# Lynne-Zheng-Linfang/HS-Pose

Hardware: AMD Instinct MI355X
Metric: point-clouds/sec (N=1028) HS-layer fwd+bwd (higher is better)
Workload: dtype f32; 1 GPU; HS stack (FaceRecon backbone -> feat) fwd+bwd, B=16/GPU N=1028 fp32, train-mode BN, random-init weights (BASELINE configs[1] shape); global_batch=16, points=1028, parallelism=dp1, hipgraph=True, split_graph=False, grad_exchange=none

## Files before the change

hs_pose_amd/_lib.py:

```python
import ctypes
import os

_HERE = os.path.dirname(os.path.abspath(__file__))
LIB_PATH = os.environ.get("HSP_LIB") or os.path.join(_HERE, "libhsp.so")
_lib = None

_vp, _i, _sz = ctypes.c_void_p, ctypes.c_int, ctypes.c_size_t

SIGNATURES = {
    "hsp_version": (_i, []),
    "hsp_error_string": (ctypes.c_char_p, [_i]),
    "hsp_last_hip_error": (ctypes.c_char_p, []),
    "hsp_knn_workspace_bytes": (_sz, [_i, _i, _i, _i]),
    "hsp_knn_f32": (_i, [_vp, _i, _i, _i, _i, _i, _vp, _vp, _sz, _vp]),
    "hsp_nn1_f32": (_i, [_vp, _i, _vp, _i, _i, _vp, _vp]),
    "hsp_rf_surface_fwd": (_i, [_vp, _vp, _vp, _i, _i, _i, _i, _i, _vp, _vp, _vp]),
    "hsp_rf_bwd_workspace_bytes": (_sz, [_i]),
    "hsp_rf_surface_bwd": (_i, [_vp, _vp, _vp, _vp, _i, _i, _i, _i, _vp, _vp, _sz, _vp]),
    "hsp_rf_conv_wants_fwin": (_i, [_i, _i, _i]),
    "hsp_rf_conv_fwd": (_i, [_vp, _vp, _vp, _vp, _i, _i, _i, _i, _i, _vp, _vp, _vp, _vp]),
    "hsp_rf_conv_bwd": (_i, [_vp, _vp, _vp, _vp, _vp, _vp, _vp, _i, _i, _i, _i, _i, _vp, _vp, _vp, _sz, _vp]),
    "hsp_rf_bwd_scatter_workspace_bytes": (_sz, [_i, _i]),
    "hsp_rf_conv_bwd_scatter": (_i, [_vp, _vp, _vp, _vp, _vp, _vp, _i, _i, _i, _i, _vp, _vp, _vp, _sz, _vp]),
    "hsp_rev_build": (_i, [_vp, _i, _i, _i, _i, _i, _vp, _vp, _vp]),
    "hsp_gather_max_bwd_csr": (_i, [_vp, _i, _vp, _vp, _vp, _i, _i, _i, _i, _i, _vp, _vp]),
    "hsp_gather_max_fwd": (_i, [_vp, _vp, _vp, _i, _i, _i, _i, _i, _i, _i, _vp, _vp, _vp]),
    "hsp_pool_fwd": (_i, [_vp, _vp, _vp, _vp, _i, _i, _i, _i, _i, _i, _vp, _vp, _vp, _vp]),
    "hsp_gather_max_bwd": (_i, [_vp, _i, _vp, _vp, _vp, _i, _i, _i, _i, _i, _i, _vp, _i, _vp, _vp]),
    "hsp_points_max_fwd": (_i, [_vp, _i, _i, _i, _vp, _vp, _vp]),
    "hsp_points_max_bwd": (_i, [_vp, _vp, _i, _i, _i, _vp, _vp]),
    "hsp_orl_workspace_bytes": (_sz, [_i, _i, _i]),
    "hsp_knn_exact_workspace_bytes": (_sz, [_i, _i, _i, _i, _i]),
    "hsp_knn_exact_f32": (_i, [_vp, _i, _i, _i, _i, _i, _i, _vp, _vp, _sz, _vp, _vp]),
    "hsp_knn_xyz_workspace_bytes": (_sz, [_i, _i]),
    "hsp_knn_xyz_f32": (_i, [_vp, _i, _i, _i, _i, _i, _vp, _vp, _vp, _sz, _vp, _vp]),
    "hsp_geometry_levels_f32": (_i, [_vp, _i, _i, _vp, _i, _vp, _i, _i, _i, _i, _i, _vp, _vp, _vp, _vp, _vp, _vp, _vp, _vp]),
    "hsp_geometry_all_workspace_bytes": (_sz, [_i, _i]),
    "hsp_geometry_all_f32": (_i, [_vp, _i, _i, _i, _i, _vp, _i, _vp, _i, _i, _i, _i, _i, _vp, _vp, _vp, _vp, _vp, _vp, _vp, _vp, _vp, _vp, _sz,
                                  _vp]),
    "hsp_knn_quadmode_f32": (_i, [_vp, _i, _i, _i, _i, _i, _vp, _vp, _sz, _i, _vp]),
    "hsp_quad_outer_f32": (_i, [_vp, _i, _i, _i, _vp, _vp]),
    "hsp_center_cloud_f32": (_i, [_vp, _i, _i, _vp, _vp, _vp]),
    "hsp_orl_exact_workspace_bytes": (_sz, [_i, _i, _i]),
    "hsp_orl_global_exact_f32": (_i, [_vp, _vp, _i, _i, _i, _i, _i, _vp, _vp, _vp, _sz, _vp]),
    "hsp_bn_eval_f32": (_i, [_vp, ctypes.c_longlong, _i, _vp, _vp, _vp, _vp, _vp, ctypes.c_float, _i, _vp, _vp]),
    "hsp_layer_out_exact_f32": (_i, [_vp, _i, _vp, _i, _vp, _i, _vp, _i, _vp, _i, _vp, _i, _vp, _vp, _i, _i, _i, _i, _vp, _i, _vp]),
    "hsp_orl_global_fwd": (_i, [_vp, _vp, _i, _i, _i, _i, _i, _vp, _vp, _vp, _sz, _vp]),
    "hsp_colsum_rows": (_i, [_vp, _i, _i, _i, _vp, _vp, _sz, _vp]),
    "hsp_add_relu_bwd": (_i, [_vp, _i, _vp, _i, _vp, _i, _i, _vp, _vp]),
    "hsp_residual_bias": (_i, [_vp, _vp, _vp, _i, _i, _i, _vp]),
    "hsp_concat_rows": (_i, [_i, _vp, _vp, _vp, _vp, _vp, _i, _i, _vp, _vp]),
    "hsp_gather_rows_fwd": (_i, [_vp, _vp, _i, _i, _i, _i, _i, _vp, _i, _vp]),
    "hsp_gather_rows_bwd": (_i, [_vp, _i, _vp, _i, _i, _i, _i, _i, _vp, _vp]),
    "hsp_gather_rows_bwd_csr": (_i, [_vp, _i, _vp, _vp, _i, _i, _i, _i, _vp, _vp]),
    "hsp_gemm_rows_workspace_bytes": (_sz, [_i, _i, _i, _i, _i]),
    "hsp_gemm_rows_f32": (_i, [_vp, _i, _vp, _i, _i, _i, _vp, _i, _vp, _i, _i, _i, _i, _i, _vp, _vp, _i, _vp, _i, ctypes.c_float, _vp, _vp, _vp, _i, _vp, _sz, _vp]),
    "hsp_gemm_rows_bf16": (_i, [_vp, _i, _vp, _i, _i, _vp, _i, _vp, _i, _i, _i, _i, _vp, _vp, _i, _vp, _i, ctypes.c_float, _vp, _vp, _vp, _i, _i, _vp, _sz, _vp]),
    "hsp_gemm_wave_supported": (_i, [_i, _i, _i, _i, _i]),
    "hsp_gemm_wave_plan_info": (_i, [_i, _i, _i, _i, _i, _vp]),
    "hsp_gemm_wave_f32": (_i, [_vp, _i, _vp, _i, _i, _i, _vp, _i, _vp, _i, _i, _i, _i, _i, _vp, _vp, _i, _vp, _i, ctypes.c_float, _vp, _vp, _vp, _i, _i, _vp]),
    "hsp_split_params_x3": (_i, [_vp, _i, _i, _vp]),
    "hsp_gemm_x3_supported": (_i, [_i, _i, _i, _i]),
    "hsp_gemm_x3_workspace_bytes": (_sz, [_i, _i, _i, _i]),
    "hsp_gemm_x3_f32": (_i, [_vp, _i, _vp, _i, ctypes.c_longlong, _i, _vp, _i, _vp, _i, ctypes.c_longlong, _i, _i, _i, _vp, _vp, _i, _vp, _i,
                             ctypes.c_float, _vp, _i, _vp, _sz, _vp]),
    "hsp_small_rows_f32": (_i, [_vp, _i, _vp, _i, _i, _i, _i, _i, ctypes.c_float, _vp, _i, _vp]),
    "hsp_small_outer_f32": (_i, [_vp, _i, _vp, _i, _i, _i, _i, _vp, _i, _vp, _i, _i, _vp, _vp]),
    "hsp_colsum_rows_xyz": (_i, [_vp, _vp, _i, _i, _i, _vp, _vp, _sz, _vp]),
    "hsp_colsum_rows_xyz_bf16": (_i, [_vp, _vp, _i, _i, _i, _vp, _vp, _sz, _vp]),
    "hsp_colsum_cloud_ok": (_i, [_i, _i, _i, _i]),
    "hsp_colsum_cloud_f32": (_i, [_vp, _vp, _i, _i, _i, _vp, _vp]),
    "hsp_small_pair_f32": (_i, [_vp, _i, _i, _i, _vp, _i, _i, ctypes.c_float, _vp, _i, _vp, _i, _i, _vp, _i, _vp, _i, _i, _vp, _vp]),
    "hsp_bn_relu_fwd_mixed": (_i, [_vp, _i, _i, _vp, _vp, ctypes.c_float, ctypes.c_float, _i, _vp, _vp, _vp, _vp, _vp, _vp, _vp, _sz, _vp]),
    "hsp_bn_relu_apply_mixed": (_i, [_vp, _i, _i, _vp, _vp, _vp, _vp, _i, _vp, _vp]),
    "hsp_bn_relu_bwd_mixed": (_i, [_vp, _vp, _i, _i, _vp, _vp, _vp, _vp, _i, _vp, _vp, _vp, _vp, _sz, _vp]),
    "hsp_cast_params_bf16": (_i, [_vp, _i, _i, _vp]),
    "hsp_cast_params_pitched_bf16": (_i, [_vp, _i, _i, _vp]),
    "hsp_wgrad_ragged_bf16": (_i, [_vp, _i, _vp, _i, _i, _i, _i, _vp, _i, _vp, _vp, _sz, _vp]),
    "hsp_wgrad_ragged_partial_bf16": (_i, [_vp, _i, _vp, _i, _i, _i, _i, _vp, _i, _vp, _vp, _sz, _vp, _vp]),
    "hsp_gemm_rows_acc_bf16": (_i, [_vp, _i, _vp, _i, _i, _vp, _i, _vp, _i, _i, _i, _i, _vp, _i, _vp, _i, _i, _vp, _sz, _vp]),
    "hsp_points_max_fwd_bf16": (_i, [_vp, _i, _i, _i, _vp, _vp, _vp]),
    "hsp_gemm_rows_bn_tiles_bf16": (_i, [_i, _i, _i]),
    "hsp_gemm_rows_bn_bf16": (_i, [_vp, _i, _vp, _i, _i, _i, _i, _vp, _vp, _i, _vp, _vp, _vp, _i, _vp, _vp, _vp]),
    "hsp_bn_relu_fwd_partials_mixed": (_i, [_vp, _i, _i, _vp, _vp, ctypes.c_float, ctypes.c_float, _i, _vp, _vp, _vp, _vp, _vp, _vp,
                                            _vp, _i, _vp, _vp]),
    "hsp_points_max_bwd_bf16": (_i, [_vp, _vp, _i, _i, _i, _vp, _vp]),
    "hsp_knn_bf16": (_i, [_vp, _i, _i, _i, _i, _i, _vp, _vp, _sz, _vp]),
    "hsp_rf_surface_fwd_bf16": (_i, [_vp, _vp, _vp, _i, _i, _i, _i, _i, _vp, _vp, _vp]),
    "hsp_rf_surface_bwd_bf16": (_i, [_vp, _vp, _vp, _vp, _i, _i, _i, _i, _vp, _vp, _sz, _vp]),
    "hsp_rf_conv_wants_fwin_bf16": (_i, [_i, _i, _i]),
    "hsp_rf_conv_fwd_bf16": (_i, [_vp, _vp, _vp, _vp, _i, _i, _i, _i, _i, _vp, _vp, _vp, _vp]),
    "hsp_rf_conv_bwd_scatter_bf16": (_i, [_vp, _vp, _vp, _vp, _vp, _vp, _i, _i, _i, _i, _vp, _vp, _vp, _sz, _vp]),
    "hsp_gather_max_fwd_bf16": (_i, [_vp, _vp, _vp, _i, _i, _i, _i, _i, _i, _i, _vp, _vp, _vp]),
    "hsp_gather_max_bwd_bf16": (_i, [_vp, _i, _vp, _vp, _vp, _i, _i, _i, _i, _i, _i, _vp, _i, _vp, _vp]),
    "hsp_orl_global_fwd_bf16": (_i, [_vp, _vp, _i, _i, _i, _i, _i, _vp, _vp, _vp, _sz, _vp]),
    "hsp_colsum_rows_bf16": (_i, [_vp, _i, _i, _i, _vp, _vp, _sz, _vp]),
    "hsp_concat_rows_pitched": (_i, [_i, _vp, _vp, _vp, _vp, _vp, _i, _i, _vp, _i, _vp]),
    "hsp_concat_rows_bf16": (_i, [_i, _vp, _vp, _vp, _vp, _vp, _i, _i, _vp, _i, _vp]),
    "hsp_gather_rows_bwd_csr_bf16": (_i, [_vp, _i, _vp, _vp, _i, _i, _i, _i, _vp, _vp]),
    "hsp_wgrad_bf16": (_i, [_vp, _i, _vp, _i, _i, _i, _i, _vp, _i, _vp, _vp, _sz, _vp]),
    "hsp_bn_relu_fwd_bf16": (_i, [_vp, _i, _i, _vp, _vp, ctypes.c_float, ctypes.c_float, _i, _vp, _vp, _vp, _vp, _vp, _vp, _vp, _sz, _vp]),
    "hsp_bn_relu_apply_bf16": (_i, [_vp, _i, _i, _vp, _vp, _vp, _vp, _i, _vp, _vp]),
    "hsp_bn_relu_bwd_bf16": (_i, [_vp, _vp, _i, _i, _vp, _vp, _vp, _vp, _i, _vp, _vp, _vp, _vp, _sz, _vp]),
    "hsp_wgrad_workspace_bytes": (_sz, [_i, _i, _i]),
    "hsp_wgrad_f32": (_i, [_vp, _i, _vp, _i, _i, _i, _i, _vp, _i, _vp, _vp, _sz, _vp]),
    "hsp_bn_workspace_bytes": (_sz, [_i, _i]),
    "hsp_bn_relu_fwd": (_i, [_vp, _i, _i, _vp, _vp, ctypes.c_float, ctypes.c_float, _i, _vp, _vp, _vp, _vp, _vp, _vp, _vp, _sz, _vp]),
    "hsp_bn_relu_apply": (_i, [_vp, _i, _i, _vp, _vp, _vp, _vp, _i, _vp, _vp]),
    "hsp_bn_relu_bwd": (_i, [_vp, _vp, _i, _i, _vp, _vp, _vp, _vp, _i, _vp, _vp, _vp, _vp, _sz, _vp]),
    "hsp_gemm_x3_bn_f32": (_i, [_vp, _i, _vp, _i, ctypes.c_longlong, _i, _vp, _i, _vp, _i, ctypes.c_longlong, _i, _i, _i, _vp, _i, _vp, _i,
                                _vp, _i, _vp, _vp, _vp]),
    "hsp_gemm_x3_bn_tiles": (_i, [_i, _i]),
    "hsp_gemm_x3_bias_bn_f32": (_i, [_vp, _i, _vp, _i, ctypes.c_longlong, _i, _i, _i, _vp, _vp, _i, _vp, _vp, _vp]),
    "hsp_bn_relu_fwd_partials": (_i, [_vp, _i, _i, _vp, _vp, ctypes.c_float, ctypes.c_float, _i, _vp, _vp, _vp, _vp, _vp, _vp, _vp, _i,
                                      _vp, _vp]),
    "hsp_bn_relu_bwd2": (_i, [_vp, _vp, _i, _vp, _i, _i, _i, _vp, _vp, _vp, _vp, _i, _vp, _vp, _vp, _vp, _sz, _vp]),
    "hsp_pc_compact_workspace_bytes": (_sz, [_i, _i]),
    "hsp_pc_compact": (_i, [_vp, _vp, _i, _i, _vp, _vp, _vp, _sz, _vp]),
    "hsp_pc_gather": (_i, [_vp, _vp, _vp, _vp, _vp, _i, _i, _i, _vp, _vp]),
    "hsp_depth_to_pcl": (_i, [_vp, _vp, _vp, _vp, _vp, _i, _i, _i, _vp, _vp]),
    "hsp_generate_rt": (_i, [_vp, _vp, _vp, _vp, _vp, _vp, _i, _i, _vp, _vp]),
    "hsp_sumsq_workspace_bytes": (_sz, [ctypes.c_longlong]),
    "hsp_sumsq_f32": (_i, [_vp, ctypes.c_longlong, _vp, _vp, _sz, _vp]),
    "hsp_ranger_step": (_i, [_vp, _vp, _vp, _vp, _vp, _vp, _i, ctypes.c_float, ctypes.c_float, ctypes.c_float,
                             ctypes.c_float, ctypes.c_float, _i, _i, ctypes.c_float, _i, _vp, ctypes.c_float, _vp]),
    "hsp_chamfer_fwd": (_i, [_vp, _vp, _i, _i, _i, _vp, _vp, _vp, _vp, _vp]),
    "hsp_chamfer_bwd": (_i, [_vp, _vp, _vp, _vp, _vp, _vp, _i, _i, _i, _vp, _vp, _vp]),
    "hsp_fps_workspace_bytes": (_sz, [_i, _i]),
    "hsp_fps_f32": (_i, [_vp, _i, _i, _i, _vp, _vp, _sz, _vp]),
    "hsp_fps_f64": (_i, [_vp, _i, _i, _i, _vp, _vp, _sz, _vp]),
    "hsp_axis_conf_fwd": (_i, [_vp, _i, _vp, _vp, _vp]),
    "hsp_axis_conf_bwd": (_i, [_vp, _vp, _vp, _i, _vp, _vp]),
    "hsp_face_split_fwd": (_i, [_vp, ctypes.c_longlong, _vp, _vp, _vp, _vp]),
    "hsp_face_split_bwd": (_i, [_vp, _vp, _vp, _vp, ctypes.c_longlong, _vp, _vp]),
    "hsp_pose_losses_workspace_bytes": (_sz, [_i]),
    "hsp_pose_losses_fwd": (_i, [_vp] * 17 + [_i, _i, _vp, _vp, _vp, _sz, _vp]),
    "hsp_pose_losses_bwd": (_i, [_vp] * 17 + [_i, _i, _vp, _vp, _vp, _sz] + [_vp] * 11 + [_vp]),
    "hsp_wgrad_partial_f32": (_i, [_vp, _i, _vp, _i, _i, _i, _i, _vp, _i, _vp, _vp, _sz, _vp, _vp]),
    "hsp_wgrad_partial_bf16": (_i, [_vp, _i, _vp, _i, _i, _i, _i, _vp, _i, _vp, _vp, _sz, _vp, _vp]),
    "hsp_wgrad_fold": (_i, [_vp, _i, _vp]),
    "hsp_step_fold": (_i, [_vp, _i, _vp, _i, _vp]),
    "hsp_rf_surface_bwd_partial": (_i, [_vp, _vp, _vp, _vp, _i, _i, _i, _i, _vp, _vp, _sz, _vp, _vp]),
    "hsp_rf_conv_bwd_scatter_partial": (_i, [_vp, _vp, _vp, _vp, _vp, _vp, _i, _i, _i, _i, _vp, _vp, _vp, _sz, _vp, _vp]),
    "hsp_rf_surface_bwd_partial_bf16": (_i, [_vp, _vp, _vp, _vp, _i, _i, _i, _i, _vp, _vp, _sz, _vp, _vp]),
    "hsp_rf_conv_bwd_scatter_partial_bf16": (_i, [_vp, _vp, _vp, _vp, _vp, _vp, _i, _i, _i, _i, _vp, _vp, _vp, _sz, _vp, _vp]),
    "hsp_wgrad_partial_pair_f32": (_i, [_vp, _i, _vp, _i, _i, _i, _i, _vp, _i, _vp, _sz] * 2 + [_vp, _vp]),
    "hsp_pose_augment": (_i, [_vp] * 14 + [_i, _i, _i] + [ctypes.c_float] * 4 + [_vp] * 5),
}


class HspLossCfg(ctypes.Structure):
    _fields_ = [(n, ctypes.c_float) for n in (
        "rot_1_w", "rot_2_w", "rot_regular", "tran_w", "size_w", "r_con_w", "recon_n_w", "recon_d_w", "recon_f_w",
        "recon_v_w", "recon_bb_r_w", "recon_bb_t_w", "recon_bb_s_w", "recon_bb_self_w", "geo_p_w", "prop_pm_w",
        "prop_sym_w")] + [("smooth_l1", ctypes.c_int)]


class HspSplitDesc(ctypes.Structure):
    _fields_ = [("src", ctypes.c_void_p), ("dst", ctypes.c_void_p), ("rows", ctypes.c_int), ("cols", ctypes.c_int),
                ("ld", ctypes.c_int), ("transpose", ctypes.c_int), ("kp", ctypes.c_int), ("tile0", ctypes.c_int),
                ("ps", ctypes.c_longlong)]


class HspError(RuntimeError):
    pass


def lib():
    global _lib
    if _lib is None:
        if not os.path.exists(LIB_PATH):
            raise HspError(
                f"{LIB_PATH} not found: the HIP extension is not built. Run "
                "`python -c 'import __graft_entry__ as g; g.build()'` (or `make -C hs_pose_amd/csrc`). "
                "hs_pose_amd has no CPU / eager fallback.")
        import torch
        L = ctypes.CDLL(LIB_PATH)
        for name, (res, args) in SIGNATURES.items():
            fn = getattr(L, name)
            fn.restype = res
            fn.argtypes = args
        _lib = L
    return _lib


def check(rc, what):
    if rc != 0:
        L = lib()
        msg = L.hsp_error_string(rc).decode()
        hip = L.hsp_last_hip_error().decode()
        raise HspError(f"{what} failed: {msg} (code {rc})" + (f" [hip: {hip}]" if hip and rc == -4 else ""))


class HspWgradPending(ctypes.Structure):
    _fields_ = [("part", ctypes.c_void_p), ("cs_part", ctypes.c_void_p), ("C", ctypes.c_void_p), ("colsum", ctypes.c_void_p),
                ("nparts", ctypes.c_int), ("M", ctypes.c_int), ("N", ctypes.c_int), ("ldc", ctypes.c_int)]


class HspDirsPending(ctypes.Structure):
# ... 3 lines not shown
```

hs_pose_amd/csrc/common.h:

```cpp
#pragma once
#include <hip/hip_runtime.h>
#include <stdint.h>
#include <limits.h>
#include <math.h>

#include "hsp.h"

#define HSP_WAVE 64
#define HSP_NUM_XCD 8
#define HSP_NUM_CU 256

namespace hsp {

void set_last_hip_error(hipError_t e);

inline int check_launch() {
    hipError_t e = hipGetLastError();
    if (e != hipSuccess) {
        set_last_hip_error(e);
        return HSP_ERR_LAUNCH;
    }
    return HSP_OK;
}

inline hipStream_t as_stream(hspStream_t s) { return reinterpret_cast<hipStream_t>(s); }

int knn_feat_select_flags(const float* x, int B, int N, int C, int k, int drop, int quad_mode, int32_t* idx, void* ws, size_t ws_bytes,
                          uint8_t* tie, float* dmat, hspStream_t stream);
int knn3_select_flags(const float* x, int B, int N, int k, int drop, int k2, int32_t* idx, int32_t* idx2, uint8_t* tie,
                      hipStream_t st, bool* needs_tie_pass);

inline int persistent_blocks(long long work_items, int blocks_per_cu) {
    long long g = (long long)HSP_NUM_CU * blocks_per_cu;
    if (work_items < g) g = ((work_items + HSP_NUM_XCD - 1) / HSP_NUM_XCD) * HSP_NUM_XCD;
    if (g < HSP_NUM_XCD) g = HSP_NUM_XCD;
    return (int)g;
}

__device__ __forceinline__ float mul_rn(float a, float b) { return __fmul_rn(a, b); }
__device__ __forceinline__ float add_rn(float a, float b) { return __fadd_rn(a, b); }
__device__ __forceinline__ float sub_rn(float a, float b) { return __fsub_rn(a, b); }

__device__ __forceinline__ float quad3(float x, float y, float z) {
    return add_rn(add_rn(mul_rn(x, x), mul_rn(y, y)), mul_rn(z, z));
}

__device__ __forceinline__ float dot3_chain(float ax, float ay, float az, float bx, float by, float bz) {
    return __fmaf_rn(az, bz, __fmaf_rn(ay, by, mul_rn(ax, bx)));
}

__device__ __forceinline__ float norm2_chain(float x, float y, float z) { return __fmaf_rn(z, z, __fmaf_rn(y, y, mul_rn(x, x))); }

__device__ __forceinline__ float3 unit_dir(float px, float py, float pz, float qx, float qy, float qz) {
    float dx = sub_rn(qx, px), dy = sub_rn(qy, py), dz = sub_rn(qz, pz);
    float n2 = norm2_chain(dx, dy, dz);
    float nrm = fmaxf(sqrtf(n2), 1e-12f);
    return make_float3(__fdiv_rn(dx, nrm), __fdiv_rn(dy, nrm), __fdiv_rn(dz, nrm));
}

__device__ __forceinline__ float3 unit_dir_fast(float px, float py, float pz, float qx, float qy, float qz) {
    const float dx = qx - px, dy = qy - py, dz = qz - pz;
    const float inv = fminf(__builtin_amdgcn_rsqf(dx * dx + dy * dy + dz * dz), 1e12f);
    return make_float3(dx * inv, dy * inv, dz * inv);
}

typedef unsigned short bf16_t;

__device__ __forceinline__ float bf16_bits_to_f32(unsigned v) { return __uint_as_float(v << 16); }
__device__ __forceinline__ unsigned f32_to_bf16_bits(float f) {
    unsigned u = __float_as_uint(f);
    if ((u & 0x7fffffffu) > 0x7f800000u) return (u >> 16) | 0x40u;
    u += 0x7fffu + ((u >> 16) & 1u);
    return u >> 16;
}

template <typename FT> struct Feat;
template <> struct Feat<float> {
    static __device__ __forceinline__ float ld(const float* p) { return *p; }
    static __device__ __forceinline__ void st(float* p, float v) { *p = v; }
    static __device__ __forceinline__ void st_nt(float* p, float v) { __builtin_nontemporal_store(v, p); }
    static __device__ __forceinline__ float4 ld4(const float* p) { return *reinterpret_cast<const float4*>(p); }
    static __device__ __forceinline__ void st4(float* p, float4 v) { *reinterpret_cast<float4*>(p) = v; }
    static __device__ __forceinline__ void st4_nt(float* p, float4 v) {
// ... 28 lines not shown
```

hs_pose_amd/csrc/csr.hip:

```cpp
#include "common.h"

namespace hsp {

#define REV_THREADS 1024

template <bool EDGES_IN_LDS>
__global__ __launch_bounds__(REV_THREADS) void rev_build_kernel(const int32_t* __restrict__ idx, int Nq, int Nsrc,
                                                                int k, int kstride, int32_t* __restrict__ rev_off,
                                                                int32_t* __restrict__ rev_edge) {
    extern __shared__ __attribute__((aligned(16))) char smem[];
    int* cnt = reinterpret_cast<int*>(smem);
    int* led = cnt + Nsrc + 1;
    __shared__ int wsum[REV_THREADS / 64];
    const int b = blockIdx.x, tid = threadIdx.x, lane = tid & 63, wv = tid >> 6;
    const int32_t* ib = idx + (size_t)b * Nq * kstride;
    int32_t* off = rev_off + (size_t)b * (Nsrc + 1);
    int32_t* edge = rev_edge + (size_t)b * Nq * k;
    int* ed = EDGES_IN_LDS ? led : edge;
    const int E = Nq * k;

    for (int m = tid; m <= Nsrc; m += REV_THREADS) cnt[m] = 0;
    __syncthreads();
    for (int e = tid; e < E; e += REV_THREADS) {
        const int i = e / k, n = e - i * k;
        atomicAdd(&cnt[ib[(size_t)i * kstride + n]], 1);
    }
    __syncthreads();
    const int per = (Nsrc + REV_THREADS - 1) / REV_THREADS;
    const int lo = min(tid * per, Nsrc), hi = min(lo + per, Nsrc);
    int s = 0;
    for (int m = lo; m < hi; ++m) s += cnt[m];
    int inc = s;
#pragma unroll
    for (int d = 1; d < 64; d <<= 1) {
        const int v = __shfl_up(inc, d);
        if (lane >= d) inc += v;
    }
    if (lane == 63) wsum[wv] = inc;
    __syncthreads();
    if (wv == 0) {
        int t = lane < REV_THREADS / 64 ? wsum[lane] : 0;
#pragma unroll
        for (int d = 1; d < REV_THREADS / 64; d <<= 1) {
            const int v = __shfl_up(t, d);
            if (lane >= d) t += v;
        }
        if (lane < REV_THREADS / 64) wsum[lane] = t;
    }
    __syncthreads();
    int run = inc - s + (wv ? wsum[wv - 1] : 0);
    for (int m = lo; m < hi; ++m) {
        const int c = cnt[m];
        cnt[m] = run;
        off[m] = run;
        run += c;
    }
    if (tid == 0) off[Nsrc] = E;
    __syncthreads();
    for (int e0 = 0; e0 < E; e0 += REV_THREADS) {
        const int e = e0 + tid;
        if (e < E) {
            const int i = e / k, n = e - i * k;
            const int pos = atomicAdd(&cnt[ib[(size_t)i * kstride + n]], 1);
            ed[pos] = e;
        }
        __syncthreads();
    }
    if (!EDGES_IN_LDS) __threadfence_block();
    __syncthreads();
    if (EDGES_IN_LDS && k == 1) {
        for (int p = tid; p < E; p += REV_THREADS) {
            const int e = led[p];
            const int i = e / k, n = e - i * k;
            const int m = ib[(size_t)i * kstride + n];
            const int a = m ? cnt[m - 1] : 0, z = cnt[m];
            int c = 0;
            for (int q = a; q < z; ++q) c += led[q] < e ? 1 : 0;
            edge[a + c] = e;
        }
    } else {
        for (int m = tid; m < Nsrc; m += REV_THREADS) {
            const int a = m ? cnt[m - 1] : 0, z = cnt[m];
            for (int p = a + 1; p < z; ++p) {
                const int v = ed[p];
                int q = p - 1;
                while (q >= a && ed[q] > v) { ed[q + 1] = ed[q]; --q; }
                ed[q + 1] = v;
            }
        }
        if (EDGES_IN_LDS) {
            __syncthreads();
            for (int e = tid; e < E; e += REV_THREADS) edge[e] = led[e];
        }
    }
}

}

using namespace hsp;

extern "C" int hsp_rev_build(const int32_t* idx, int B, int Nq, int Nsrc, int k, int kstride, int32_t* rev_off,
                             int32_t* rev_edge, hspStream_t stream) {
    if (!idx || !rev_off || !rev_edge || B <= 0 || Nq <= 0 || Nsrc <= 0 || k <= 0 || kstride < k) return HSP_ERR_BAD_ARG;
    const size_t lds0 = (size_t)(Nsrc + 1) * sizeof(int);
    if (lds0 > 140 * 1024) return HSP_ERR_UNSUPPORTED;
    const size_t lds1 = lds0 + (size_t)Nq * k * sizeof(int);
    const bool in_lds = lds1 <= 140 * 1024;
    const size_t lds = in_lds ? lds1 : lds0;
    auto kern = in_lds ? rev_build_kernel<true> : rev_build_kernel<false>;
    if (lds > 60 * 1024) {
        hipError_t e = hipFuncSetAttribute(reinterpret_cast<const void*>(kern), hipFuncAttributeMaxDynamicSharedMemorySize, (int)lds);
        if (e != hipSuccess) { set_last_hip_error(e); return HSP_ERR_LAUNCH; }
    }
    hipLaunchKernelGGL(kern, dim3(B), dim3(REV_THREADS), lds, as_stream(stream), idx, Nq, Nsrc, k, kstride, rev_off,
                       rev_edge);
    return check_launch();
}
```

hs_pose_amd/csrc/gather.hip:

```cpp
#include "common.h"
#include <type_traits>

namespace hsp {

template <typename FT>
__device__ __forceinline__ void gather_max_rows(const FT* __restrict__ fb, const int32_t* __restrict__ nb, int k,
                                                int C, float4& best, int& a0, int& a1, int& a2, int& a3) {
    constexpr int NB = 8;
    int cur[NB], nxt[NB];
#pragma unroll
    for (int u = 0; u < NB; ++u) cur[u] = nb[min(u, k - 1)];
    for (int n0 = 0; n0 < k; n0 += NB) {
#pragma unroll
        for (int u = 0; u < NB; ++u) nxt[u] = nb[min(n0 + NB + u, k - 1)];
        float4 f[NB];
#pragma unroll
        for (int u = 0; u < NB; ++u) f[u] = Feat<FT>::ld4(fb + (size_t)cur[u] * C);
#pragma unroll
        for (int u = 0; u < NB; ++u) {
            const int n = n0 + u;
            if (n < k) {
                if (f[u].x > best.x) { best.x = f[u].x; a0 = n; }
                if (f[u].y > best.y) { best.y = f[u].y; a1 = n; }
                if (f[u].z > best.z) { best.z = f[u].z; a2 = n; }
                if (f[u].w > best.w) { best.w = f[u].w; a3 = n; }
            }
        }
#pragma unroll
        for (int u = 0; u < NB; ++u) cur[u] = nxt[u];
    }
}


template <typename FT>
__global__ __launch_bounds__(256) void gather_max_fwd_kernel(const FT* __restrict__ feat,
                                                             const int32_t* __restrict__ idx,
                                                             const int32_t* __restrict__ qsel, int B, int Nsrc,
                                                             int Nidx, int Nq, int k, int kstride, int C,
                                                             FT* __restrict__ out,
                                                             uint8_t* __restrict__ argmax,
                                                             const float* __restrict__ xyz = nullptr,
                                                             float* __restrict__ xyz_sel = nullptr) {
    const int cq = C >> 2;
    const long long total = (long long)B * Nq * cq;
    for (long long e = (long long)blockIdx.x * 256 + threadIdx.x; e < total; e += (long long)gridDim.x * 256) {
        const int g = (int)(e % cq);
        const long long row = e / cq;
        const int q = (int)(row % Nq);
        const int b = (int)(row / Nq);
        const int qi = qsel ? qsel[q] : q;
        if (xyz_sel && g < 3)
            xyz_sel[row * 3 + g] = xyz[((size_t)b * Nidx + qi) * 3 + g];
        const int32_t* nb = idx + ((size_t)b * Nidx + qi) * kstride;
// ... 107 lines not shown
        if (i < N) {
            const unsigned short* my = strip + pw * k;
            float4 f[K];
#pragma unroll
            for (int n = 0; n < K; ++n) {
                const char* rp = slab + ((unsigned)my[n] << SH);
                if constexpr (sizeof(FT) == 4) f[n] = *reinterpret_cast<const float4*>(rp);
                else {
                    const uint2 u2 = *reinterpret_cast<const uint2*>(rp);
                    f[n] = make_float4(__uint_as_float(u2.x << 16), __uint_as_float(u2.x & 0xffff0000u), __uint_as_float(u2.y << 16),
                                       __uint_as_float(u2.y & 0xffff0000u));
                }
            }
            ORL_STAMP(3 + 3 * (i0 / PASS));
            float4 best = f[0];
#pragma unroll
            for (int n = 1; n + 1 < K; n += 2) {
                best.x = max3_raw(best.x, f[n].x, f[n + 1].x); best.y = max3_raw(best.y, f[n].y, f[n + 1].y);
                best.z = max3_raw(best.z, f[n].z, f[n + 1].z); best.w = max3_raw(best.w, f[n].w, f[n + 1].w);
            }
            if ((K & 1) == 0) {
                best.x = max3_raw(best.x, f[K - 1].x, f[K - 1].x); best.y = max3_raw(best.y, f[K - 1].y, f[K - 1].y);
                best.z = max3_raw(best.z, f[K - 1].z, f[K - 1].z); best.w = max3_raw(best.w, f[K - 1].w, f[K - 1].w);
            }
            int a0 = 0, a1 = 0, a2 = 0, a3 = 0;
#pragma unroll
            for (int n = K - 1; n >= 1; --n) {
                a0 = f[n].x == best.x ? n : a0; a1 = f[n].y == best.y ? n : a1;
                a2 = f[n].z == best.z ? n : a2; a3 = f[n].w == best.w ? n : a3;
            }
            a0 = f[0].x == best.x ? 0 : a0; a1 = f[0].y == best.y ? 0 : a1; a2 = f[0].z == best.z ? 0 : a2; a3 = f[0].w == best.w ? 0 : a3;
            *reinterpret_cast<uchar4*>(argmax + ((size_t)b * N + i) * C + c0 + (q << 2)) =
                make_uchar4((unsigned char)a0, (unsigned char)a1, (unsigned char)a2, (unsigned char)a3);
            s.x += best.x; s.y += best.y; s.z += best.z; s.w += best.w;
        }
        __builtin_amdgcn_fence(__ATOMIC_ACQUIRE, "wavefront");
        ORL_STAMP(4 + 3 * (i0 / PASS));
    }
    ORL_STAMP(30);
#pragma unroll
    for (int d = 2; d < 64; d <<= 1) {
        s.x += __shfl_xor(s.x, d); s.y += __shfl_xor(s.y, d); s.z += __shfl_xor(s.z, d); s.w += __shfl_xor(s.w, d);
    }
    if (lane < 2) red[wave * 2 + q] = s;
    __syncthreads();
    if (tid < 2) {
        float4 t = red[q];
        for (int w = 1; w < ORLT_WG / 64; ++w) { const float4 v = red[w * 2 + q]; t.x += v.x; t.y += v.y; t.z += v.z; t.w += v.w; }
        *reinterpret_cast<float4*>(fg + (size_t)b * C + c0 + (q << 2)) = make_float4(t.x * inv_n, t.y * inv_n, t.z * inv_n, t.w * inv_n);
    }
    ORL_STAMP(31);
}

__device__ __forceinline__ float chunk_fold8(const float* __restrict__ p, int nchunk, int stride) {
    float s[8] = {0.f, 0.f, 0.f, 0.f, 0.f, 0.f, 0.f, 0.f};
    int ch = 0;
    for (; ch + 7 < nchunk; ch += 8) {
#pragma unroll
        for (int u = 0; u < 8; ++u) s[u] += p[(size_t)(ch + u) * stride];
    }
    for (; ch < nchunk; ++ch) s[ch & 7] += p[(size_t)ch * stride];
    return ((s[0] + s[1]) + (s[2] + s[3])) + ((s[4] + s[5]) + (s[6] + s[7]));
}

__global__ __launch_bounds__(256) void chunk_fold_kernel(const float* __restrict__ part, int B, int nchunk, int C,
                                                         float scale, float* __restrict__ out) {
    const int e = blockIdx.x * 256 + threadIdx.x;
    if (e >= B * C) return;
    const int b = e / C, c = e - b * C;
    out[e] = chunk_fold8(part + (size_t)b * nchunk * C + c, nchunk, C) * scale;
}

template <typename FT>
__global__ __launch_bounds__(256) void colsum_partial_kernel(const FT* __restrict__ x, int N, int C,
                                                             float* __restrict__ part, int nchunk, int rows) {
    __shared__ float4 red[256];
    const int cq = C >> 2;
    const int tid = threadIdx.x;
    const int g = tid % cq, rl = tid / cq, RL = 256 / cq;
    const int b = blockIdx.y, chunk = blockIdx.x;
    const int r0 = chunk * rows, r1 = min(N, r0 + rows);
    float4 s = make_float4(0.f, 0.f, 0.f, 0.f);
    for (int i = r0 + rl; i < r1; i += RL) {
        const float4 v = Feat<FT>::ld4(x + ((size_t)b * N + i) * C + (g << 2));
        s.x += v.x; s.y += v.y; s.z += v.z; s.w += v.w;
    }
    red[tid] = s;
    __syncthreads();
    if (rl == 0) {
        for (int l = 1; l < RL; ++l) { const float4 v = red[l * cq + g]; s.x += v.x; s.y += v.y; s.z += v.z; s.w += v.w; }
        *reinterpret_cast<float4*>(part + ((size_t)b * nchunk + chunk) * C + (g << 2)) = s;
    }
}

__device__ __forceinline__ float fma_plain(float a, float b, float c) {
    float r;
    asm volatile("v_fma_f32 %0, %1, %2, %3" : "=v"(r) : "v"(a), "v"(b), "v"(c));
    return r;
}

template <typename FT>
__global__ __launch_bounds__(256) void colsum_xyz_partial_kernel(const FT* __restrict__ x, const float* __restrict__ xyz, int N, int C,
                                                                 float* __restrict__ part, int nchunk, int rows) {
    __shared__ float4 red[4][256];
    const int cq = C >> 2;
    const int tid = threadIdx.x;
    const int g = tid % cq, rl = tid / cq, RL = 256 / cq;
    const int b = blockIdx.y, chunk = blockIdx.x;
    const int r0 = chunk * rows, r1 = min(N, r0 + rows);
    float4 s[4];
#pragma unroll
    for (int q = 0; q < 4; ++q) s[q] = make_float4(0.f, 0.f, 0.f, 0.f);
    for (int i = r0 + rl; i < r1; i += RL) {
        const float4 v = Feat<FT>::ld4(x + ((size_t)b * N + i) * C + (g << 2));
        const float* p3 = xyz + ((size_t)b * N + i) * 3;
        const float w[3] = {p3[0], p3[1], p3[2]};
        s[0].x += v.x; s[0].y += v.y; s[0].z += v.z; s[0].w += v.w;
#pragma unroll
        for (int q = 0; q < 3; ++q) {
            s[q + 1].x = fma_plain(v.x, w[q], s[q + 1].x); s[q + 1].y = fma_plain(v.y, w[q], s[q + 1].y);
            s[q + 1].z = fma_plain(v.z, w[q], s[q + 1].z); s[q + 1].w = fma_plain(v.w, w[q], s[q + 1].w);
        }
    }
#pragma unroll
    for (int q = 0; q < 4; ++q) red[q][tid] = s[q];
    __syncthreads();
    if (rl == 0) {
#pragma unroll
        for (int q = 0; q < 4; ++q) {
            float4 a = s[q];
            for (int l = 1; l < RL; ++l) { const float4 v = red[q][l * cq + g]; a.x += v.x; a.y += v.y; a.z += v.z; a.w += v.w; }
            *reinterpret_cast<float4*>(part + (((size_t)b * nchunk + chunk) * 4 + q) * C + (g << 2)) = a;
        }
    }
}

template <bool XYZ>
__global__ __launch_bounds__(1024) void colsum_cloud_kernel(const float* __restrict__ x, const float* __restrict__ xyz, int N, int C,
                                                            int nchunk, int rows, float* __restrict__ out) {
    extern __shared__ float4 cc_smem[];
    constexpr int NS = XYZ ? 4 : 1;
    const int cq = C >> 2, RL = 256 / cq, G = cq >> 3;
    const int tid = threadIdx.x;
    const int gl = tid % G, rl = (tid / G) % RL, cs = tid / (G * RL);
    const int g = blockIdx.x * G + gl, b = blockIdx.y;
    float4* red = cc_smem;
    float4* cp = cc_smem + 1024;
    for (int c0 = 0; c0 < nchunk; c0 += 32) {
        const int chunk = c0 + cs;
        const int r0 = chunk * rows, r1 = chunk < nchunk ? min(N, r0 + rows) : 0;
        float4 s[NS];
#pragma unroll
        for (int q = 0; q < NS; ++q) s[q] = make_float4(0.f, 0.f, 0.f, 0.f);
        for (int i = r0 + rl; i < r1; i += RL) {
            const float4 v = *reinterpret_cast<const float4*>(x + ((size_t)b * N + i) * C + (g << 2));
            s[0].x += v.x; s[0].y += v.y; s[0].z += v.z; s[0].w += v.w;
            if constexpr (XYZ) {
                const float* p3 = xyz + ((size_t)b * N + i) * 3;
                const float w[3] = {p3[0], p3[1], p3[2]};
#pragma unroll
                for (int q = 0; q < 3; ++q) {
                    s[q + 1].x = fma_plain(v.x, w[q], s[q + 1].x); s[q + 1].y = fma_plain(v.y, w[q], s[q + 1].y);
                    s[q + 1].z = fma_plain(v.z, w[q], s[q + 1].z); s[q + 1].w = fma_plain(v.w, w[q], s[q + 1].w);
                }
            }
        }
#pragma unroll
        for (int q = 0; q < NS; ++q) {
            red[tid] = s[q];
            __syncthreads();
            if (rl == 0 && chunk < nchunk) {
                float4 a = s[q];
                for (int l = 1; l < RL; ++l) { const float4 v = red[(cs * RL + l) * G + gl]; a.x += v.x; a.y += v.y; a.z += v.z; a.w += v.w; }
                cp[((size_t)q * nchunk + chunk) * G + gl] = a;
            }
            __syncthreads();
        }
    }
    const int TC = G << 2;
    if (tid < NS * TC) {
        const int q = tid / TC, c = tid - q * TC;
        out[(size_t)b * NS * C + (size_t)q * C + blockIdx.x * TC + c] =
            chunk_fold8(reinterpret_cast<const float*>(cp) + (size_t)q * nchunk * TC + c, nchunk, TC);
    }
}

__global__ __launch_bounds__(256) void colsum_partial_scalar_kernel(const float* __restrict__ x, int N, int C,
                                                                    float* __restrict__ part, int nchunk, int rows) {
    __shared__ float red[256];
    const int tid = threadIdx.x;
    const int RL = 256 / C;
    const int col = tid % C, rl = tid / C;
    const int b = blockIdx.y, chunk = blockIdx.x;
    const int r0 = chunk * rows, r1 = min(N, r0 + rows);
    float s = 0.f;
    if (rl < RL)
        for (int i = r0 + rl; i < r1; i += RL) s += x[((size_t)b * N + i) * C + col];
    red[tid] = s;
    __syncthreads();
    if (rl == 0) {
        for (int l = 1; l < RL; ++l) s += red[l * C + col];
        part[((size_t)b * nchunk + chunk) * C + col] = s;
    }
}

struct ConcatSeg { const void* src; const int32_t* idx; int width; int kind; int nsrc; int col0; };
struct ConcatDesc { ConcatSeg seg[8]; int nseg; int even; int q0[9]; };

template <typename FT>
__global__ __launch_bounds__(256) void concat_rows_kernel(ConcatDesc d, int B, int N, int W, FT* __restrict__ out) {
    using Pair = typename std::conditional<sizeof(FT) == 4, float2, unsigned>::type;
    const long long rows = (long long)B * N;
    if (d.even == 2) {
        const int lane = threadIdx.x & 63;
        const int total = d.q0[d.nseg];
        for (long long row = (long long)blockIdx.x * 4 + (threadIdx.x >> 6); row < rows; row += (long long)gridDim.x * 4) {
            const int b = (int)(row / N);
            FT* o = out + (size_t)row * W;
            for (int q = lane; q < total; q += 64) {
                int sgi = 0;
                while (q >= d.q0[sgi + 1]) ++sgi;
                const ConcatSeg sg = d.seg[sgi];
                const int c = q - d.q0[sgi];
                if (sg.kind >= 2) {
                    const float* ps = reinterpret_cast<const float*>(sg.src);
                    Feat<FT>::st(o + sg.col0 + c, sg.kind == 2 ? ps[(size_t)b * sg.width + c] : ((long long)ps[b] == c ? 1.f : 0.f));
                    continue;
                }
                const FT* src = reinterpret_cast<const FT*>(sg.src);
                src += sg.kind == 0 ? (size_t)row * sg.width : ((size_t)b * sg.nsrc + sg.idx[row]) * sg.width;
                reinterpret_cast<uint4*>(o + sg.col0)[c] = reinterpret_cast<const uint4*>(src)[c];
            }
            const int used = d.seg[d.nseg - 1].col0 + d.seg[d.nseg - 1].width;
            if (lane < W - used) Feat<FT>::st(o + used + lane, 0.f);
        }
        return;
    }
// ... 467 lines not shown
        hipLaunchKernelGGL(gather_max_bwd_kernel, dim3(stream_grid(total)), dim3(256), 0, st,
                           reinterpret_cast<const float*>(grad_out), grad_bcast, idx, qsel, argmax, B, Nsrc, Nidx, Nq, kstride, C,
                           grad_feat);
        return check_launch();
    }
    return HSP_ERR_UNSUPPORTED;
}
extern "C" int hsp_gather_max_bwd(const float* grad_out, int grad_bcast, const int32_t* idx, const int32_t* qsel,
                                  const uint8_t* argmax, int B, int Nsrc, int Nidx, int Nq, int kstride, int C,
                                  float* grad_feat, int accumulate, const float* extra, hspStream_t stream) {
    return gather_max_bwd_impl<float>(grad_out, grad_bcast, idx, qsel, argmax, B, Nsrc, Nidx, Nq, kstride, C, grad_feat,
                                      accumulate, extra, stream);
}
extern "C" int hsp_gather_max_bwd_bf16(const void* grad_out, int grad_bcast, const int32_t* idx, const int32_t* qsel,
                                       const uint8_t* argmax, int B, int Nsrc, int Nidx, int Nq, int kstride, int C,
                                       hsp_bf16_t* grad_feat, int accumulate, const hsp_bf16_t* extra, hspStream_t stream) {
    return gather_max_bwd_impl<bf16_t>(grad_out, grad_bcast, idx, qsel, argmax, B, Nsrc, Nidx, Nq, kstride, C, grad_feat,
                                       accumulate, extra, stream);
}

extern "C" int hsp_gather_rows_fwd(const float* feat, const int32_t* idx, int idx_shared, int B, int Nsrc, int Nq,
                                   int C, float* out, int out_stride, hspStream_t stream) {
    if (!feat || !idx || !out || B <= 0 || Nsrc <= 0 || Nq <= 0 || C <= 0 || out_stride < C) return HSP_ERR_BAD_ARG;
    hipStream_t st = as_stream(stream);
    if ((C & 3) == 0) {
        const long long total = (long long)B * Nq * (C >> 2);
        hipLaunchKernelGGL(gather_rows_fwd_kernel, dim3(stream_grid(total)), dim3(256), 0, st, feat, idx, idx_shared, B,
                           Nsrc, Nq, C, out, out_stride);
    } else {
        const long long total = (long long)B * Nq * C;
        hipLaunchKernelGGL(gather_rows_fwd_scalar_kernel, dim3(stream_grid(total)), dim3(256), 0, st, feat, idx,
                           idx_shared, B, Nsrc, Nq, C, out, out_stride);
    }
    return check_launch();
}

extern "C" int hsp_gather_rows_bwd(const float* grad_out, int grad_stride, const int32_t* idx, int idx_shared, int B,
                                   int Nsrc, int Nq, int C, float* grad_feat, hspStream_t stream) {
    if (!grad_out || !idx || !grad_feat || B <= 0 || Nsrc <= 0 || Nq <= 0 || C <= 0 || grad_stride < C)
        return HSP_ERR_BAD_ARG;
    hipStream_t st = as_stream(stream);
    if ((C & 3) == 0 && (grad_stride & 1) == 0 && (reinterpret_cast<uintptr_t>(grad_out) & 7) == 0)
        if (const int tc = pick_scatter_cols(Nsrc, C))
            return launch_scatter_tile<1, float>(tc, grad_out, nullptr, grad_stride, 0, idx, idx_shared, nullptr, nullptr, B,
                                                 Nsrc, Nq, Nq, 1, C, grad_feat, 0, nullptr, st);
    hipError_t e = hipMemsetAsync(grad_feat, 0, (size_t)B * Nsrc * C * sizeof(float), st);
    if (e != hipSuccess) { set_last_hip_error(e); return HSP_ERR_LAUNCH; }
    const long long total = (long long)B * Nq * C;
    hipLaunchKernelGGL(gather_rows_bwd_kernel, dim3(stream_grid(total)), dim3(256), 0, st, grad_out, grad_stride, idx,
                       idx_shared, B, Nsrc, Nq, C, grad_feat);
    return check_launch();
}

template <typename FT>
__global__ __launch_bounds__(256) void gather_rows_bwd_csr_kernel(const FT* __restrict__ gout, int gstride,
                                                                  const int32_t* __restrict__ rev_off,
                                                                  const int32_t* __restrict__ rev_edge, int B,
                                                                  int Nsrc, int Nq, int C,
                                                                  FT* __restrict__ gfeat) {
    const int pairs = C >> 1;
    const int tpr = pairs < 256 ? pairs : 256;
    const int RB = 256 / tpr;
    const int rl = threadIdx.x / tpr, t = threadIdx.x - rl * tpr;
    const long long row = (long long)blockIdx.x * RB + rl;
    if (rl >= RB || row >= (long long)B * Nsrc) return;
    const int m = (int)(row % Nsrc), b = (int)(row / Nsrc);
    const int32_t* off = rev_off + (size_t)b * (Nsrc + 1);
    const int32_t* edge = rev_edge + (size_t)b * Nq;
    const int o0 = off[m], o1 = off[m + 1];
    const FT* gb = gout + (size_t)b * Nq * gstride;
    for (int p = t; p < pairs; p += tpr) {
        float2 acc = make_float2(0.f, 0.f);
        for (int e = o0; e < o1; e += 4) {
            float2 v[4];
#pragma unroll
            for (int u = 0; u < 4; ++u) {
                const int q = edge[min(e + u, o1 - 1)];
                if constexpr (sizeof(FT) == 4) {
                    v[u] = *reinterpret_cast<const float2*>(gb + (size_t)q * gstride + 2 * p);
                } else {
                    const unsigned w = *reinterpret_cast<const unsigned*>(gb + (size_t)q * gstride + 2 * p);
                    v[u] = make_float2(__uint_as_float(w << 16), __uint_as_float(w & 0xffff0000u));
                }
            }
#pragma unroll
            for (int u = 0; u < 4; ++u)
                if (e + u < o1) { acc.x += v[u].x; acc.y += v[u].y; }
        }
        if constexpr (sizeof(FT) == 4) *reinterpret_cast<float2*>(gfeat + (size_t)row * C + 2 * p) = acc;
        else *reinterpret_cast<unsigned*>(gfeat + (size_t)row * C + 2 * p) = f32_to_bf16_bits(acc.x) | (f32_to_bf16_bits(acc.y) << 16);
    }
}

template <typename FT>
static int gather_rows_bwd_csr_impl(const FT* grad_out, int grad_stride, const int32_t* rev_off,
                                    const int32_t* rev_edge, int B, int Nsrc, int Nq, int C, FT* grad_feat,
                                    hspStream_t stream) {
    if (!grad_out || !rev_off || !rev_edge || !grad_feat || B <= 0 || Nsrc <= 0 || Nq <= 0 || C <= 0 || grad_stride < C)
        return HSP_ERR_BAD_ARG;
    if ((C & 1) || (grad_stride & 1) || (reinterpret_cast<uintptr_t>(grad_out) & (2 * sizeof(FT) - 1)) ||
        (256 % ((C >> 1) < 256 ? (C >> 1) : 256)))
        return HSP_ERR_UNSUPPORTED;
    const int tpr = (C >> 1) < 256 ? (C >> 1) : 256;
    const int RB = 256 / tpr;
    const long long rows = (long long)B * Nsrc;
    hipLaunchKernelGGL(gather_rows_bwd_csr_kernel<FT>, dim3((unsigned)((rows + RB - 1) / RB)), dim3(256), 0, as_stream(stream),
                       grad_out, grad_stride, rev_off, rev_edge, B, Nsrc, Nq, C, grad_feat);
    return check_launch();
}
extern "C" int hsp_gather_rows_bwd_csr(const float* grad_out, int grad_stride, const int32_t* rev_off,
                                       const int32_t* rev_edge, int B, int Nsrc, int Nq, int C, float* grad_feat,
                                       hspStream_t stream) {
    return gather_rows_bwd_csr_impl<float>(grad_out, grad_stride, rev_off, rev_edge, B, Nsrc, Nq, C, grad_feat, stream);
}
extern "C" int hsp_gather_rows_bwd_csr_bf16(const hsp_bf16_t* grad_out, int grad_stride, const int32_t* rev_off,
                                            const int32_t* rev_edge, int B, int Nsrc, int Nq, int C, hsp_bf16_t* grad_feat,
                                            hspStream_t stream) {
    return gather_rows_bwd_csr_impl<bf16_t>(grad_out, grad_stride, rev_off, rev_edge, B, Nsrc, Nq, C, grad_feat, stream);
}

extern "C" int hsp_gather_max_bwd_csr(const float* grad_out, int grad_bcast, const uint8_t* argmax,
                                      const int32_t* rev_off, const int32_t* rev_edge, int B, int Nsrc, int Nq, int k,
                                      int C, float* grad_feat, hspStream_t stream) {
    if (!grad_out || !argmax || !rev_off || !rev_edge || !grad_feat || B <= 0 || Nsrc <= 0 || Nq <= 0 || k <= 0 || C <= 0)
        return HSP_ERR_BAD_ARG;
    if (C & 3) return HSP_ERR_UNSUPPORTED;
    const long long total = (long long)B * Nsrc * (C >> 2);
    hipLaunchKernelGGL(gather_max_bwd_csr_kernel, dim3(stream_grid(total)), dim3(256), 0, as_stream(stream), grad_out,
                       grad_bcast, argmax, rev_off, rev_edge, B, Nsrc, Nq, k, C, grad_feat);
    return check_launch();
}

extern "C" int hsp_points_max_fwd(const float* x, int B, int N, int C, float* out, int32_t* argrow, hspStream_t stream) {
    if (!x || !out || !argrow || B <= 0 || N <= 0 || C <= 0) return HSP_ERR_BAD_ARG;
    hipLaunchKernelGGL(points_max_fwd_kernel<float>, dim3((C + 63) / 64, B), dim3(1024), 0, as_stream(stream), x, N, C, out,
                       argrow);
    return check_launch();
}

extern "C" int hsp_points_max_fwd_bf16(const hsp_bf16_t* x, int B, int N, int C, float* out, int32_t* argrow,
                                       hspStream_t stream) {
    if (!x || !out || !argrow || B <= 0 || N <= 0 || C <= 0) return HSP_ERR_BAD_ARG;
    hipLaunchKernelGGL(points_max_fwd_kernel<bf16_t>, dim3((C + 63) / 64, B), dim3(1024), 0, as_stream(stream),
                       reinterpret_cast<const bf16_t*>(x), N, C, out, argrow);
    return check_launch();
}

extern "C" int hsp_points_max_bwd(const float* grad_out, const int32_t* argrow, int B, int N, int C, float* grad_x,
                                  hspStream_t stream) {
    if (!grad_out || !argrow || !grad_x || B <= 0 || N <= 0 || C <= 0) return HSP_ERR_BAD_ARG;
    if (C & 3) return HSP_ERR_UNSUPPORTED;
    const long long total = (long long)B * N * (C >> 2);
    hipLaunchKernelGGL(points_max_bwd_kernel<float>, dim3(stream_grid(total)), dim3(256), 0, as_stream(stream), grad_out,
                       argrow, N, C >> 2, total, grad_x);
    return check_launch();
}

extern "C" int hsp_points_max_bwd_bf16(const float* grad_out, const int32_t* argrow, int B, int N, int C, hsp_bf16_t* grad_x,
                                       hspStream_t stream) {
    if (!grad_out || !argrow || !grad_x || B <= 0 || N <= 0 || C <= 0) return HSP_ERR_BAD_ARG;
    if (C & 3) return HSP_ERR_UNSUPPORTED;
// ... 41 lines not shown
}
extern "C" int hsp_orl_global_fwd(const float* feat, const int32_t* idx, int B, int N, int k, int kstride, int C,
                                  float* fg, uint8_t* argmax, void* ws, size_t ws_bytes, hspStream_t stream) {
    return orl_global_fwd_impl<float>(feat, idx, B, N, k, kstride, C, fg, argmax, ws, ws_bytes, stream);
}
extern "C" int hsp_orl_global_fwd_bf16(const hsp_bf16_t* feat, const int32_t* idx, int B, int N, int k, int kstride, int C,
                                       float* fg, uint8_t* argmax, void* ws, size_t ws_bytes, hspStream_t stream) {
    return orl_global_fwd_impl<bf16_t>(feat, idx, B, N, k, kstride, C, fg, argmax, ws, ws_bytes, stream);
}

extern "C" int hsp_colsum_rows(const float* x, int B, int N, int C, float* out, void* ws, size_t ws_bytes,
                               hspStream_t stream) {
    if (!x || !out || B <= 0 || N <= 0 || C <= 0) return HSP_ERR_BAD_ARG;
    if (!colsum_vec4(C) && C > 256) return HSP_ERR_UNSUPPORTED;
    if (!ws || ws_bytes < hsp_orl_workspace_bytes(B, N, C)) return HSP_ERR_WORKSPACE;
    hipStream_t st = as_stream(stream);
    const int rows = chunk_rows(B, N, C);
    const int nchunk = (N + rows - 1) / rows;
    float* part = reinterpret_cast<float*>(ws);
    if (colsum_vec4(C))
        hipLaunchKernelGGL(colsum_partial_kernel<float>, dim3(nchunk, B), dim3(256), 0, st, x, N, C, part, nchunk, rows);
    else
        hipLaunchKernelGGL(colsum_partial_scalar_kernel, dim3(nchunk, B), dim3(256), 0, st, x, N, C, part, nchunk, rows);
    hipLaunchKernelGGL(chunk_fold_kernel, dim3((B * C + 255) / 256), dim3(256), 0, st, part, B, nchunk, C, 1.0f, out);
    return check_launch();
}

template <typename FT>
static int colsum_rows_xyz_impl(const FT* x, const float* xyz, int B, int N, int C, float* out4, void* ws, size_t ws_bytes,
                                hspStream_t stream) {
    if (!x || !xyz || !out4 || B <= 0 || N <= 0 || C <= 0) return HSP_ERR_BAD_ARG;
    if (!colsum_vec4(C)) return HSP_ERR_UNSUPPORTED;
    if (!ws || ws_bytes < 4 * hsp_orl_workspace_bytes(B, N, C)) return HSP_ERR_WORKSPACE;
    hipStream_t st = as_stream(stream);
    const int rows = chunk_rows(B, N, C);
    const int nchunk = (N + rows - 1) / rows;
    float* part = reinterpret_cast<float*>(ws);
    hipLaunchKernelGGL(colsum_xyz_partial_kernel<FT>, dim3(nchunk, B), dim3(256), 0, st, x, xyz, N, C, part, nchunk, rows);
    hipLaunchKernelGGL(chunk_fold_kernel, dim3((B * 4 * C + 255) / 256), dim3(256), 0, st, part, B, nchunk, 4 * C, 1.0f, out4);
    return check_launch();
}
extern "C" int hsp_colsum_rows_xyz(const float* x, const float* xyz, int B, int N, int C, float* out4, void* ws, size_t ws_bytes,
                                   hspStream_t stream) {
    return colsum_rows_xyz_impl<float>(x, xyz, B, N, C, out4, ws, ws_bytes, stream);
}
extern "C" int hsp_colsum_rows_xyz_bf16(const hsp_bf16_t* x, const float* xyz, int B, int N, int C, float* out4, void* ws,
                                        size_t ws_bytes, hspStream_t stream) {
    return colsum_rows_xyz_impl<bf16_t>(x, xyz, B, N, C, out4, ws, ws_bytes, stream);
}

static size_t colsum_cloud_lds(int B, int N, int C, int with_xyz) {
    const int rows = chunk_rows(B, N, C);
    return (1024 + (size_t)(with_xyz ? 4 : 1) * ((N + rows - 1) / rows) * (C >> 5)) * sizeof(float4);
}
extern "C" int hsp_colsum_cloud_ok(int B, int N, int C, int with_xyz) {
    if (B <= 0 || B > 65535 || N <= 0 || C <= 0 || (C & 31) || !colsum_vec4(C)) return 0;
    return colsum_cloud_lds(B, N, C, with_xyz) <= 64 * 1024 ? 1 : 0;
}
extern "C" int hsp_colsum_cloud_f32(const float* x, const float* xyz, int B, int N, int C, float* out, hspStream_t stream) {
    if (!x || !out || B <= 0 || N <= 0 || C <= 0) return HSP_ERR_BAD_ARG;
    if (!hsp_colsum_cloud_ok(B, N, C, xyz != nullptr)) return HSP_ERR_UNSUPPORTED;
    hipStream_t st = as_stream(stream);
    const int rows = chunk_rows(B, N, C);
    const int nchunk = (N + rows - 1) / rows;
    const size_t lds = colsum_cloud_lds(B, N, C, xyz != nullptr);
    if (xyz)
        hipLaunchKernelGGL(colsum_cloud_kernel<true>, dim3(8, B), dim3(1024), lds, st, x, xyz, N, C, nchunk, rows, out);
    else
        hipLaunchKernelGGL(colsum_cloud_kernel<false>, dim3(8, B), dim3(1024), lds, st, x, xyz, N, C, nchunk, rows, out);
    return check_launch();
}

extern "C" int hsp_colsum_rows_bf16(const hsp_bf16_t* x, int B, int N, int C, float* out, void* ws, size_t ws_bytes,
                                    hspStream_t stream) {
    if (!x || !out || B <= 0 || N <= 0 || C <= 0) return HSP_ERR_BAD_ARG;
    if (!colsum_vec4(C)) return HSP_ERR_UNSUPPORTED;
    if (!ws || ws_bytes < hsp_orl_workspace_bytes(B, N, C)) return HSP_ERR_WORKSPACE;
    hipStream_t st = as_stream(stream);
    const int rows = chunk_rows(B, N, C);
    const int nchunk = (N + rows - 1) / rows;
    float* part = reinterpret_cast<float*>(ws);
    hipLaunchKernelGGL(colsum_partial_kernel<bf16_t>, dim3(nchunk, B), dim3(256), 0, st, x, N, C, part, nchunk, rows);
    hipLaunchKernelGGL(chunk_fold_kernel, dim3((B * C + 255) / 256), dim3(256), 0, st, part, B, nchunk, C, 1.0f, out);
    return check_launch();
}

template <typename FT>
static int concat_rows_impl(int nseg, const void* const* src, const int32_t* const* idx, const int* width,
                            const int* kind, const int* nsrc, int B, int N, FT* out, int out_pitch, hspStream_t stream) {
    if (nseg <= 0 || nseg > 8 || !src || !width || !kind || !out || B <= 0 || N <= 0) return HSP_ERR_BAD_ARG;
    ConcatDesc d;
    d.nseg = nseg;
    int col = 0;
    for (int s = 0; s < nseg; ++s) {
        if (!src[s] || width[s] <= 0 || kind[s] < 0 || kind[s] > 3 || (kind[s] == 1 && (!idx || !idx[s]))) return HSP_ERR_BAD_ARG;
        d.seg[s].src = src[s];
        d.seg[s].idx = idx ? idx[s] : nullptr;
        d.seg[s].width = width[s];
        d.seg[s].kind = kind[s];
        d.seg[s].nsrc = nsrc ? nsrc[s] : 0;
        d.seg[s].col0 = col;
        col += width[s];
    }
    if (out_pitch < col) return HSP_ERR_BAD_ARG;
    d.even = (out_pitch & 1) ? 0 : 1;
    for (int s = 0; s < nseg; ++s)
// ... 58 lines not shown
```

hs_pose_amd/csrc/gemm.hip:

```cpp
#include "common.h"
#include "folds.h"

namespace hsp {

using f32x16 = __attribute__((ext_vector_type(16))) float;

#define WG_UNROLL 4

template <bool COLSUM, int KB, typename FT>
__device__ __forceinline__ void wgrad_body(const int bid, const FT* __restrict__ A, int lda,
                                           const FT* __restrict__ B, int ldb, int M, int N, int K,
                                           int SK, int kslice, float* __restrict__ part,
                                           float* __restrict__ cs_part) {
    extern __shared__ __attribute__((aligned(16))) char smem[];
    const int lane = threadIdx.x & 63;
    const int wv = __builtin_amdgcn_readfirstlane(threadIdx.x >> 6);
    const int tiles = (M >> 6) * (N >> 6);
    int slice, t;
    if (KB == 1) {
        const int w = bid * 4 + wv;
        if (w >= tiles * SK) return;
        slice = w / tiles; t = w - slice * tiles;
    } else {
        const int grp = bid / tiles;
        t = bid - grp * tiles;
        slice = grp * 4 + wv;
    }
    const int tiles_m = M >> 6;
    const int tn = t / tiles_m, tm = t - tn * tiles_m;
    const int m0 = tm << 6, n0 = tn << 6;
    const int k0 = slice * kslice;
    const int k1 = min(K, k0 + kslice);
    const int h = lane >> 5, i = lane & 31;
    constexpr int ES = sizeof(FT);
    const __amdgpu_buffer_rsrc_t ra = __builtin_amdgcn_make_buffer_rsrc(
        const_cast<FT*>(A), 0, (int)((((size_t)K - 1) * lda + M) * ES), 0x00020000);
    const __amdgpu_buffer_rsrc_t rb = __builtin_amdgcn_make_buffer_rsrc(
        const_cast<FT*>(B), 0, (int)((((size_t)K - 1) * ldb + N) * ES), 0x00020000);
    const int va = (h * lda + m0 + 2 * i) * ES, vb = (h * ldb + n0 + 2 * i) * ES;
    f32x16 c00, c01, c10, c11;
#pragma unroll
    for (int r = 0; r < 16; ++r) { c00[r] = 0.f; c01[r] = 0.f; c10[r] = 0.f; c11[r] = 0.f; }
    float2 cs = make_float2(0.f, 0.f);

    float2 a0[WG_UNROLL], b0[WG_UNROLL], a1[WG_UNROLL], b1[WG_UNROLL];
    auto load_group = [&](int kk, float2 (&aa)[WG_UNROLL], float2 (&bb)[WG_UNROLL]) {
#pragma unroll
        for (int u = 0; u < WG_UNROLL; ++u) {
            if constexpr (ES == 4) {
                const auto x = __builtin_amdgcn_raw_buffer_load_b64(ra, va, (kk + 2 * u) * lda * 4, 0);
                const auto y = __builtin_amdgcn_raw_buffer_load_b64(rb, vb, (kk + 2 * u) * ldb * 4, 0);
                aa[u] = make_float2(__int_as_float(x[0]), __int_as_float(x[1]));
                bb[u] = make_float2(__int_as_float(y[0]), __int_as_float(y[1]));
            } else {
// ... 33 lines not shown
            const int row = (r & 3) + 8 * (r >> 2) + 4 * h;
            *reinterpret_cast<float2*>(pc + (size_t)(m0 + 2 * row) * N + n0 + 2 * i) = make_float2(c00[r], c01[r]);
            *reinterpret_cast<float2*>(pc + (size_t)(m0 + 2 * row + 1) * N + n0 + 2 * i) = make_float2(c10[r], c11[r]);
        }
        if (COLSUM && tm == 0) {
            cs.x += __shfl_xor(cs.x, 32);
            cs.y += __shfl_xor(cs.y, 32);
            if (h == 0) *reinterpret_cast<float2*>(cs_part + (size_t)slice * N + n0 + 2 * i) = cs;
        }
        return;
    }
    float* buf = reinterpret_cast<float*>(smem);
    float2* csb = reinterpret_cast<float2*>(buf + 4 * 4 * 16 * 64);
#pragma unroll
    for (int r = 0; r < 16; ++r) {
        buf[((wv * 4 + 0) * 16 + r) * 64 + lane] = c00[r];
        buf[((wv * 4 + 1) * 16 + r) * 64 + lane] = c01[r];
        buf[((wv * 4 + 2) * 16 + r) * 64 + lane] = c10[r];
        buf[((wv * 4 + 3) * 16 + r) * 64 + lane] = c11[r];
    }
    if (COLSUM) csb[wv * 64 + lane] = cs;
    __syncthreads();
    const int grp = bid / tiles;
    float* pc = part + (size_t)grp * M * N;
    const int ta = wv >> 1, tb = wv & 1;
#pragma unroll
    for (int r = 0; r < 16; ++r) {
        float v = buf[((0 * 4 + wv) * 16 + r) * 64 + lane];
        v += buf[((1 * 4 + wv) * 16 + r) * 64 + lane];
        v += buf[((2 * 4 + wv) * 16 + r) * 64 + lane];
        v += buf[((3 * 4 + wv) * 16 + r) * 64 + lane];
        const int row = (r & 3) + 8 * (r >> 2) + 4 * h;
        pc[(size_t)(m0 + 2 * row + ta) * N + n0 + 2 * i + tb] = v;
    }
    if (COLSUM && tm == 0 && wv == 0) {
        float2 c = csb[lane];
#pragma unroll
        for (int w2 = 1; w2 < 4; ++w2) { c.x += csb[w2 * 64 + lane].x; c.y += csb[w2 * 64 + lane].y; }
        c.x += __shfl_xor(c.x, 32);
        c.y += __shfl_xor(c.y, 32);
        if (h == 0) *reinterpret_cast<float2*>(cs_part + (size_t)grp * N + n0 + 2 * i) = c;
    }
}

template <bool COLSUM, int KB, typename FT>
__global__ __launch_bounds__(256) void wgrad_kernel(const FT* __restrict__ A, int lda,
                                                    const FT* __restrict__ B, int ldb, int M, int N, int K,
                                                    int SK, int kslice, float* __restrict__ part,
                                                    float* __restrict__ cs_part) {
    wgrad_body<COLSUM, KB, FT>((int)blockIdx.x, A, lda, B, ldb, M, N, K, SK, kslice, part, cs_part);
}

struct WgradProb { const float* A; const float* B; float* part; int lda, ldb, M, N, K, SK, kslice; };
__global__ __launch_bounds__(256) void wgrad_pair_kernel(const WgradProb p0, const WgradProb p1, int blocks0) {
    const bool second = (int)blockIdx.x >= blocks0;
    const WgradProb& p = second ? p1 : p0;
    wgrad_body<false, 4, float>((int)blockIdx.x - (second ? blocks0 : 0), p.A, p.lda, p.B, p.ldb, p.M, p.N, p.K, p.SK, p.kslice,
                                p.part, nullptr);
}

__global__ __launch_bounds__(256) void wgrad_reduce_kernel(const float* __restrict__ part, int SK, int M, int N,
                                                           float* __restrict__ C, int ldc,
                                                           const float* __restrict__ cs_part,
                                                           float* __restrict__ colsum) {
    __shared__ float4 red[4][64];
    const int le = threadIdx.x & 63, sg = threadIdx.x >> 6;
    const int nq = N >> 2;
    const long long total = (long long)M * nq;
    const long long ncs = colsum ? (N >> 2) : 0;
    const long long e = (long long)blockIdx.x * 64 + le;
    float4 s = make_float4(0.f, 0.f, 0.f, 0.f);
    const float* src = nullptr;
    size_t stride = 0;
    if (e < total) { src = part + (size_t)e * 4; stride = (size_t)M * N; }
    else if (e < total + ncs) { src = cs_part + (size_t)(e - total) * 4; stride = (size_t)N; }
    if (src) {
        float4 s2 = make_float4(0.f, 0.f, 0.f, 0.f);
        int sl = sg;
        for (; sl + 4 < SK; sl += 8) {
            const float4 v = *reinterpret_cast<const float4*>(src + (size_t)sl * stride);
            const float4 u = *reinterpret_cast<const float4*>(src + (size_t)(sl + 4) * stride);
            s.x += v.x; s.y += v.y; s.z += v.z; s.w += v.w;
            s2.x += u.x; s2.y += u.y; s2.z += u.z; s2.w += u.w;
        }
        if (sl < SK) {
            const float4 v = *reinterpret_cast<const float4*>(src + (size_t)sl * stride);
            s.x += v.x; s.y += v.y; s.z += v.z; s.w += v.w;
        }
        s.x += s2.x; s.y += s2.y; s.z += s2.z; s.w += s2.w;
    }
    red[sg][le] = s;
    __syncthreads();
    if (sg == 0 && src) {
        float4 r = red[0][le];
#pragma unroll
        for (int g = 1; g < 4; ++g) { const float4 v = red[g][le]; r.x += v.x; r.y += v.y; r.z += v.z; r.w += v.w; }
        if (e < total) {
            const int m = (int)(e / nq), q = (int)(e - (long long)m * nq);
            float* c = C + (size_t)m * ldc + (q << 2);
            c[0] = r.x; c[1] = r.y; c[2] = r.z; c[3] = r.w;
        } else {
            *reinterpret_cast<float4*>(colsum + (size_t)(e - total) * 4) = r;
        }
    }
}

struct WgradFoldTab {
// ... 469 lines not shown
            if (rc) return rc;
            if (pending) { *pending = HspWgradPending{part, cs_part, C, colsum_B, sk2, M, N, ldc}; return HSP_OK; }
            const long long total = (long long)M * (N >> 2) + (colsum_B ? (N >> 2) : 0);
            hipLaunchKernelGGL(wgrad_reduce_kernel, dim3((unsigned)((total + 63) / 64)), dim3(256), 0, st, part, sk2, M, N, C, ldc,
                               cs_part, colsum_B);
            return check_launch();
        }
    }
    const int sk = wgrad_pick_sk(M, N, K, &ks, &kb);
    const int nparts = sk / kb;
    float* part = reinterpret_cast<float*>(ws);
    float* cs_part = part + (size_t)nparts * M * N;
    int rc = colsum_B ? wgrad_launch<true, FT>(A, lda, B, ldb, M, N, K, sk, ks, kb, part, cs_part, st)
                      : wgrad_launch<false, FT>(A, lda, B, ldb, M, N, K, sk, ks, kb, part, cs_part, st);
    if (rc) return rc;
    if (pending) { *pending = HspWgradPending{part, cs_part, C, colsum_B, nparts, M, N, ldc}; return HSP_OK; }
    const long long total = (long long)M * (N >> 2) + (colsum_B ? (N >> 2) : 0);
    hipLaunchKernelGGL(wgrad_reduce_kernel, dim3((unsigned)((total + 63) / 64)), dim3(256), 0, st, part, nparts, M, N, C,
                       ldc, cs_part, colsum_B);
    return check_launch();
}

extern "C" int hsp_wgrad_f32(const float* A, int lda, const float* B, int ldb, int M, int N, int K, float* C, int ldc,
                             float* colsum_B, void* ws, size_t ws_bytes, hspStream_t stream) {
    return wgrad_impl<float>(A, lda, B, ldb, M, N, K, C, ldc, colsum_B, ws, ws_bytes, stream);
}
extern "C" int hsp_wgrad_bf16(const hsp_bf16_t* A, int lda, const hsp_bf16_t* B, int ldb, int M, int N, int K, float* C,
                              int ldc, float* colsum_B, void* ws, size_t ws_bytes, hspStream_t stream) {
    return wgrad_impl<bf16_t>(A, lda, B, ldb, M, N, K, C, ldc, colsum_B, ws, ws_bytes, stream);
}

extern "C" int hsp_wgrad_ragged_bf16(const hsp_bf16_t* A, int lda, const hsp_bf16_t* B, int ldb, int M, int N, int K, float* C,
                                     int ldc, float* colsum_B, void* ws, size_t ws_bytes, hspStream_t stream) {
    return wgrad_impl<bf16_t>(A, lda, B, ldb, M, N, K, C, ldc, colsum_B, ws, ws_bytes, stream, nullptr, true);
}
extern "C" int hsp_wgrad_ragged_partial_bf16(const hsp_bf16_t* A, int lda, const hsp_bf16_t* B, int ldb, int M, int N, int K,
                                             float* C, int ldc, float* colsum_B, void* ws, size_t ws_bytes,
                                             HspWgradPending* pending, hspStream_t stream) {
    if (!pending) return HSP_ERR_BAD_ARG;
    return wgrad_impl<bf16_t>(A, lda, B, ldb, M, N, K, C, ldc, colsum_B, ws, ws_bytes, stream, pending, true);
}

extern "C" int hsp_wgrad_partial_f32(const float* A, int lda, const float* B, int ldb, int M, int N, int K, float* C, int ldc,
                                     float* colsum_B, void* ws, size_t ws_bytes, HspWgradPending* pending, hspStream_t stream) {
    if (!pending) return HSP_ERR_BAD_ARG;
    return wgrad_impl<float>(A, lda, B, ldb, M, N, K, C, ldc, colsum_B, ws, ws_bytes, stream, pending);
}
extern "C" int hsp_wgrad_partial_bf16(const hsp_bf16_t* A, int lda, const hsp_bf16_t* B, int ldb, int M, int N, int K, float* C,
                                      int ldc, float* colsum_B, void* ws, size_t ws_bytes, HspWgradPending* pending,
                                      hspStream_t stream) {
    if (!pending) return HSP_ERR_BAD_ARG;
    return wgrad_impl<bf16_t>(A, lda, B, ldb, M, N, K, C, ldc, colsum_B, ws, ws_bytes, stream, pending);
}
extern "C" int hsp_wgrad_partial_pair_f32(const float* A0, int lda0, const float* B0, int ldb0, int M0, int N0, int K0, float* C0,
                                          int ldc0, void* ws0, size_t ws_bytes0, const float* A1, int lda1, const float* B1,
                                          int ldb1, int M1, int N1, int K1, float* C1, int ldc1, void* ws1, size_t ws_bytes1,
                                          HspWgradPending* pending, hspStream_t stream) {
    if (!pending) return HSP_ERR_BAD_ARG;
    int ks0, kb0, ks1, kb1;
    const bool shapes_ok = A0 && B0 && C0 && A1 && B1 && C1 && M0 > 0 && N0 > 0 && K0 > 0 && M1 > 0 && N1 > 0 && K1 > 0 &&
                           !((M0 | N0 | M1 | N1) & 63) && !((lda0 | ldb0 | lda1 | ldb1) & 1) && lda0 >= M0 && ldb0 >= N0 &&
                           lda1 >= M1 && ldb1 >= N1 && ldc0 >= N0 && ldc1 >= N1;
    if (shapes_ok) {
        int sk0 = wgrad_pick_sk(M0, N0, K0, &ks0, &kb0), sk1 = wgrad_pick_sk(M1, N1, K1, &ks1, &kb1);
        if (kb0 == 4 && kb1 == 4) {
            constexpr int G = 4 * WG_UNROLL;
            const int t0 = (M0 >> 6) * (N0 >> 6), t1 = (M1 >> 6) * (N1 >> 6);
            int total = t0 * (sk0 / 4) + t1 * (sk1 / 4);
            for (int it = 0; it < 8 && total > 2 * HSP_NUM_CU && sk0 > 8 && sk1 > 8; ++it) {
                const double f = (double)(2 * HSP_NUM_CU) / total;
                auto shrink = [&](int K, int& sk, int& ks) {
                    int want = (int)(sk * f) & ~3;
                    if (want >= sk) want = sk - 4;
                    if (want < 8) want = 8;
                    ks = ((K + want - 1) / want + G - 1) / G * G;
                    sk = (((K + ks - 1) / ks) + 3) & ~3;
                };
                shrink(K0, sk0, ks0);
                shrink(K1, sk1, ks1);
                total = t0 * (sk0 / 4) + t1 * (sk1 / 4);
            }
        }
        if (kb0 == 4 && kb1 == 4 && ws0 && ws1 && ws_bytes0 >= hsp_wgrad_workspace_bytes(M0, N0, K0) &&
            ws_bytes1 >= hsp_wgrad_workspace_bytes(M1, N1, K1)) {
            const WgradProb p0{A0, B0, reinterpret_cast<float*>(ws0), lda0, ldb0, M0, N0, K0, sk0, ks0};
            const WgradProb p1{A1, B1, reinterpret_cast<float*>(ws1), lda1, ldb1, M1, N1, K1, sk1, ks1};
            const int blocks0 = (M0 >> 6) * (N0 >> 6) * (sk0 / 4), blocks1 = (M1 >> 6) * (N1 >> 6) * (sk1 / 4);
            const size_t lds = (size_t)4 * 4 * 16 * 64 * sizeof(float) + (size_t)4 * 64 * sizeof(float2);
            static bool attr_set = false;
            if (!attr_set) {
                hipError_t e = hipFuncSetAttribute(reinterpret_cast<const void*>(wgrad_pair_kernel),
                                                   hipFuncAttributeMaxDynamicSharedMemorySize, (int)lds);
                if (e != hipSuccess) { set_last_hip_error(e); return HSP_ERR_LAUNCH; }
                attr_set = true;
            }
            hipLaunchKernelGGL(wgrad_pair_kernel, dim3(blocks0 + blocks1), dim3(256), lds, as_stream(stream), p0, p1, blocks0);
            int rc = check_launch();
            if (rc) return rc;
            pending[0] = HspWgradPending{p0.part, nullptr, C0, nullptr, sk0 / 4, M0, N0, ldc0};
            pending[1] = HspWgradPending{p1.part, nullptr, C1, nullptr, sk1 / 4, M1, N1, ldc1};
            return HSP_OK;
        }
    }
    int rc = wgrad_impl<float>(A0, lda0, B0, ldb0, M0, N0, K0, C0, ldc0, nullptr, ws0, ws_bytes0, stream, pending);
    if (rc) return rc;
    return wgrad_impl<float>(A1, lda1, B1, ldb1, M1, N1, K1, C1, ldc1, nullptr, ws1, ws_bytes1, stream, pending + 1);
}

extern "C" int hsp_wgrad_fold(const HspWgradPending* pending, int n, hspStream_t stream) {
    if (!pending || n <= 0 || n > HSP_FOLD_MAX_WGRAD) return HSP_ERR_BAD_ARG;
    WgradFoldTab tab;
    tab.n = n;
    int blocks = 0;
    for (int i = 0; i < n; ++i) {
        const HspWgradPending& p = pending[i];
        if (!p.part || !p.C || p.nparts <= 0 || p.M <= 0 || p.N <= 0 || (p.N & 3) || p.ldc < p.N || (p.colsum && !p.cs_part))
            return HSP_ERR_BAD_ARG;
        tab.first[i] = blocks;
        const long long total = (long long)p.M * (p.N >> 2) + (p.colsum ? (p.N >> 2) : 0);
        blocks += (int)((total + 63) / 64);
        tab.p[i] = p;
    }
    tab.first[n] = blocks;
    hipLaunchKernelGGL(wgrad_reduce_multi_kernel, dim3((unsigned)blocks), dim3(256), 0, as_stream(stream), tab);
    return check_launch();
}

static bool wgrad_pending_ok(const HspWgradPending& p) {
    return p.part && p.C && p.nparts > 0 && p.M > 0 && p.N > 0 && !(p.N & 3) && p.ldc >= p.N && !(p.colsum && !p.cs_part);
}

extern "C" int hsp_step_fold(const HspWgradPending* wgrads, int nw, const HspDirsPending* dirs, int nd, hspStream_t stream) {
    if (nw < 0 || nd < 0 || nw > HSP_FOLD_MAX_WGRAD || nd > HSP_FOLD_MAX_DIRS || (nw && !wgrads) || (nd && !dirs)) return HSP_ERR_BAD_ARG;
    if (nw + nd == 0) return HSP_OK;
    StepFoldTab tab;
    tab.nw = nw; tab.nd = nd;
    int blocks = 0;
    for (int i = 0; i < nw; ++i) {
        const HspWgradPending& p = wgrads[i];
        if (!wgrad_pending_ok(p)) return HSP_ERR_BAD_ARG;
        tab.wfirst[i] = blocks;
        const long long total = (long long)p.M * (p.N >> 2) + (p.colsum ? (p.N >> 2) : 0);
        blocks += (int)((total + 63) / 64);
        tab.w[i] = p;
    }
    tab.wfirst[nw] = blocks;
    int dblocks = 0;
    for (int i = 0; i < nd; ++i) {
        const HspDirsPending& p = dirs[i];
        if (!p.part || !p.dirs || !p.grad_dirs || p.nparts <= 0 || p.SC <= 0) return HSP_ERR_BAD_ARG;
        tab.dfirst[i] = dblocks;
        dblocks += (p.SC + 63) / 64;
        tab.d[i] = p;
    }
    tab.dfirst[nd] = dblocks;
    hipLaunchKernelGGL(step_fold_kernel, dim3((unsigned)(blocks + dblocks)), dim3(256), 0, as_stream(stream), tab);
    return check_launch();
}
```

hs_pose_amd/ops.py:

```python
import ctypes
import os

import torch

from ._lib import HspError, check, lib

_vp = ctypes.c_void_p

DETERMINISTIC = os.environ.get("HSP_DETERMINISTIC", "0") == "1"


def _p(t):
    return _vp(t.data_ptr()) if t is not None else _vp(0)


def _stream():
    return _vp(torch.cuda.current_stream().cuda_stream)


def _req(t, dtype, name):
    if not isinstance(t, torch.Tensor) or not t.is_cuda:
        raise HspError(f"{name}: expected a GPU tensor (hs_pose_amd has no CPU path), got "
                       f"{getattr(t, 'device', type(t))}")
    if t.dtype != dtype:
# ... 2 lines not shown


_FEAT_DTYPES = (torch.float32, torch.bfloat16)


def _reqf(t, name, like=None):
    if not isinstance(t, torch.Tensor) or not t.is_cuda:
        raise HspError(f"{name}: expected a GPU tensor (hs_pose_amd has no CPU path), got "
                       f"{getattr(t, 'device', type(t))}")
    if t.dtype not in _FEAT_DTYPES or (like is not None and t.dtype != like.dtype):
        raise HspError(f"{name}: expected dtype {like.dtype if like is not None else 'float32 or bfloat16'}, got {t.dtype}")
    return t if t.is_contiguous() else t.contiguous()


def _sfx(t):
    return "_bf16" if t.dtype == torch.bfloat16 else ""


def _es(t):
    return 2 if t.dtype == torch.bfloat16 else 4


def _ws(nbytes, device):
    return torch.empty(max(int(nbytes), 16), dtype=torch.uint8, device=device)


class KernelTimer:

    def __init__(self, only=None):
        self.only = set(only) if only else None
        self.records = []

    def summary(self):
        out = {}
        for name, key, ab, fl, e0, e1 in self.records:
            d = out.setdefault((name, key), dict(calls=0, total_ms=0.0, abytes=ab, aflops=fl))
            d["calls"] += 1
            d["total_ms"] += e0.elapsed_time(e1)
        for d in out.values():
            d["avg_us"] = 1e3 * d["total_ms"] / d["calls"]
        return out


_timer = None
design_stream_bytes = {}


def set_timer(t):
    global _timer
    prev, _timer = _timer, t
    return prev


def _run(name, args, key="", abytes=0, aflops=0):
    fn = getattr(lib(), name)
    t = _timer
    if t is not None and (t.only is None or name in t.only):
        e0 = torch.cuda.Event(enable_timing=True)
        e1 = torch.cuda.Event(enable_timing=True)
        e0.record()
        rc = fn(*args)
        e1.record()
        t.records.append((name, key, abytes, aflops, e0, e1))
    else:
        rc = fn(*args)
    check(rc, name)



def knn_xyz(xyz, k, k2=0, drop_first=True):
    x = _req(xyz.detach(), torch.float32, "knn_xyz.xyz")
    B, N, C = x.shape
    if C != 3:
        raise HspError("knn_xyz: expects (B,N,3) coordinates")
    k2 = int(k2) if k2 and k2 < k else 0
    m = k + (1 if drop_first else 0)
    if m + 1 > 33 or N < 2 or N * 16 > 160 * 1024:
        idx = knn(x, k, drop_first, _plain_xyz=True)
        return idx, (idx[:, :, :k2].contiguous() if k2 else None)
    idx = torch.empty(B, N, k, dtype=torch.int32, device=x.device)
    idx2 = torch.empty(B, N, k2, dtype=torch.int32, device=x.device) if k2 else None
    wsb = lib().hsp_knn_xyz_workspace_bytes(B, N)
    ws = _ws(wsb, x.device)
    _run("hsp_knn_xyz_f32", (_p(x), B, N, k, k2, 1 if drop_first else 0, _p(idx), _p(idx2), _p(ws), wsb, None, _stream()),
         key=f"B{B}N{N}k{k}", abytes=B * N * (12 + 4 * (k + k2)))
    return idx, idx2


def geometry_all(xyz, k0, kpool0, sel1, sel2, k1, kpool, k2):
    x = _req(xyz.detach(), torch.float32, "geometry_all.xyz")
    s1, s2 = _req(sel1, torch.int32, "geometry_all.sel1"), _req(sel2, torch.int32, "geometry_all.sel2")
    B, N0, C = x.shape
    N1, N2 = s1.numel(), s2.numel()
    if (C != 3 or not (64 <= N2 <= N1 <= 576) or not (576 < N0 <= 1088) or B * N0 >= 131072 or k1 + 2 > 33 or k2 + 2 > 33 or k0 + 2 > 33
            or k1 + 1 > N1 or k2 + 1 > N2 or not 0 < kpool <= k1 or not 0 < kpool0 < k0):
        return None
    dev = x.device
    i32 = dict(dtype=torch.int32, device=dev)
    out = dict(v1=torch.empty(B, N1, 3, dtype=torch.float32, device=dev), v2=torch.empty(B, N2, 3, dtype=torch.float32, device=dev),
               idx0=torch.empty(B, N0, k0, **i32), idx0_pool=torch.empty(B, N0, kpool0, **i32),
               idx1=torch.empty(B, N1, k1, **i32), idx1_pool=torch.empty(B, N1, kpool, **i32), idx2=torch.empty(B, N2, k2, **i32),
               up1=torch.empty(B, N0, **i32), up2=torch.empty(B, N0, **i32))
    wsb = lib().hsp_geometry_all_workspace_bytes(B, N0)
    ws = _ws(wsb, dev)
    _run("hsp_geometry_all_f32", (_p(x), B, N0, k0, kpool0, _p(s1), N1, _p(s2), N2, k1, kpool, k2, 1, _p(out["idx0"]), _p(out["idx0_pool"]),
                                  _p(out["v1"]), _p(out["v2"]), _p(out["idx1"]), _p(out["idx1_pool"]), _p(out["idx2"]), _p(out["up1"]),
                                  _p(out["up2"]), _p(ws), wsb, _stream()),
         key=f"B{B}N{N0}/{N1}/{N2}k{k0}", abytes=B * (12 * N0 + 4 * (N0 * (k0 + kpool0) + N1 * (k1 + kpool + 3) + N2 * (k2 + 3)) + 8 * N0))
    return out


def geometry_levels(xyz, sel1, sel2, k1, kpool, k2):
    x = _req(xyz.detach(), torch.float32, "geometry_levels.xyz")
    s1, s2 = _req(sel1, torch.int32, "geometry_levels.sel1"), _req(sel2, torch.int32, "geometry_levels.sel2")
    B, N0, C = x.shape
    N1, N2 = s1.numel(), s2.numel()
    if C != 3 or not (64 <= N2 <= N1 <= 576) or N1 > N0 or k1 + 2 > 33 or k2 + 2 > 33 or k1 + 1 > N1 or k2 + 1 > N2 or not 0 < kpool <= k1:
        return None
    dev = x.device
# ... 46 lines not shown
    if _ext_state is None:
        from . import _ext
        try:
            _ext_state = bool(_ext.available()) and _ext.ext() is not None
        except _ext.HspExtError:
            _ext_state = False
    return _ext_state


def center_cloud(points):
    pts = _req(points.detach(), torch.float32, "center_cloud.points")
    if _timer is None and _ext_ok():
        from ._ext import ext
        return ext().center_cloud(pts)
    B, N, _ = pts.shape
    out = torch.empty_like(pts)
    mean = torch.empty(B, 1, 3, dtype=torch.float32, device=pts.device)
    _run("hsp_center_cloud_f32", (_p(pts), B, N, _p(out), _p(mean), _stream()), key=f"B{B}N{N}", abytes=24 * B * N)
    return out, mean


def nn1(target, source):
    t = _req(target.detach(), torch.float32, "nn1.target")
    s = _req(source.detach(), torch.float32, "nn1.source")
    B, Nt, C = t.shape
    if C != 3 or s.shape[2] != 3 or s.shape[0] != B:
        raise HspError("nn1: expects (B,Nt,3) and (B,Ns,3)")
    idx = torch.empty(B, Nt, dtype=torch.int32, device=t.device)
    _run("hsp_nn1_f32", (_p(t), Nt, _p(s), s.shape[1], B, _p(idx), _stream()),
         key=f"B{B}Nt{Nt}Ns{s.shape[1]}", abytes=B * (16 * Nt + 12 * s.shape[1]))
    return idx


def rev_index(idx, k, n_src):
    cache = getattr(idx, "_hsp_rev", None)
    if cache is None:
        cache = {}
        idx._hsp_rev = cache
    hit = cache.get((k, n_src))
    if hit is not None:
        return hit
    if idx.dim() == 2:
        (B, Nq), kstride = idx.shape, 1
    else:
        B, Nq, kstride = idx.shape
    off = torch.empty(B, n_src + 1, dtype=torch.int32, device=idx.device)
    edge = torch.empty(B, Nq * k, dtype=torch.int32, device=idx.device)
    _run("hsp_rev_build", (_p(idx), B, Nq, n_src, k, kstride, _p(off), _p(edge), _stream()),
         key=f"B{B}Nq{Nq}k{k}", abytes=B * (8 * Nq * k + 4 * n_src))
    cache[(k, n_src)] = (off, edge)
    return off, edge



class _RFSurface(torch.autograd.Function):
    @staticmethod
    def forward(ctx, xyz, idx, dirs_n, S):
        xyz = _req(xyz, torch.float32, "rf_surface.xyz")
        idx = _req(idx, torch.int32, "rf_surface.idx")
        dirs_n = _req(dirs_n, torch.float32, "rf_surface.dirs")
        B, N, k = idx.shape
        SC = dirs_n.shape[1]
        K = SC // S
        out = torch.empty(B, N, K, dtype=torch.float32, device=xyz.device)
        arg = torch.empty(B, N, SC, dtype=torch.uint16, device=xyz.device)
        _run("hsp_rf_surface_fwd", (_p(xyz), _p(idx), _p(dirs_n), B, N, k, S, K, _p(out), _p(arg), _stream()),
             key=f"B{B}N{N}k{k}S{S}C{K}", abytes=B * N * (12 + 4 * k + 4 * K + SC) + 12 * SC)
        ctx.save_for_backward(xyz, idx, dirs_n, arg)
        ctx.S = S
        return out

    @staticmethod
    def backward(ctx, g):
        xyz, idx, dirs_n, arg = ctx.saved_tensors
        g = _req(g, torch.float32, "rf_surface.grad")
        B, N, k = idx.shape
        SC = dirs_n.shape[1]
        gd = torch.empty_like(dirs_n)
        L = lib()
        wsb = L.hsp_rf_bwd_scatter_workspace_bytes(B, SC)
        ws = _ws(wsb, g.device)
        _rf_bwd_dirs_call("hsp_rf_surface_bwd", "", (_p(xyz), _p(dirs_n), _p(arg), _p(g), B, N, ctx.S, SC // ctx.S, _p(gd)), ws, wsb,
                          (dirs_n, gd), key=f"B{B}N{N}S{ctx.S}C{SC // ctx.S}", abytes=B * N * (12 + 4 * (SC // ctx.S) + SC) + 24 * SC)
        return None, None, gd, None


class _RFConv(torch.autograd.Function):
    @staticmethod
    def forward(ctx, xyz, idx, dirs_n, fm, S):
        xyz = _req(xyz, torch.float32, "rf_conv.xyz")
        idx = _req(idx, torch.int32, "rf_conv.idx")
        dirs_n = _req(dirs_n, torch.float32, "rf_conv.dirs")
        fm = _req(fm, torch.float32, "rf_conv.fm")
        B, N, k = idx.shape
        SC = dirs_n.shape[1]
        C = SC // S
        if fm.shape[-1] != (S + 1) * C:
            raise HspError("rf_conv: fm must have (S+1)*C columns")
        out = torch.empty(B, N, C, dtype=torch.float32, device=xyz.device)
        out, arg, fwin = _rf_conv_fwd_raw(xyz, idx, dirs_n, fm, S, any(ctx.needs_input_grad))
        ctx.save_for_backward(xyz, idx, dirs_n, fwin if fwin is not None else fm, arg)
        ctx.S = S
        return out

    @staticmethod
    def backward(ctx, g):
# ... 257 lines not shown
    sfx = "bf16" if A2.dtype == torch.bfloat16 else "f32"
    es = 2 if A2.dtype == torch.bfloat16 else 4
    batch = WgradBatch.current
    sf = StepFolds.current
    sink = batch.items if batch is not None else sf.wgrads if sf is not None and sf.bare_wgrad else None
    if sink is not None:
        from ._lib import HspWgradPending
        pend = HspWgradPending()
        _run(f"{entry}_partial_{sfx}", (_p(A2), A2.stride(0), _p(B2), B2.stride(0), M, N, K, _p(out), out.stride(0), _p(cs),
                                        _p(ws), wsb, ctypes.byref(pend), _stream()),
             key=f"M{M}N{N}K{K}", abytes=es * K * (M + N) + 4 * M * N, aflops=2 * M * N * K)
        sink.append((pend, ws, _hold(out), _hold(cs)))
    else:
        _run(f"{entry}_{sfx}", (_p(A2), A2.stride(0), _p(B2), B2.stride(0), M, N, K, _p(out), out.stride(0), _p(cs),
                                _p(ws), wsb, _stream()),
             key=f"M{M}N{N}K{K}", abytes=es * K * (M + N) + 4 * M * N, aflops=2 * M * N * K)
    return (out, cs) if colsum else out


def wgrad(A2, B2, out=None, colsum=False):
    K, M = A2.shape
    N = B2.shape[1]
    if out is None:
        out = torch.empty(M, N, dtype=torch.float32, device=A2.device)
    bf16 = A2.dtype == torch.bfloat16
    if _wgrad_ragged_ok(A2, B2, out):
        return _wgrad_custom(A2, B2, out, colsum, entry="hsp_wgrad_ragged" if bf16 else "hsp_wgrad")
    if _wgrad_ok(A2, B2, out):
        return _wgrad_custom(A2, B2, out, colsum)
    if bf16:
        raise HspError("bf16 weight gradient: channel counts must be multiples of 64")
    return _wgrad_fallback(A2, B2, out, colsum)


def _wgrad_ragged_ok(A2, B2, out):
    K, M = A2.shape
    N = B2.shape[1]
    if A2.dtype == torch.bfloat16:
        return (M % 64 != 0 and N % 128 == 0 and A2.stride(1) == 1 and B2.stride(1) == 1 and A2.stride(0) % 8 == 0
                and B2.stride(0) % 8 == 0)
    return (M % 64 != 0 and M >= 128 and N % 128 == 0
            and -(-M // 128) * (N // 128) >= 4 and A2.dtype == torch.float32 and B2.dtype == torch.float32 and A2.is_cuda
            and A2.stride(1) == 1 and B2.stride(1) == 1 and out.stride(1) == 1 and A2.stride(0) % 4 == 0 and B2.stride(0) % 4 == 0
            and A2.stride(0) >= (M + 3) // 4 * 4 and A2.data_ptr() % 16 == 0 and B2.data_ptr() % 16 == 0)


def _wgrad_ok(A2, B2, out):
    K, M = A2.shape
    N = B2.shape[1]
    return (M % 64 == 0 and N % 64 == 0 and A2.stride(1) == 1 and B2.stride(1) == 1 and out.stride(1) == 1
            and A2.stride(0) % 2 == 0 and B2.stride(0) % 2 == 0 and A2.dtype in _FEAT_DTYPES and A2.is_cuda)


def wgrad_pair(A0, B0, out0, A1, B1, out1):
    batch = WgradBatch.current
    if batch is None or A0.dtype != torch.float32 or not _wgrad_ok(A0, B0, out0) or not _wgrad_ok(A1, B1, out1):
        wgrad(A0, B0, out=out0)
        wgrad(A1, B1, out=out1)
        return
    from ._lib import HspWgradPending
    L = lib()
    (K0, M0), N0 = A0.shape, B0.shape[1]
    (K1, M1), N1 = A1.shape, B1.shape[1]
    wsb0, wsb1 = L.hsp_wgrad_workspace_bytes(M0, N0, K0), L.hsp_wgrad_workspace_bytes(M1, N1, K1)
    ws0, ws1 = _ws(wsb0, A0.device), _ws(wsb1, A0.device)
    pend = (HspWgradPending * 2)()
    _run("hsp_wgrad_partial_pair_f32", (_p(A0), A0.stride(0), _p(B0), B0.stride(0), M0, N0, K0, _p(out0), out0.stride(0), _p(ws0), wsb0,
                                        _p(A1), A1.stride(0), _p(B1), B1.stride(0), M1, N1, K1, _p(out1), out1.stride(0), _p(ws1), wsb1,
                                        pend, _stream()),
         key=f"M{M0}N{N0}K{K0}+M{M1}N{N1}K{K1}", abytes=4 * (K0 * (M0 + N0) + M0 * N0 + K1 * (M1 + N1) + M1 * N1),
         aflops=2 * (M0 * N0 * K0 + M1 * N1 * K1))
    batch.items.append((HspWgradPending.from_buffer_copy(pend[0]), ws0, _hold(out0)))
    batch.items.append((HspWgradPending.from_buffer_copy(pend[1]), ws1, _hold(out1)))


def _ld(t):
    if t.dim() != 2 or t.stride(1) != 1:
        raise HspError("gemm_rows: operands must be 2-D with contiguous rows (stride(1) == 1)")
    return t.stride(0) if t.shape[0] > 1 else max(t.stride(0), t.shape[1])


def gemm_rows(A1, B1, nn1=False, A2=None, B2=None, nn2=False, bias=None, resid=None, cloud_bias=None, rows_per_cloud=0,
              out=None, alpha=1.0, xyz3=None, w3=None):
    dt = A1.dtype
    if dt not in (torch.float32, torch.bfloat16):
        raise HspError(f"gemm_rows: fp32 or bf16 operands, got {dt}")
    for t_, nm in ((A1, "A1"), (B1, "B1"), (A2, "A2"), (B2, "B2"), (resid, "resid")):
        if t_ is not None and (not t_.is_cuda or t_.dtype != dt):
            raise HspError(f"gemm_rows.{nm}: expected a {dt} GPU tensor")
    if out is not None and (not out.is_cuda or out.dtype not in (dt, torch.float32)):
        raise HspError(f"gemm_rows.out: expected a {dt} (or, for bf16 operands, fp32) GPU tensor")
    M, K1 = A1.shape
    N = B1.shape[1] if nn1 else B1.shape[0]
    if (B1.shape[0] if nn1 else B1.shape[1]) != K1:
        raise HspError("gemm_rows: A1 / B1 inner dimensions differ")
    K2 = 0
    if A2 is not None:
        K2 = A2.shape[1]
        if A2.shape[0] != M or (B2.shape[1] if nn2 else B2.shape[0]) != N or (B2.shape[0] if nn2 else B2.shape[1]) != K2:
            raise HspError("gemm_rows: second source has the wrong shape")
    if out is None:
        out = torch.empty(M, N, dtype=dt, device=A1.device)
    for t_ in (bias, cloud_bias, xyz3, w3):
        if t_ is not None and (t_.dtype != torch.float32 or not t_.is_cuda or not t_.is_contiguous()):
            raise HspError("gemm_rows: bias / cloud_bias / xyz3 / w3 must be contiguous fp32 GPU tensors")
    if (xyz3 is None) != (w3 is None) or (xyz3 is not None and (xyz3.shape != (M, 3) or w3.shape != (N, 3))):
        raise HspError("gemm_rows: xyz3 (M,3) and w3 (N,3) go together")
    flops = 2 * M * N * (K1 + K2)
    es = 4 if dt == torch.float32 else 2
    ab = es * (M * (K1 + K2) + N * (K1 + K2) + M * N * (2 if resid is not None else 1))
    key = f"M{M}N{N}K{K1}" + (f"+{K2}" if K2 else "")
    wsb = lib().hsp_gemm_rows_workspace_bytes(M, N, K1, K2, es)
    ws = _ws(wsb, A1.device) if wsb else None
    if dt == torch.float32:
        _run("hsp_gemm_rows_f32", (_p(A1), _ld(A1), _p(B1), _ld(B1), 1 if nn1 else 0, K1,
                                   _p(A2), _ld(A2) if A2 is not None else 0, _p(B2), _ld(B2) if B2 is not None else 0,
                                   1 if nn2 else 0, K2, M, N, _p(bias), _p(resid), _ld(resid) if resid is not None else 0,
                                   _p(cloud_bias), int(rows_per_cloud), float(alpha), _p(xyz3), _p(w3), _p(out), _ld(out),
                                   _p(ws), wsb, _stream()),
             key=key, abytes=ab, aflops=flops)
    else:
        if nn1 or nn2:
            raise HspError("gemm_rows: bf16 operands must be (N,K) (pass the transposed copy)")
        _run("hsp_gemm_rows_bf16", (_p(A1), _ld(A1), _p(B1), _ld(B1), K1,
                                    _p(A2), _ld(A2) if A2 is not None else 0, _p(B2), _ld(B2) if B2 is not None else 0, K2,
                                    M, N, _p(bias), _p(resid), _ld(resid) if resid is not None else 0, _p(cloud_bias),
# ... 340 lines not shown
    return out


def _orl_fwd_raw(F3, idx_x, k):
    B, N, C = F3.shape
    fg = torch.empty(B, C, dtype=torch.float32, device=F3.device)
    arg = torch.empty(B, N, C, dtype=torch.uint8, device=F3.device)
    L = lib()
    wsb = L.hsp_orl_workspace_bytes(B, N, C)
    ws = _ws(wsb, F3.device)
    _run("hsp_orl_global_fwd" + _sfx(F3), (_p(F3), _p(idx_x), B, N, k, idx_x.shape[2], C, _p(fg), _p(arg), _p(ws), wsb, _stream()),
         key=f"B{B}N{N}k{k}C{C}", abytes=B * N * (_es(F3) * C + 4 * k + C))
    return fg, arg


def _residual_bias(out3, f3, t2):
    B, N, C = out3.shape
    _run("hsp_residual_bias", (_p(out3), _p(f3), _p(t2.contiguous()), B, N, C, _stream()), key=f"B{B}N{N}C{C}",
         abytes=12 * B * N * C)


def colsum_rows(x3):
    B, N, C = x3.shape
    if x3.dtype == torch.float32 and (((C % 4 or 256 % (C // 4)) and C > 256) or not x3.is_contiguous()):
        return x3.sum(dim=1)
    out = torch.empty(B, C, dtype=torch.float32, device=x3.device)
    L = lib()
    wsb = L.hsp_orl_workspace_bytes(B, N, C)
    ws = _ws(wsb, x3.device)
    _run("hsp_colsum_rows" + _sfx(x3), (_p(x3), B, N, C, _p(out), _p(ws), wsb, _stream()), key=f"B{B}N{N}C{C}",
         abytes=_es(x3) * B * N * C)
    return out


def colsum_rows_xyz(g, xyz):
    B, N, C = g.shape
    mom = torch.empty(B, 4 * C, dtype=torch.float32, device=g.device)
    wsb = 4 * lib().hsp_orl_workspace_bytes(B, N, C)
    ws = _ws(wsb, g.device)
    _run("hsp_colsum_rows_xyz" + _sfx(g), (_p(g), _p(xyz), B, N, C, _p(mom), _p(ws), wsb, _stream()), key=f"B{B}N{N}C{C}",
         abytes=B * N * (_es(g) * C + 12))
    return mom


LAUNCH_DIET = True
_between_launches_hook = None


def _orl_bwd_small_ok(B, N, C, with_xyz):
    return (LAUNCH_DIET and B <= 64 and C % 128 == 0 and C <= 2048
            and lib().hsp_colsum_cloud_ok(B, N, C, 1 if with_xyz else 0) == 1)


def _orl_bwd_small(g, xyz, fg, Wb, gWb, gste=None):
    B, N, C = g.shape
    ns = 4 if xyz is not None else 1
    mom = torch.empty(B, ns * C, dtype=torch.float32, device=g.device)
    _run("hsp_colsum_cloud_f32", (_p(g), _p(xyz), B, N, C, _p(mom), _stream()), key=f"B{B}N{N}C{C}{'x' if xyz is not None else ''}",
         abytes=B * N * (4 * C + (12 if xyz is not None else 0)))
    if _between_launches_hook is not None:
        _between_launches_hook(mom)
    gfg = torch.empty(B, C, dtype=torch.float32, device=g.device)
    _run("hsp_small_pair_f32", (_p(mom), _ld(mom), B, C, _p(Wb), _ld(Wb), Wb.shape[1], 1.0 / N, _p(gfg), _ld(gfg),
                                _p(fg), _ld(fg), fg.shape[1], _p(gWb), _ld(gWb),
                                _p(mom[:, C:]) if xyz is not None else None, _ld(mom) if xyz is not None else 0,
                                C if xyz is not None else 0, _p(gste), _stream()),
         key=f"B{B}C{C}", abytes=4 * (B * 3 * C + 2 * C * C))
    return gfg


def _orl_bwd_accumulate_raw(gfg_over_n, idx_x, arg, k, gF3, extra=None):
    B, N, C = gF3.shape
    if DETERMINISTIC and gF3.dtype == torch.float32:
        tmp = torch.empty_like(gF3)
        off, edge = rev_index(idx_x, k, N)
        _run("hsp_gather_max_bwd_csr", (_p(gfg_over_n), 1, _p(arg), _p(off), _p(edge), B, N, N, k, C, _p(tmp), _stream()),
             key=f"B{B}Ns{N}Nq{N}k{k}C{C}bc", abytes=B * N * (4 * C + 8 * k + C))
        gF3.add_(tmp)
        if extra is not None:
            gF3.add_(extra)
    else:
        _run("hsp_gather_max_bwd" + _sfx(gF3), (_p(gfg_over_n), 1, _p(idx_x), _vp(0), _p(arg), B, N, N, N, idx_x.shape[2], C,
                                                _p(gF3), 1, _p(extra), _stream()),
             key=f"B{B}Ns{N}Nq{N}C{C}bc+", abytes=B * N * (3 * _es(gF3) * C + 4 * idx_x.shape[2] + C))


def _rf_conv_fwd_raw(xyz, idx, directions, fm, S, need_bwd=True):
    B, N, k = idx.shape
    SC = directions.shape[1]
    C = SC // S
    sfx, es = _sfx(fm), _es(fm)
    out = torch.empty(B, N, C, dtype=fm.dtype, device=xyz.device)
    arg = torch.empty(B, N, SC, dtype=torch.uint16, device=xyz.device)
    want = need_bwd and (sfx or not DETERMINISTIC) and getattr(lib(), "hsp_rf_conv_wants_fwin" + sfx)(N, S, C)
    fwin = torch.empty(B, N, SC, dtype=fm.dtype, device=xyz.device) if want else None
    key = f"B{B}N{N}k{k}S{S}C{C}"
    stream = B * N * (12 + 4 * k + es * (S + 1) * C + es * C + 2 * SC + (es * SC if fwin is not None else 0)) + 12 * SC
    if sfx:
        ab = stream
    else:
        design_stream_bytes[("hsp_rf_conv_fwd", key)] = stream
        ab = B * N * (12 + 4 * k + 4 * (S + 1) * C + 4 * C + SC) + 12 * SC
    _run("hsp_rf_conv_fwd" + sfx, (_p(xyz), _p(idx), _p(directions), _p(fm), B, N, k, S, C, _p(out), _p(arg), _p(fwin), _stream()),
         key=key, abytes=ab)
    return out, arg, fwin


def _rf_conv_bwd_raw(xyz, idx, directions, fm, arg, gF3, S):
    B, N, _ = gF3.shape
    SC = directions.shape[1]
    C = SC // S
    sfx, es = _sfx(gF3), _es(gF3)
# ... 93 lines not shown
    def forward(ctx, xyz, X, idx_f, idx_x, k, S, weights, bias, directions, w_ste3, w_conv23, bn_shift=None, out_f32=False):
        w_ste, w_conv2 = w_ste3.squeeze(-1), w_conv23.squeeze(-1)
        xyz = _req(xyz, torch.float32, "hs_layer.xyz")
        X = _reqf(X, "hs_layer.X")
        idx_f = _req(idx_f, torch.int32, "hs_layer.idx_f")
        idx_x = _req(idx_x, torch.int32, "hs_layer.idx_x")
        directions = _req(directions, torch.float32, "hs_layer.directions")
        B, N, Cin = X.shape
        SC = directions.shape[1]
        C = SC // S
        X2 = X.view(B * N, Cin)
        exact = _exact and bn_shift is None and _exact_layer_ok(N, Cin, C, (X2, weights, w_ste, w_conv2))
        fm = gemm_wave(X2, weights, True, bias=bias) if exact else _fm_rows(X2, weights, bias)
        need_bwd = any(ctx.needs_input_grad)
        F3, arg, fwin = _rf_conv_fwd_raw(xyz, idx_f, directions, fm.view(B, N, -1), S, need_bwd)
        if fwin is not None:
            fm = fwin
        fm = fm.view(B, N, -1)
        F2 = F3.view(B * N, C)
        out3 = torch.empty(B, N, C, dtype=torch.float32 if out_f32 else X.dtype, device=X.device)
        if exact:
            fg, arg_o = _orl_fwd_exact(F3, idx_x, k)
            _layer_out_exact(F2, w_conv2, fg, N, out3, ste=gemm_wave(X2, w_ste, False))
            part = None
        else:
            fg, arg_o = _orl_fwd_raw(F3, idx_x, k)
            t2 = _mm_nt(fg, w_conv2[:, C:])
            part = _layer_out_rows(X2, w_ste, F2, w_conv2, t2, out3, bn_shift=bn_shift)
        ctx.save_for_backward(xyz, X, idx_f, idx_x, fm, arg, F3, arg_o, fg, weights, directions, w_ste3, w_conv23)
        ctx.k, ctx.S, ctx.x3 = k, S, x3_planes
        if bn_shift is not None:
            if part is None:
                part = torch.empty(0, dtype=torch.float32, device=out3.device)
            ctx.mark_non_differentiable(part)
            ctx.set_materialize_grads(False)
            return out3, part
        return out3

    @staticmethod
    def backward(ctx, g, _gpart=None):
        xyz, X, idx_f, idx_x, fm, arg, F3, arg_o, fg, weights, directions, w_ste3, w_conv23 = ctx.saved_tensors
        w_ste, w_conv2 = w_ste3.squeeze(-1), w_conv23.squeeze(-1)
        k, S = ctx.k, ctx.S
        f32 = X.dtype == torch.float32
        if not f32 and g.dtype == torch.float32:
            g = g.bfloat16()
        g = _reqf(g, "hs_layer.grad", like=X)
        B, N, Cin = X.shape
        C = F3.shape[2]
        g2, X2, F2 = g.view(B * N, C), X.view(B * N, Cin), F3.view(B * N, C)
        Wb = w_conv2[:, C:]
        small = f32 and _orl_bwd_small_ok(B, N, C, False)
        g_conv2 = torch.empty_like(w_conv2)
        if small:
            gfg_n = _orl_bwd_small(g, None, fg, Wb, g_conv2[:, C:])
        else:
            gt = colsum_rows(g)
        with WgradBatch(), x3_scope(ctx.x3):
            g_ste = torch.empty(C, Cin, dtype=torch.float32, device=g.device)
            wgrad_pair(g2, F2, g_conv2[:, :C], g2, X2, g_ste)
            if not small:
                _tiny_tn(gt, fg, g_conv2[:, C:])
            gF3 = torch.empty(B, N, C, dtype=g.dtype, device=g.device)
            _mm_nn(g2, w_conv2, out=gF3.view(B * N, C), cols=slice(0, C))
            if not small:
                gfg_n = _mm_nn(gt, Wb, alpha=1.0 / N)
            _orl_bwd_accumulate_raw(gfg_n, idx_x, arg_o, k, gF3, extra=g)
            gfm, gD = _rf_conv_bwd_raw(xyz, idx_f, directions, fm.view(B, N, -1), arg, gF3, S)
            gfm2 = gfm.view(B * N, -1)
            gW, gb = wgrad(X2, gfm2, colsum=True)
            gX3 = torch.empty(B, N, Cin, dtype=g.dtype, device=g.device)
            _grad_in_rows(g2, w_ste, gfm2, weights, gX3.view(B * N, Cin))
        return None, gX3, None, None, None, None, gW, gb, gD, g_ste.unsqueeze_(-1), g_conv2.unsqueeze_(-1), None, None


class _SurfaceLayer(torch.autograd.Function):

    @staticmethod
    def forward(ctx, xyz, idx_x, k, S, directions, w_ste3, w_conv23, relu=False, out_dtype=torch.float32):
        w_ste, w_conv2 = w_ste3.squeeze(-1), w_conv23.squeeze(-1)
        xyz = _req(xyz, torch.float32, "surface_layer.xyz")
        idx_x = _req(idx_x, torch.int32, "surface_layer.idx")
        directions = _req(directions, torch.float32, "surface_layer.directions")
        B, N, _ = xyz.shape
        SC = directions.shape[1]
        C = SC // S
        if idx_x.shape[2] != k:
            raise HspError("surface_layer: idx must have exactly k columns")
        F3 = torch.empty(B, N, C, dtype=out_dtype, device=xyz.device)
        arg = torch.empty(B, N, SC, dtype=torch.uint16, device=xyz.device)
        slot = 1 if out_dtype == torch.float32 else 2
        _run("hsp_rf_surface_fwd" + _sfx(F3), (_p(xyz), _p(idx_x), _p(directions), B, N, k, S, C, _p(F3), _p(arg), _stream()),
             key=f"B{B}N{N}k{k}S{S}C{C}", abytes=B * N * (12 + 4 * k + _es(F3) * C + slot * SC) + 12 * SC)
        F2, x2 = F3.view(B * N, C), xyz.view(B * N, 3)
        out3 = torch.empty(B, N, C, dtype=out_dtype, device=xyz.device)
        if _exact and _exact_layer_ok(N, 3, C, (w_conv2, F2)):
            fg, arg_o = _orl_fwd_exact(F3, idx_x, k)
            _layer_out_exact(F2, w_conv2, fg, N, out3, xyz3=x2, w3=w_ste.contiguous(), relu=relu)
        else:
            fg, arg_o = _orl_fwd_raw(F3, idx_x, k)
            t2 = _mm_nt(fg, w_conv2[:, C:])
            _layer_out_rows(x2, w_ste, F2, w_conv2, t2, out3, relu=relu)
        ctx.k, ctx.S, ctx.relu, ctx.x3 = k, S, relu, x3_planes
        if relu:
            ctx.save_for_backward(xyz, idx_x, arg, F3, arg_o, fg, directions, w_conv23, out3)
            ctx.set_materialize_grads(False)
            return out3, out3.view_as(out3)
        ctx.save_for_backward(xyz, idx_x, arg, F3, arg_o, fg, directions, w_conv23)
        return out3

    @staticmethod
    def backward(ctx, *gs):
        if ctx.relu:
# ... 470 lines not shown
            from ._ext import ext
            y = ext().bn_eval(x, bn.running_mean, bn.running_var, _eval_invstd(bn), bn.weight, bn.bias, bn.eps, relu)
            return (y, y.view_as(y)) if fork else y
        y = _BNEval.apply(x, bn.weight, bn.bias, bn.running_mean, bn.running_var, _eval_invstd(bn), bn.eps, relu)
        return (y, y.view_as(y)) if fork else y
    if not fused:
        y = bn(x.reshape(-1, C)).view_as(x)
        y = torch.relu_(y) if relu else y
        return (y, y) if fork else y
    return _BNRelu.apply(x, bn.weight, bn.bias, bn.running_mean, bn.running_var, bn.num_batches_tracked, bn.eps,
                         bn.momentum, relu, out_dtype, fork, partial)



class _GatherRows(torch.autograd.Function):
    @staticmethod
    def forward(ctx, feat, idx):
        feat = _req(feat, torch.float32, "gather_rows.feat")
        idx = _req(idx, torch.int32, "gather_rows.idx")
        B, Nsrc, C = feat.shape
        shared = 1 if idx.dim() == 1 else 0
        Nq = idx.shape[-1]
        out = torch.empty(B, Nq, C, dtype=torch.float32, device=feat.device)
        _run("hsp_gather_rows_fwd", (_p(feat), _p(idx), shared, B, Nsrc, Nq, C, _p(out), C, _stream()),
             key=f"B{B}Ns{Nsrc}Nq{Nq}C{C}", abytes=B * (4 * Nsrc * C + Nq * (4 + 4 * C)))
        ctx.save_for_backward(idx)
        ctx.dims = (B, Nsrc, Nq, C, shared)
        return out

    @staticmethod
    def backward(ctx, g):
        (idx,) = ctx.saved_tensors
        B, Nsrc, Nq, C, shared = ctx.dims
        if not (g.is_cuda and g.dtype == torch.float32):
            raise HspError("gather_rows.grad: expected a float32 GPU tensor")
        if g.stride(2) == 1 and g.stride(0) == Nq * g.stride(1) and g.stride(1) >= C:
            gstride = g.stride(1)
        else:
            g = g.contiguous()
            gstride = C
        gfeat = torch.empty(B, Nsrc, C, dtype=torch.float32, device=g.device)
        _run("hsp_gather_rows_bwd", (_p(g), gstride, _p(idx), shared, B, Nsrc, Nq, C, _p(gfeat), _stream()),
             key=f"B{B}Ns{Nsrc}Nq{Nq}C{C}", abytes=B * (4 * Nsrc * C + Nq * (4 + 4 * C)))
        return gfeat, None


def gather_rows(feat, idx):
    return _GatherRows.apply(feat, idx)



ONE_HOT_WIDTH = 6

FEAT_PITCH_ALIGN = 8


class _AssembleFeat(torch.autograd.Function):

    @staticmethod
    def forward(ctx, kinds, idxs, *tensors):
        B, N, dt = None, None, None
        for t, kd in zip(tensors, kinds):
            if kd == 0:
                B, N, dt = t.shape[0], t.shape[1], t.dtype
        tensors = [(_req(t, torch.float32, "assemble_feat.src") if kd >= 2 or dt == torch.float32 else
                    _req(t, dt, "assemble_feat.src")) for t, kd in zip(tensors, kinds)]
        idxs = [(_req(i, torch.int32, "assemble_feat.idx") if i is not None else None) for i in idxs]
        n = len(tensors)
        widths = [(t.shape[-1] if kd != 3 else ONE_HOT_WIDTH) for t, kd in zip(tensors, kinds)]
        for t, kd in zip(tensors, kinds):
            if kd == 3 and t.numel() != B:
                raise HspError("assemble_feat: a kind-3 segment is one float id per cloud")
        W = sum(widths)
        P = (W + FEAT_PITCH_ALIGN - 1) // FEAT_PITCH_ALIGN * FEAT_PITCH_ALIGN if FEAT_PITCH_ALIGN > 1 else W
        full = torch.empty(B, N, P, dtype=dt, device=tensors[0].device)
        out = full[:, :, :W] if P != W else full
        src = (ctypes.c_void_p * n)(*[t.data_ptr() for t in tensors])
        ix = (ctypes.c_void_p * n)(*[(i.data_ptr() if i is not None else 0) for i in idxs])
        wd = (ctypes.c_int * n)(*widths)
        kd = (ctypes.c_int * n)(*kinds)
        ns = (ctypes.c_int * n)(*[(t.shape[1] if k_ == 1 else 0) for t, k_ in zip(tensors, kinds)])
        es = 2 if dt == torch.bfloat16 else 4
        if dt == torch.bfloat16:
            _run("hsp_concat_rows_bf16", (n, ctypes.cast(src, _vp), ctypes.cast(ix, _vp), ctypes.cast(wd, _vp),
                                          ctypes.cast(kd, _vp), ctypes.cast(ns, _vp), B, N, _p(full), P, _stream()),
                 key=f"B{B}N{N}W{W}", abytes=2 * es * B * N * W)
        else:
            _run("hsp_concat_rows_pitched", (n, ctypes.cast(src, _vp), ctypes.cast(ix, _vp), ctypes.cast(wd, _vp),
                                             ctypes.cast(kd, _vp), ctypes.cast(ns, _vp), B, N, _p(full), P, _stream()),
                 key=f"B{B}N{N}W{W}", abytes=2 * es * B * N * W)
        ctx.kinds, ctx.widths = kinds, widths
        ctx.nsrc = [(t.shape[1] if t.dim() > 1 else 0) for t in tensors]
        ctx.save_for_backward(*[i for i in idxs if i is not None])
        ctx.has_idx = [i is not None for i in idxs]
        return out

    @staticmethod
    def backward(ctx, g):
        if not g.is_contiguous():
            g = g.contiguous()
        B, N, W = g.shape
        saved = list(ctx.saved_tensors)
        grads, col = [], 0
        for s_, (kd, w) in enumerate(zip(ctx.kinds, ctx.widths)):
            gs = g[:, :, col:col + w]
            if not ctx.needs_input_grad[2 + s_]:
                grads.append(None)
                if ctx.has_idx[s_]:
                    saved.pop(0)
            elif kd == 0:
                grads.append(gs)
            elif kd == 1:
                idx = saved.pop(0)
                Ns = ctx.nsrc[s_]
                gfeat = torch.empty(B, Ns, w, dtype=g.dtype, device=g.device)
                es = _es(g)
                if w % 2 == 0 and W % 2 == 0 and (w // 2 >= 256 or 256 % (w // 2) == 0) and gs.data_ptr() % (2 * es) == 0:
                    off, edge = rev_index(idx, 1, Ns)
                    _run("hsp_gather_rows_bwd_csr" + _sfx(g), (_p(gs), W, _p(off), _p(edge), B, Ns, N, w, _p(gfeat), _stream()),
                         key=f"B{B}Ns{Ns}Nq{N}C{w}", abytes=B * (es * Ns * w + N * (4 + es * w)))
                elif g.dtype == torch.bfloat16:
                    raise HspError("assemble_feat backward: bf16 segments must be even-width and 4-byte aligned")
                else:
                    _run("hsp_gather_rows_bwd", (_p(gs), W, _p(idx), 0, B, Ns, N, w, _p(gfeat), _stream()),
                         key=f"B{B}Ns{Ns}Nq{N}C{w}", abytes=B * (4 * Ns * w + N * (4 + 4 * w)))
                grads.append(gfeat)
            elif kd == 3:
                grads.append(None)
            else:
                grads.append(gs.sum(dim=1))
            col += w
        return (None, None, *grads)


def assemble_feat(segments):
    tensors = [s_[0] for s_ in segments]
    idxs = [s_[1] for s_ in segments]
    kinds = [s_[2] for s_ in segments]
    return _AssembleFeat.apply(kinds, idxs, *tensors)



class _Chamfer(torch.autograd.Function):
    @staticmethod
    def forward(ctx, xyz1, xyz2):
        xyz1 = _req(xyz1, torch.float32, "chamfer.xyz1")
        xyz2 = _req(xyz2, torch.float32, "chamfer.xyz2")
        B, n, _ = xyz1.shape
        m = xyz2.shape[1]
        d1 = torch.empty(B, n, dtype=torch.float32, device=xyz1.device)
        d2 = torch.empty(B, m, dtype=torch.float32, device=xyz1.device)
        i1 = torch.empty(B, n, dtype=torch.int32, device=xyz1.device)
        i2 = torch.empty(B, m, dtype=torch.int32, device=xyz1.device)
        _run("hsp_chamfer_fwd", (_p(xyz1), _p(xyz2), B, n, m, _p(d1), _p(d2), _p(i1), _p(i2), _stream()),
             key=f"B{B}n{n}m{m}", abytes=B * (n + m) * 20)
        ctx.save_for_backward(xyz1, xyz2, i1, i2)
        ctx.mark_non_differentiable(i1, i2)
        return d1, d2, i1, i2

    @staticmethod
    def backward(ctx, g1, g2, _gi1, _gi2):
        xyz1, xyz2, i1, i2 = ctx.saved_tensors
        B, n, _ = xyz1.shape
        m = xyz2.shape[1]
        g1 = _req(g1 if g1 is not None else torch.zeros(B, n, device=xyz1.device), torch.float32, "chamfer.g1")
        g2 = _req(g2 if g2 is not None else torch.zeros(B, m, device=xyz1.device), torch.float32, "chamfer.g2")
        gx1 = torch.empty_like(xyz1)
        gx2 = torch.empty_like(xyz2)
        _run("hsp_chamfer_bwd", (_p(xyz1), _p(xyz2), _p(i1), _p(i2), _p(g1), _p(g2), B, n, m, _p(gx1), _p(gx2),
                                 _stream()), key=f"B{B}n{n}m{m}", abytes=B * (n + m) * 32)
# ... 85 lines not shown
```

include/hsp.h:

```cpp
#ifndef HSP_H_
#define HSP_H_

#include <stddef.h>
#include <stdint.h>

#ifdef __cplusplus
extern "C" {
#endif

#define HSP_OK 0
#define HSP_ERR_BAD_ARG (-1)
#define HSP_ERR_UNSUPPORTED (-2)
#define HSP_ERR_WORKSPACE (-3)
#define HSP_ERR_LAUNCH (-4)

#define HSP_MAX_K 32

typedef void *hspStream_t;
typedef uint16_t hsp_bf16_t;

int hsp_version(void);
const char *hsp_error_string(int code);
const char *hsp_last_hip_error(void);

size_t hsp_knn_workspace_bytes(int B, int N, int C, int k);
int hsp_knn_f32(const float *x, int B, int N, int C, int k, int drop_first, int32_t *idx,
                void *ws, size_t ws_bytes, hspStream_t stream);
size_t hsp_knn_exact_workspace_bytes(int B, int N, int C, int k, int drop_first);
int hsp_knn_exact_f32(const float *x, int B, int N, int C, int k, int drop_first, int quad_mode, int32_t *idx, void *ws,
                      size_t ws_bytes, int *tie_rows, hspStream_t stream);
size_t hsp_knn_xyz_workspace_bytes(int B, int N);
int hsp_knn_xyz_f32(const float *xyz, int B, int N, int k, int k2, int drop_first, int32_t *idx, int32_t *idx2, void *ws,
                    size_t ws_bytes, int *tie_rows, hspStream_t stream);
int hsp_geometry_levels_f32(const float *xyz, int B, int N0, const int32_t *sel1, int N1, const int32_t *sel2, int N2, int k1,
                            int kpool, int k2, int drop_first, float *v1, float *v2, int32_t *idx1, int32_t *idx1_pool,
                            int32_t *idx2, int32_t *up1, int32_t *up2, hspStream_t stream);
size_t hsp_geometry_all_workspace_bytes(int B, int N0);
int hsp_geometry_all_f32(const float *xyz, int B, int N0, int k0, int kpool0, const int32_t *sel1, int N1, const int32_t *sel2, int N2,
                         int k1, int kpool, int k2, int drop_first, int32_t *idx0, int32_t *idx0_pool, float *v1, float *v2,
                         int32_t *idx1, int32_t *idx1_pool, int32_t *idx2, int32_t *up1, int32_t *up2, void *ws, size_t ws_bytes,
                         hspStream_t stream);
int hsp_knn_quadmode_f32(const float *x, int B, int N, int C, int k, int drop_first, int32_t *idx, void *ws, size_t ws_bytes,
                         int quad_mode, hspStream_t stream);
int hsp_quad_outer_f32(const float *x, int B, int N, int C, float *quad, hspStream_t stream);
int hsp_center_cloud_f32(const float *pts, int B, int N, float *centred, float *mean, hspStream_t stream);

int hsp_nn1_f32(const float *tgt, int Nt, const float *src, int Ns, int B, int32_t *idx,
                hspStream_t stream);

int hsp_rf_surface_fwd(const float *xyz, const int32_t *idx, const float *dirs, int B, int N, int k,
                       int S, int K, float *out, uint16_t *argrow, hspStream_t stream);
size_t hsp_rf_bwd_scatter_workspace_bytes(int B, int SC);
int hsp_rf_surface_bwd(const float *xyz, const float *dirs, const uint16_t *argrow, const float *grad_out,
                       int B, int N, int S, int K, float *grad_dirs, void *ws, size_t ws_bytes,
                       hspStream_t stream);

int hsp_rf_conv_wants_fwin(int N, int S, int C);
int hsp_rf_conv_fwd(const float *xyz, const int32_t *idx, const float *dirs, const float *fm, int B,
                    int N, int k, int S, int C, float *out, uint16_t *argrow, float *fwin,
                    hspStream_t stream);
int hsp_rf_conv_bwd_scatter(const float *xyz, const float *dirs, const float *fm, const float *fwin,
                            const uint16_t *argrow,
                            const float *grad_out, int B, int N, int S, int C, float *grad_fm,
                            float *grad_dirs, void *ws, size_t ws_bytes, hspStream_t stream);
size_t hsp_rf_bwd_workspace_bytes(int SC);
int hsp_rf_conv_bwd(const float *xyz, const float *dirs, const float *fm, const uint16_t *argrow,
                    const float *grad_out, const int32_t *rev_off, const int32_t *rev_edge, int B, int N,
                    int k, int S, int C, float *grad_fm, float *grad_dirs, void *ws, size_t ws_bytes,
                    hspStream_t stream);

int hsp_rev_build(const int32_t *idx, int B, int Nq, int Nsrc, int k, int kstride, int32_t *rev_off,
                  int32_t *rev_edge, hspStream_t stream);

int hsp_gather_max_fwd(const float *feat, const int32_t *idx, const int32_t *qsel, int B, int Nsrc,
                       int Nidx, int Nq, int k, int kstride, int C, float *out, uint8_t *argmax,
                       hspStream_t stream);
int hsp_pool_fwd(const float *feat, const float *xyz, const int32_t *idx, const int32_t *qsel, int B, int N, int Nq, int k,
                 int kstride, int C, float *out, uint8_t *argmax, float *xyz_sel, hspStream_t stream);
int hsp_gather_max_bwd(const float *grad_out, int grad_bcast, const int32_t *idx, const int32_t *qsel,
                       const uint8_t *argmax, int B, int Nsrc, int Nidx, int Nq, int kstride, int C,
                       float *grad_feat, int accumulate ,
                       const float *extra ,
                       hspStream_t stream);
int hsp_gather_max_bwd_csr(const float *grad_out, int grad_bcast, const uint8_t *argmax, const int32_t *rev_off,
                           const int32_t *rev_edge, int B, int Nsrc, int Nq, int k, int C, float *grad_feat,
                           hspStream_t stream);

int hsp_points_max_fwd(const float *x, int B, int N, int C, float *out, int32_t *argrow, hspStream_t stream);
int hsp_points_max_bwd(const float *grad_out, const int32_t *argrow, int B, int N, int C, float *grad_x,
                       hspStream_t stream);

size_t hsp_orl_workspace_bytes(int B, int N, int C);
int hsp_orl_global_fwd(const float *feat, const int32_t *idx, int B, int N, int k, int kstride, int C,
                       float *fg, uint8_t *argmax, void *ws, size_t ws_bytes, hspStream_t stream);
size_t hsp_orl_exact_workspace_bytes(int B, int N, int C);
int hsp_orl_global_exact_f32(const float *feat, const int32_t *idx, int B, int N, int k, int kstride, int C, float *fg,
                             uint8_t *argmax, void *ws, size_t ws_bytes, hspStream_t stream);
int hsp_bn_eval_f32(const float *x, long long R, int C, const float *running_mean, const float *running_var,
                    const float *invstd, const float *weight, const float *bias, float eps, int relu, float *y,
                    hspStream_t stream);
int hsp_layer_out_exact_f32(const float *F, int ldf, const float *Wa, int ldwa, const float *fg, int ldfg, const float *Wb,
                            int ldwb, const float *cloud_t, int two_chain, const float *ste, int ldste, const float *xyz3,
                            const float *w3, int relu, int M, int C, int rows_per_cloud, float *out, int ldo,
                            hspStream_t stream);
int hsp_colsum_rows(const float *x, int B, int N, int C, float *out, void *ws, size_t ws_bytes,
                    hspStream_t stream);

int hsp_add_relu_bwd(const float *ga, int lda, const float *gb, int ldb, const float *y, int R, int C, float *out,
                     hspStream_t stream);
int hsp_residual_bias(float *out, const float *f, const float *t, int B, int N, int C, hspStream_t stream);

int hsp_concat_rows(int nseg, const float *const *src, const int32_t *const *idx, const int *width,
                    const int *kind, const int *nsrc, int B, int N, float *out, hspStream_t stream);

int hsp_gather_rows_fwd(const float *feat, const int32_t *idx, int idx_shared, int B, int Nsrc, int Nq,
                        int C, float *out, int out_stride, hspStream_t stream);
int hsp_gather_rows_bwd(const float *grad_out, int grad_stride, const int32_t *idx, int idx_shared, int B,
                        int Nsrc, int Nq, int C, float *grad_feat, hspStream_t stream);
int hsp_gather_rows_bwd_csr(const float *grad_out, int grad_stride, const int32_t *rev_off, const int32_t *rev_edge,
                            int B, int Nsrc, int Nq, int C, float *grad_feat, hspStream_t stream);

int hsp_gemm_rows_f32(const float *A1, int lda1, const float *B1, int ldb1, int b1_layout, int K1,
                      const float *A2, int lda2, const float *B2, int ldb2, int b2_layout, int K2, int M, int N,
                      const float *bias, const float *resid, int ldr, const float *cloud_bias, int rows_per_cloud,
                      float alpha, const float *xyz3, const float *w3, float *C, int ldc, void *ws, size_t ws_bytes,
                      hspStream_t stream);
size_t hsp_gemm_rows_workspace_bytes(int M, int N, int K1, int K2, int elem_bytes);
int hsp_gemm_rows_bf16(const hsp_bf16_t *A1, int lda1, const hsp_bf16_t *B1, int ldb1, int K1,
                       const hsp_bf16_t *A2, int lda2, const hsp_bf16_t *B2, int ldb2, int K2, int M, int N,
                       const float *bias, const hsp_bf16_t *resid, int ldr, const float *cloud_bias,
                       int rows_per_cloud, float alpha, const float *xyz3, const float *w3, void *C, int ldc,
                       int c_is_f32 ,
                       void *ws, size_t ws_bytes, hspStream_t stream);

int hsp_gemm_wave_supported(int M, int N, int K1, int K2, int cfg);
int hsp_gemm_wave_plan_info(int M, int N, int K1, int K2, int cfg, int *out);
int hsp_gemm_wave_f32(const float *A1, int lda1, const float *B1, int ldb1, int b1_layout, int K1,
                      const float *A2, int lda2, const float *B2, int ldb2, int b2_layout, int K2, int M, int N,
                      const float *bias, const float *resid, int ldr, const float *cloud_bias, int rows_per_cloud,
                      float alpha, const float *xyz3, const float *w3, float *C, int ldc, int cfg, hspStream_t stream);

typedef struct HspSplitDesc { const float *src; void *dst; int rows, cols, ld, transpose, kp, tile0; long long ps; } HspSplitDesc;
int hsp_split_params_x3(const HspSplitDesc *table_dev, int n, int total_tiles, hspStream_t stream);
int hsp_gemm_x3_supported(int M, int N, int K1, int K2);
size_t hsp_gemm_x3_workspace_bytes(int M, int N, int K1, int K2);
int hsp_gemm_x3_f32(const float *A1, int lda1, const hsp_bf16_t *P1, int ldp1, long long ps1, int K1,
                    const float *A2, int lda2, const hsp_bf16_t *P2, int ldp2, long long ps2, int K2, int M, int N,
                    const float *bias, const float *resid, int ldr, const float *cloud_bias, int rows_per_cloud,
                    float alpha, float *C, int ldc, void *ws, size_t ws_bytes, hspStream_t stream);
int hsp_gemm_x3_bn_f32(const float *A1, int lda1, const hsp_bf16_t *P1, int ldp1, long long ps1, int K1,
                       const float *A2, int lda2, const hsp_bf16_t *P2, int ldp2, long long ps2, int K2, int M, int N,
                       const float *resid, int ldr, const float *cloud_bias, int rows_per_cloud, float *C, int ldc,
                       float *bn_shift, float *bn_part, hspStream_t stream);
int hsp_gemm_x3_bn_tiles(int M, int N);
int hsp_gemm_x3_bias_bn_f32(const float *A1, int lda1, const hsp_bf16_t *P1, int ldp1, long long ps1, int K1, int M, int N,
                            const float *bias, float *C, int ldc, float *bn_shift, float *bn_part, hspStream_t stream);

int hsp_small_rows_f32(const float *A, int lda, const float *W, int ldw, int w_layout, int M, int N, int K, float alpha,
                       float *out, int ldo, hspStream_t stream);
int hsp_small_outer_f32(const float *a, int lda, const float *c, int ldc, int B, int Ma, int Nb, float *out, int ldo,
                        const float *mom, int ldm, int Cm, float *gste, hspStream_t stream);
int hsp_colsum_rows_xyz(const float *x, const float *xyz, int B, int N, int C, float *out4, void *ws, size_t ws_bytes,
                        hspStream_t stream);
int hsp_colsum_rows_xyz_bf16(const hsp_bf16_t *x, const float *xyz, int B, int N, int C, float *out4, void *ws, size_t ws_bytes,
                             hspStream_t stream);

int hsp_colsum_cloud_ok(int B, int N, int C, int with_xyz);
int hsp_colsum_cloud_f32(const float *x, const float *xyz, int B, int N, int C, float *out, hspStream_t stream);
int hsp_small_pair_f32(const float *gt, int ldgt, int B, int Ma, const float *W, int ldw, int Nn, float alpha, float *out_nn,
                       int ldnn, const float *c, int ldc, int Nb, float *out_o, int ldo, const float *mom, int ldm, int Cm,
                       float *gste, hspStream_t stream);

typedef struct HspCastDesc { const float *src; void *dst; void *dstT; int rows, cols, ld, tile0; } HspCastDesc;
int hsp_cast_params_bf16(const HspCastDesc *table_dev, int n, int total_tiles, hspStream_t stream);
typedef struct HspCastPitchedDesc {
    const float *src; void *dst; void *dstT; int rows, cols, ld, tile0, ldd, lddT;
} HspCastPitchedDesc;
int hsp_cast_params_pitched_bf16(const HspCastPitchedDesc *table_dev, int n, int total_tiles, hspStream_t stream);

size_t hsp_wgrad_workspace_bytes(int M, int N, int K);
#define HSP_FOLD_MAX_WGRAD 24
#define HSP_FOLD_MAX_DIRS 8
typedef struct HspWgradPending {
    const void *part, *cs_part;
    void *C, *colsum;
    int nparts, M, N, ldc;
} HspWgradPending;
int hsp_wgrad_fold(const HspWgradPending *pending, int n, hspStream_t stream);
typedef struct HspDirsPending {
    const void *part, *dirs;
    void *grad_dirs;
    int nparts, SC;
} HspDirsPending;
int hsp_step_fold(const HspWgradPending *wgrads, int nw, const HspDirsPending *dirs, int nd, hspStream_t stream);
int hsp_rf_surface_bwd_partial(const float *xyz, const float *dirs, const uint16_t *argrow, const float *grad_out, int B, int N,
                               int S, int K, float *grad_dirs, void *ws, size_t ws_bytes, HspDirsPending *pending,
                               hspStream_t stream);
int hsp_rf_conv_bwd_scatter_partial(const float *xyz, const float *dirs, const float *fm, const float *fwin,
                                    const uint16_t *argrow, const float *grad_out, int B, int N, int S, int C, float *grad_fm,
                                    float *grad_dirs, void *ws, size_t ws_bytes, HspDirsPending *pending, hspStream_t stream);
int hsp_rf_surface_bwd_partial_bf16(const float *xyz, const float *dirs, const uint16_t *argrow, const hsp_bf16_t *grad_out,
                                    int B, int N, int S, int K, float *grad_dirs, void *ws, size_t ws_bytes,
                                    HspDirsPending *pending, hspStream_t stream);
int hsp_rf_conv_bwd_scatter_partial_bf16(const float *xyz, const float *dirs, const hsp_bf16_t *fm, const hsp_bf16_t *fwin,
                                         const uint16_t *argrow, const hsp_bf16_t *grad_out, int B, int N, int S, int C,
                                         hsp_bf16_t *grad_fm, float *grad_dirs, void *ws, size_t ws_bytes,
                                         HspDirsPending *pending, hspStream_t stream);
int hsp_wgrad_partial_pair_f32(const float *A0, int lda0, const float *B0, int ldb0, int M0, int N0, int K0, float *C0, int ldc0,
                               void *ws0, size_t ws_bytes0, const float *A1, int lda1, const float *B1, int ldb1, int M1, int N1,
                               int K1, float *C1, int ldc1, void *ws1, size_t ws_bytes1, HspWgradPending *pending,
                               hspStream_t stream);
int hsp_wgrad_f32(const float *A, int lda, const float *B, int ldb, int M, int N, int K, float *C, int ldc,
                  float *colsum_B, void *ws, size_t ws_bytes, hspStream_t stream);
int hsp_wgrad_partial_f32(const float *A, int lda, const float *B, int ldb, int M, int N, int K, float *C, int ldc,
                          float *colsum_B, void *ws, size_t ws_bytes, HspWgradPending *pending, hspStream_t stream);

size_t hsp_bn_workspace_bytes(int R, int C);
int hsp_bn_relu_fwd(const float *x, int R, int C, const float *gamma, const float *beta, float eps,
                    float momentum, int relu, float *y, float *save_mean, float *save_invstd,
                    float *running_mean, float *running_var, long long *num_batches_tracked, void *ws,
                    size_t ws_bytes, hspStream_t stream);
int hsp_bn_relu_apply(const float *x, int R, int C, const float *mean, const float *invstd,
                      const float *gamma, const float *beta, int relu, float *y, hspStream_t stream);
int hsp_bn_relu_bwd(const float *x, const float *dy, int R, int C, const float *gamma, const float *beta,
                    const float *save_mean, const float *save_invstd, int relu, float *dx, float *dgamma,
                    float *dbeta, void *ws, size_t ws_bytes, hspStream_t stream);
int hsp_bn_relu_fwd_partials(const float *x, int R, int C, const float *gamma, const float *beta, float eps, float momentum,
                             int relu, float *y, float *save_mean, float *save_invstd, float *running_mean, float *running_var,
                             long long *num_batches_tracked, const float *partial, int nblk, const float *shift,
                             hspStream_t stream);
int hsp_bn_relu_bwd2(const float *x, const float *dy, int ldy, const float *dy2, int ldy2, int R, int C, const float *gamma,
                     const float *beta, const float *save_mean, const float *save_invstd, int relu, float *dx, float *dgamma,
                     float *dbeta, void *ws, size_t ws_bytes, hspStream_t stream);

size_t hsp_pc_compact_workspace_bytes(int B, int HW);
int hsp_pc_compact(const float *mask, const float *depth, int B, int HW, int32_t *pix, int32_t *count,
                   void *ws, size_t ws_bytes, hspStream_t stream);
int hsp_pc_gather(const float *depth, const float *coor2d, const float *camK, const int32_t *pix,
                  const int32_t *choose, int B, int HW, int S, float *pc, hspStream_t stream);

int hsp_depth_to_pcl(const float *depth, const float *xymap, const double *camK, const int32_t *pix,
                     const int32_t *choose, int B, int HW, int S, float *pc, hspStream_t stream);

int hsp_generate_rt(const float *p_green, const float *p_red, const float *f_green, const float *f_red,
                    const float *T, const float *sym, int sym_stride, int B, float *out, hspStream_t stream);

typedef struct HspRowDesc { long long offset; int len; int gc; } HspRowDesc;
size_t hsp_sumsq_workspace_bytes(long long n);
int hsp_sumsq_f32(const float *x, long long n, float *out, void *ws, size_t ws_bytes, hspStream_t stream);
int hsp_ranger_step(float *params, const float *grads, float *exp_avg, float *exp_avg_sq, float *slow,
                    const HspRowDesc *rows, int nrows, float beta1, float beta2, float eps, float weight_decay,
                    float step_lr, int adaptive, int lookahead, float la_alpha, int gc_after,
                    const float *gnorm_sq, float max_norm, hspStream_t stream);

int hsp_chamfer_fwd(const float *xyz1, const float *xyz2, int B, int n, int m, float *dist1, float *dist2,
                    int32_t *idx1, int32_t *idx2, hspStream_t stream);
int hsp_chamfer_bwd(const float *xyz1, const float *xyz2, const int32_t *idx1, const int32_t *idx2,
                    const float *gd1, const float *gd2, int B, int n, int m, float *gx1, float *gx2,
                    hspStream_t stream);

size_t hsp_fps_workspace_bytes(int B, int N);
int hsp_fps_f32(const float *xyz, int B, int N, int n_samples, int32_t *sel, void *ws, size_t ws_bytes,
                hspStream_t stream);
int hsp_fps_f64(const double *xyz, int B, int N, int n_samples, int32_t *sel, void *ws, size_t ws_bytes,
                hspStream_t stream);

int hsp_knn_bf16(const hsp_bf16_t *x, int B, int N, int C, int k, int drop_first, int32_t *idx, void *ws,
                 size_t ws_bytes, hspStream_t stream);
int hsp_rf_surface_fwd_bf16(const float *xyz, const int32_t *idx, const float *dirs, int B, int N, int k, int S, int K,
                            hsp_bf16_t *out, uint16_t *argrow, hspStream_t stream);
int hsp_rf_surface_bwd_bf16(const float *xyz, const float *dirs, const uint16_t *argrow, const hsp_bf16_t *grad_out, int B,
                            int N, int S, int K, float *grad_dirs, void *ws, size_t ws_bytes, hspStream_t stream);
int hsp_rf_conv_wants_fwin_bf16(int N, int S, int C);
int hsp_rf_conv_fwd_bf16(const float *xyz, const int32_t *idx, const float *dirs, const hsp_bf16_t *fm, int B, int N, int k,
                         int S, int C, hsp_bf16_t *out, uint16_t *argrow, hsp_bf16_t *fwin, hspStream_t stream);
int hsp_rf_conv_bwd_scatter_bf16(const float *xyz, const float *dirs, const hsp_bf16_t *fm, const hsp_bf16_t *fwin,
                                 const uint16_t *argrow, const hsp_bf16_t *grad_out, int B, int N, int S, int C,
                                 hsp_bf16_t *grad_fm, float *grad_dirs, void *ws, size_t ws_bytes, hspStream_t stream);
int hsp_gather_max_fwd_bf16(const hsp_bf16_t *feat, const int32_t *idx, const int32_t *qsel, int B, int Nsrc, int Nidx,
                            int Nq, int k, int kstride, int C, hsp_bf16_t *out, uint8_t *argmax, hspStream_t stream);
int hsp_gather_max_bwd_bf16(const void *grad_out, int grad_bcast, const int32_t *idx, const int32_t *qsel,
                            const uint8_t *argmax, int B, int Nsrc, int Nidx, int Nq, int kstride, int C,
                            hsp_bf16_t *grad_feat, int accumulate, const hsp_bf16_t *extra, hspStream_t stream);
int hsp_orl_global_fwd_bf16(const hsp_bf16_t *feat, const int32_t *idx, int B, int N, int k, int kstride, int C, float *fg,
                            uint8_t *argmax, void *ws, size_t ws_bytes, hspStream_t stream);
int hsp_colsum_rows_bf16(const hsp_bf16_t *x, int B, int N, int C, float *out, void *ws, size_t ws_bytes,
                         hspStream_t stream);
int hsp_concat_rows_pitched(int nseg, const float *const *src, const int32_t *const *idx, const int *width, const int *kind,
                            const int *nsrc, int B, int N, float *out, int out_pitch, hspStream_t stream);
int hsp_concat_rows_bf16(int nseg, const void *const *src, const int32_t *const *idx, const int *width, const int *kind,
                         const int *nsrc, int B, int N, hsp_bf16_t *out, int out_pitch, hspStream_t stream);
int hsp_gather_rows_bwd_csr_bf16(const hsp_bf16_t *grad_out, int grad_stride, const int32_t *rev_off,
                                 const int32_t *rev_edge, int B, int Nsrc, int Nq, int C, hsp_bf16_t *grad_feat,
                                 hspStream_t stream);
int hsp_wgrad_bf16(const hsp_bf16_t *A, int lda, const hsp_bf16_t *B, int ldb, int M, int N, int K, float *C, int ldc,
                   float *colsum_B, void *ws, size_t ws_bytes, hspStream_t stream);
int hsp_wgrad_partial_bf16(const hsp_bf16_t *A, int lda, const hsp_bf16_t *B, int ldb, int M, int N, int K, float *C, int ldc,
                           float *colsum_B, void *ws, size_t ws_bytes, HspWgradPending *pending, hspStream_t stream);
int hsp_wgrad_ragged_bf16(const hsp_bf16_t *A, int lda, const hsp_bf16_t *B, int ldb, int M, int N, int K, float *C, int ldc,
                          float *colsum_B, void *ws, size_t ws_bytes, hspStream_t stream);
int hsp_wgrad_ragged_partial_bf16(const hsp_bf16_t *A, int lda, const hsp_bf16_t *B, int ldb, int M, int N, int K, float *C,
                                  int ldc, float *colsum_B, void *ws, size_t ws_bytes, HspWgradPending *pending,
                                  hspStream_t stream);
int hsp_gemm_rows_acc_bf16(const hsp_bf16_t *A1, int lda1, const hsp_bf16_t *B1, int ldb1, int K1, const hsp_bf16_t *A2,
                           int lda2, const hsp_bf16_t *B2, int ldb2, int K2, int M, int N, const float *resid, int ldr, void *C,
                           int ldc, int c_is_f32, void *ws, size_t ws_bytes, hspStream_t stream);
int hsp_gemm_rows_bn_tiles_bf16(int M, int N, int K);
int hsp_gemm_rows_bn_bf16(const hsp_bf16_t *A, int lda, const hsp_bf16_t *B, int ldb, int K, int M, int N, const float *bias,
                          const float *cloud_bias, int rows_per_cloud, const float *xyz3, const float *w3, float *C, int ldc,
                          float *bn_shift, float *bn_part, hspStream_t stream);
int hsp_bn_relu_fwd_partials_mixed(const float *x, int R, int C, const float *gamma, const float *beta, float eps, float momentum,
                                   int relu, hsp_bf16_t *y, float *save_mean, float *save_invstd, float *running_mean,
                                   float *running_var, long long *num_batches_tracked, const float *partial, int nblk,
                                   const float *shift, hspStream_t stream);
int hsp_points_max_fwd_bf16(const hsp_bf16_t *x, int B, int N, int C, float *out, int32_t *argrow, hspStream_t stream);
int hsp_points_max_bwd_bf16(const float *grad_out, const int32_t *argrow, int B, int N, int C, hsp_bf16_t *grad_x,
                            hspStream_t stream);
int hsp_bn_relu_fwd_mixed(const float *x, int R, int C, const float *gamma, const float *beta, float eps, float momentum,
                          int relu, hsp_bf16_t *y, float *save_mean, float *save_invstd, float *running_mean,
                          float *running_var, long long *num_batches_tracked, void *ws, size_t ws_bytes, hspStream_t stream);
int hsp_bn_relu_apply_mixed(const float *x, int R, int C, const float *mean, const float *invstd, const float *gamma,
                            const float *beta, int relu, hsp_bf16_t *y, hspStream_t stream);
int hsp_bn_relu_bwd_mixed(const float *x, const hsp_bf16_t *dy, int R, int C, const float *gamma, const float *beta,
                          const float *save_mean, const float *save_invstd, int relu, hsp_bf16_t *dx, float *dgamma,
                          float *dbeta, void *ws, size_t ws_bytes, hspStream_t stream);
int hsp_bn_relu_fwd_bf16(const hsp_bf16_t *x, int R, int C, const float *gamma, const float *beta, float eps, float momentum,
                         int relu, hsp_bf16_t *y, float *save_mean, float *save_invstd, float *running_mean,
                         float *running_var, long long *num_batches_tracked, void *ws, size_t ws_bytes, hspStream_t stream);
int hsp_bn_relu_apply_bf16(const hsp_bf16_t *x, int R, int C, const float *mean, const float *invstd, const float *gamma,
                           const float *beta, int relu, hsp_bf16_t *y, hspStream_t stream);
int hsp_bn_relu_bwd_bf16(const hsp_bf16_t *x, const hsp_bf16_t *dy, int R, int C, const float *gamma, const float *beta,
                         const float *save_mean, const float *save_invstd, int relu, hsp_bf16_t *dx, float *dgamma,
                         float *dbeta, void *ws, size_t ws_bytes, hspStream_t stream);

#define HSP_LOSS_TERMS 19
typedef struct HspLossCfg {
    float rot_1_w, rot_2_w, rot_regular, tran_w, size_w, r_con_w;
    float recon_n_w, recon_d_w, recon_f_w, recon_v_w, recon_bb_r_w, recon_bb_t_w, recon_bb_s_w, recon_bb_self_w;
    float geo_p_w, prop_pm_w, prop_sym_w;
    int smooth_l1;
} HspLossCfg;
size_t hsp_pose_losses_workspace_bytes(int B);
int hsp_pose_losses_fwd(const float *PC, const float *gt_R, const float *gt_t, const float *gt_s, const float *mean_shape,
                        const float *sym, const float *obj_id, const float *recon, const float *face_normal,
                        const float *face_dis, const float *face_f, const float *p_green, const float *p_red,
                        const float *f_green, const float *f_red, const float *pred_T, const float *pred_s, int B, int N,
                        const HspLossCfg *cfg, float *terms, void *ws, size_t ws_bytes, hspStream_t stream);
// ... 27 lines not shown
```

Baseline: 9341 point-clouds/sec.

## Merge CSR reverse-index builds, concat-backward gathers, and colsum into wgrad launches

Adds a multi-map reverse-index builder and a multi-segment CSR gather-rows backward kernel, so the concat backward handles 2–4 indexed segments in one launch each. It also lets the ORL backward's per-cloud column sum run inside the paired wgrad launch, and pulls the colsum body into a shared header with a multi-chunk variant. The aim is fewer small kernel launches and better GPU fill in the backward pass. The cost is extra host-side pointer-table setup and more complex kernels, and the merged launch may take the LDS size of its largest map.

```diff
diff --git a/hs_pose_amd/_lib.py b/hs_pose_amd/_lib.py
--- a/hs_pose_amd/_lib.py
+++ b/hs_pose_amd/_lib.py
@@ -23,6 +23,7 @@
     "hsp_rf_bwd_scatter_workspace_bytes": (_sz, [_i, _i]),
     "hsp_rf_conv_bwd_scatter": (_i, [_vp, _vp, _vp, _vp, _vp, _vp, _i, _i, _i, _i, _vp, _vp, _vp, _sz, _vp]),
     "hsp_rev_build": (_i, [_vp, _i, _i, _i, _i, _i, _vp, _vp, _vp]),
+    "hsp_rev_build_multi": (_i, [_i, _vp, _i, _vp, _vp, _vp, _vp, _vp, _vp, _vp]),
     "hsp_gather_max_bwd_csr": (_i, [_vp, _i, _vp, _vp, _vp, _i, _i, _i, _i, _i, _vp, _vp]),
     "hsp_gather_max_fwd": (_i, [_vp, _vp, _vp, _i, _i, _i, _i, _i, _i, _i, _vp, _vp, _vp]),
     "hsp_pool_fwd": (_i, [_vp, _vp, _vp, _vp, _i, _i, _i, _i, _i, _i, _vp, _vp, _vp, _vp]),
@@ -53,6 +54,8 @@
     "hsp_gather_rows_fwd": (_i, [_vp, _vp, _i, _i, _i, _i, _i, _vp, _i, _vp]),
     "hsp_gather_rows_bwd": (_i, [_vp, _i, _vp, _i, _i, _i, _i, _i, _vp, _vp]),
     "hsp_gather_rows_bwd_csr": (_i, [_vp, _i, _vp, _vp, _i, _i, _i, _i, _vp, _vp]),
+    "hsp_gather_rows_bwd_csr_multi": (_i, [_i, _vp, _i, _vp, _vp, _i, _vp, _i, _vp, _vp, _vp]),
+    "hsp_gather_rows_bwd_csr_multi_bf16": (_i, [_i, _vp, _i, _vp, _vp, _i, _vp, _i, _vp, _vp, _vp]),
     "hsp_gemm_rows_workspace_bytes": (_sz, [_i, _i, _i, _i, _i]),
     "hsp_gemm_rows_f32": (_i, [_vp, _i, _vp, _i, _i, _i, _vp, _i, _vp, _i, _i, _i, _i, _i, _vp, _vp, _i, _vp, _i, ctypes.c_float, _vp, _vp, _vp, _i, _vp, _sz, _vp]),
     "hsp_gemm_rows_bf16": (_i, [_vp, _i, _vp, _i, _i, _vp, _i, _vp, _i, _i, _i, _i, _vp, _vp, _i, _vp, _i, ctypes.c_float, _vp, _vp, _vp, _i, _i, _vp, _sz, _vp]),
@@ -145,6 +148,7 @@
     "hsp_rf_surface_bwd_partial_bf16": (_i, [_vp, _vp, _vp, _vp, _i, _i, _i, _i, _vp, _vp, _sz, _vp, _vp]),
     "hsp_rf_conv_bwd_scatter_partial_bf16": (_i, [_vp, _vp, _vp, _vp, _vp, _vp, _i, _i, _i, _i, _vp, _vp, _vp, _sz, _vp, _vp]),
     "hsp_wgrad_partial_pair_f32": (_i, [_vp, _i, _vp, _i, _i, _i, _i, _vp, _i, _vp, _sz] * 2 + [_vp, _vp]),
+    "hsp_wgrad_partial_pair_colsum_f32": (_i, [_vp, _i, _vp, _i, _i, _i, _i, _vp, _i, _vp, _sz] * 2 + [_vp, _vp, _i, _i, _i, _vp, _vp]),
     "hsp_pose_augment": (_i, [_vp] * 14 + [_i, _i, _i] + [ctypes.c_float] * 4 + [_vp] * 5),
 }
 
diff --git a/hs_pose_amd/csrc/colsum_cloud.h b/hs_pose_amd/csrc/colsum_cloud.h
--- /dev/null
+++ b/hs_pose_amd/csrc/colsum_cloud.h
@@ -0,0 +1,110 @@
+#pragma once
+#include "common.h"
+
+namespace hsp {
+
+__device__ __forceinline__ float chunk_fold8(const float* __restrict__ p, int nchunk, int stride) {
+    float s[8] = {0.f, 0.f, 0.f, 0.f, 0.f, 0.f, 0.f, 0.f};
+    int ch = 0;
+    for (; ch + 7 < nchunk; ch += 8) {
+#pragma unroll
+        for (int u = 0; u < 8; ++u) s[u] += p[(size_t)(ch + u) * stride];
+    }
+    for (; ch < nchunk; ++ch) s[ch & 7] += p[(size_t)ch * stride];
+    return ((s[0] + s[1]) + (s[2] + s[3])) + ((s[4] + s[5]) + (s[6] + s[7]));
+}
+
+__device__ __forceinline__ float fma_plain(float a, float b, float c) {
+    float r;
+    asm volatile("v_fma_f32 %0, %1, %2, %3" : "=v"(r) : "v"(a), "v"(b), "v"(c));
+    return r;
+}
+
+template <bool XYZ, int NT, int R>
+__device__ __forceinline__ void colsum_cloud_body(float4* __restrict__ cc_smem, const int tile, const int b,
+                                                  const float* __restrict__ x, const float* __restrict__ xyz, int N, int C,
+                                                  int nchunk, int rows, float* __restrict__ out) {
+    static_assert(!XYZ || R == 1, "the coordinate moments are summed one chunk at a time");
+    constexpr int NS = XYZ ? 4 : 1;
+    constexpr int CPR = NT / 32;
+    const int cq = C >> 2, RL = 256 / cq, G = cq >> 3;
+    const int tid = threadIdx.x;
+    const int gl = tid % G, rl = (tid / G) % RL, cs = tid / (G * RL);
+    const int g = tile * G + gl;
+    float4* red = cc_smem;
+    float4* cp = cc_smem + R * NT;
+    for (int c0 = 0; c0 < nchunk; c0 += CPR * R) {
+        float4 s[R][NS];
+#pragma unroll
+        for (int u = 0; u < R; ++u)
+#pragma unroll
+            for (int q = 0; q < NS; ++q) s[u][q] = make_float4(0.f, 0.f, 0.f, 0.f);
+        if constexpr (R == 1) {
+            const int chunk = c0 + cs;
+            const int r0 = chunk * rows, r1 = chunk < nchunk ? min(N, r0 + rows) : 0;
+            for (int i = r0 + rl; i < r1; i += RL) {
+                const float4 v = *reinterpret_cast<const float4*>(x + ((size_t)b * N + i) * C + (g << 2));
+                s[0][0].x += v.x; s[0][0].y += v.y; s[0][0].z += v.z; s[0][0].w += v.w;
+                if constexpr (XYZ) {
+                    const float* p3 = xyz + ((size_t)b * N + i) * 3;
+                    const float w[3] = {p3[0], p3[1], p3[2]};
+#pragma unroll
+                    for (int q = 0; q < 3; ++q) {
+                        s[0][q + 1].x = fma_plain(v.x, w[q], s[0][q + 1].x); s[0][q + 1].y = fma_plain(v.y, w[q], s[0][q + 1].y);
+                        s[0][q + 1].z = fma_plain(v.z, w[q], s[0][q + 1].z); s[0][q + 1].w = fma_plain(v.w, w[q], s[0][q + 1].w);
+                    }
+                }
+            }
+        } else {
+            int r0[R], r1[R];
+#pragma unroll
+            for (int u = 0; u < R; ++u) {
+                const int chunk = c0 + u * CPR + cs;
+                r0[u] = chunk * rows + rl;
+                r1[u] = chunk < nchunk ? min(N, chunk * rows + rows) : 0;
+            }
+            for (int j = 0; j < rows; j += 2 * RL) {
+                float4 v[R][2];
+#pragma unroll
+                for (int u = 0; u < R; ++u)
+#pragma unroll
+                    for (int h = 0; h < 2; ++h)
+                        v[u][h] = *reinterpret_cast<const float4*>(x + ((size_t)b * N + min(r0[u] + j + h * RL, N - 1)) * C + (g << 2));
+#pragma unroll
+                for (int u = 0; u < R; ++u)
+#pragma unroll
+                    for (int h = 0; h < 2; ++h)
+                        if (r0[u] + j + h * RL < r1[u]) {
+                            s[u][0].x += v[u][h].x; s[u][0].y += v[u][h].y; s[u][0].z += v[u][h].z; s[u][0].w += v[u][h].w;
+                        }
+            }
+        }
+#pragma unroll
+        for (int q = 0; q < NS; ++q) {
+#pragma unroll
+            for (int u = 0; u < R; ++u) red[u * NT + tid] = s[u][q];
+            __syncthreads();
+#pragma unroll
+            for (int u = 0; u < R; ++u) {
+                const int chunk = c0 + u * CPR + cs;
+                if (rl == 0 && chunk < nchunk) {
+                    float4 a = s[u][q];
+                    for (int l = 1; l < RL; ++l) {
+                        const float4 v = red[u * NT + (cs * RL + l) * G + gl];
+                        a.x += v.x; a.y += v.y; a.z += v.z; a.w += v.w;
+                    }
+                    cp[((size_t)q * nchunk + chunk) * G + gl] = a;
+                }
+            }
+            __syncthreads();
+        }
+    }
+    const int TC = G << 2;
+    if (tid < NS * TC) {
+        const int q = tid / TC, c = tid - q * TC;
+        out[(size_t)b * NS * C + (size_t)q * C + tile * TC + c] =
+            chunk_fold8(reinterpret_cast<const float*>(cp) + (size_t)q * nchunk * TC + c, nchunk, TC);
+    }
+}
+
+}
diff --git a/hs_pose_amd/csrc/common.h b/hs_pose_amd/csrc/common.h
--- a/hs_pose_amd/csrc/common.h
+++ b/hs_pose_amd/csrc/common.h
@@ -29,6 +29,8 @@
                           uint8_t* tie, float* dmat, hspStream_t stream);
 int knn3_select_flags(const float* x, int B, int N, int k, int drop, int k2, int32_t* idx, int32_t* idx2, uint8_t* tie,
                       hipStream_t st, bool* needs_tie_pass);
+
+int colsum_cloud_plan(int B, int N, int C, int* rows, int* nchunk);
 
 inline int persistent_blocks(long long work_items, int blocks_per_cu) {
     long long g = (long long)HSP_NUM_CU * blocks_per_cu;
diff --git a/hs_pose_amd/csrc/csr.hip b/hs_pose_amd/csrc/csr.hip
--- a/hs_pose_amd/csrc/csr.hip
+++ b/hs_pose_amd/csrc/csr.hip
@@ -5,14 +5,13 @@
 #define REV_THREADS 1024
 
 template <bool EDGES_IN_LDS>
-__global__ __launch_bounds__(REV_THREADS) void rev_build_kernel(const int32_t* __restrict__ idx, int Nq, int Nsrc,
-                                                                int k, int kstride, int32_t* __restrict__ rev_off,
-                                                                int32_t* __restrict__ rev_edge) {
+__device__ __forceinline__ void rev_build_body(const int b, const int32_t* __restrict__ idx, int Nq, int Nsrc,
+                                               int k, int kstride, int32_t* __restrict__ rev_off,
+                                               int32_t* __restrict__ rev_edge, int* __restrict__ wsum) {
     extern __shared__ __attribute__((aligned(16))) char smem[];
     int* cnt = reinterpret_cast<int*>(smem);
     int* led = cnt + Nsrc + 1;
-    __shared__ int wsum[REV_THREADS / 64];
-    const int b = blockIdx.x, tid = threadIdx.x, lane = tid & 63, wv = tid >> 6;
+    const int tid = threadIdx.x, lane = tid & 63, wv = tid >> 6;
     const int32_t* ib = idx + (size_t)b * Nq * kstride;
     int32_t* off = rev_off + (size_t)b * (Nsrc + 1);
     int32_t* edge = rev_edge + (size_t)b * Nq * k;
@@ -95,6 +94,23 @@
     }
 }
 
+template <bool EDGES_IN_LDS>
+__global__ __launch_bounds__(REV_THREADS) void rev_build_kernel(const int32_t* __restrict__ idx, int Nq, int Nsrc,
+                                                                int k, int kstride, int32_t* __restrict__ rev_off,
+                                                                int32_t* __restrict__ rev_edge) {
+    __shared__ int wsum[REV_THREADS / 64];
+    rev_build_body<EDGES_IN_LDS>((int)blockIdx.x, idx, Nq, Nsrc, k, kstride, rev_off, rev_edge, wsum);
+}
+
+struct RevBuildMap { const int32_t* idx; int32_t* rev_off; int32_t* rev_edge; int Nq, Nsrc, k, kstride, in_lds; };
+struct RevBuildTab { RevBuildMap m[4]; };
+__global__ __launch_bounds__(REV_THREADS) void rev_build_multi_kernel(const RevBuildTab tab) {
+    __shared__ int wsum[REV_THREADS / 64];
+    const RevBuildMap m = tab.m[blockIdx.y];
+    if (m.in_lds) rev_build_body<true>((int)blockIdx.x, m.idx, m.Nq, m.Nsrc, m.k, m.kstride, m.rev_off, m.rev_edge, wsum);
+    else rev_build_body<false>((int)blockIdx.x, m.idx, m.Nq, m.Nsrc, m.k, m.kstride, m.rev_off, m.rev_edge, wsum);
+}
+
 }
 
 using namespace hsp;
@@ -116,3 +132,27 @@
                        rev_edge);
     return check_launch();
 }
+
+extern "C" int hsp_rev_build_multi(int nmaps, const int32_t* const* idx, int B, const int* Nq, const int* Nsrc, const int* k,
+                                   const int* kstride, int32_t* const* rev_off, int32_t* const* rev_edge, hspStream_t stream) {
+    if (nmaps <= 0 || nmaps > 4 || !idx || !Nq || !Nsrc || !k || !kstride || !rev_off || !rev_edge || B <= 0 || B > 65535)
+        return HSP_ERR_BAD_ARG;
+    RevBuildTab tab;
+    size_t lds = 0;
+    for (int i = 0; i < nmaps; ++i) {
+        if (!idx[i] || !rev_off[i] || !rev_edge[i] || Nq[i] <= 0 || Nsrc[i] <= 0 || k[i] <= 0 || kstride[i] < k[i]) return HSP_ERR_BAD_ARG;
+        const size_t lds0 = (size_t)(Nsrc[i] + 1) * sizeof(int);
+        if (lds0 > 140 * 1024) return HSP_ERR_UNSUPPORTED;
+        const size_t lds1 = lds0 + (size_t)Nq[i] * k[i] * sizeof(int);
+        const bool in_lds = lds1 <= 140 * 1024;
+        lds = lds > (in_lds ? lds1 : lds0) ? lds : (in_lds ? lds1 : lds0);
+        tab.m[i] = RevBuildMap{idx[i], rev_off[i], rev_edge[i], Nq[i], Nsrc[i], k[i], kstride[i], in_lds ? 1 : 0};
+    }
+    if (lds > 60 * 1024) {
+        hipError_t e = hipFuncSetAttribute(reinterpret_cast<const void*>(rev_build_multi_kernel),
+                                           hipFuncAttributeMaxDynamicSharedMemorySize, (int)lds);
+        if (e != hipSuccess) { set_last_hip_error(e); return HSP_ERR_LAUNCH; }
+    }
+    hipLaunchKernelGGL(rev_build_multi_kernel, dim3(B, nmaps), dim3(REV_THREADS), lds, as_stream(stream), tab);
+    return check_launch();
+}
diff --git a/hs_pose_amd/csrc/gather.hip b/hs_pose_amd/csrc/gather.hip
--- a/hs_pose_amd/csrc/gather.hip
+++ b/hs_pose_amd/csrc/gather.hip
@@ -1,4 +1,5 @@
 #include "common.h"
+#include "colsum_cloud.h"
 #include <type_traits>
 
 namespace hsp {
@@ -212,17 +213,6 @@
     ORL_STAMP(31);
 }
 
-__device__ __forceinline__ float chunk_fold8(const float* __restrict__ p, int nchunk, int stride) {
-    float s[8] = {0.f, 0.f, 0.f, 0.f, 0.f, 0.f, 0.f, 0.f};
-    int ch = 0;
-    for (; ch + 7 < nchunk; ch += 8) {
-#pragma unroll
-        for (int u = 0; u < 8; ++u) s[u] += p[(size_t)(ch + u) * stride];
-    }
-    for (; ch < nchunk; ++ch) s[ch & 7] += p[(size_t)ch * stride];
-    return ((s[0] + s[1]) + (s[2] + s[3])) + ((s[4] + s[5]) + (s[6] + s[7]));
-}
-
 __global__ __launch_bounds__(256) void chunk_fold_kernel(const float* __restrict__ part, int B, int nchunk, int C,
                                                          float scale, float* __restrict__ out) {
     const int e = blockIdx.x * 256 + threadIdx.x;
@@ -253,12 +243,6 @@
     }
 }
 
-__device__ __forceinline__ float fma_plain(float a, float b, float c) {
-    float r;
-    asm volatile("v_fma_f32 %0, %1, %2, %3" : "=v"(r) : "v"(a), "v"(b), "v"(c));
-    return r;
-}
-
 template <typename FT>
 __global__ __launch_bounds__(256) void colsum_xyz_partial_kernel(const FT* __restrict__ x, const float* __restrict__ xyz, int N, int C,
                                                                  float* __restrict__ part, int nchunk, int rows) {
@@ -299,50 +283,7 @@
 __global__ __launch_bounds__(1024) void colsum_cloud_kernel(const float* __restrict__ x, const float* __restrict__ xyz, int N, int C,
                                                             int nchunk, int rows, float* __restrict__ out) {
     extern __shared__ float4 cc_smem[];
-    constexpr int NS = XYZ ? 4 : 1;
-    const int cq = C >> 2, RL = 256 / cq, G = cq >> 3;
-    const int tid = threadIdx.x;
-    const int gl = tid % G, rl = (tid / G) % RL, cs = tid / (G * RL);
-    const int g = blockIdx.x * G + gl, b = blockIdx.y;
-    float4* red = cc_smem;
-    float4* cp = cc_smem + 1024;
-    for (int c0 = 0; c0 < nchunk; c0 += 32) {
-        const int chunk = c0 + cs;
-        const int r0 = chunk * rows, r1 = chunk < nchunk ? min(N, r0 + rows) : 0;
-        float4 s[NS];
-#pragma unroll
-        for (int q = 0; q < NS; ++q) s[q] = make_float4(0.f, 0.f, 0.f, 0.f);
-        for (int i = r0 + rl; i < r1; i += RL) {
-            const float4 v = *reinterpret_cast<const float4*>(x + ((size_t)b * N + i) * C + (g << 2));
-            s[0].x += v.x; s[0].y += v.y; s[0].z += v.z; s[0].w += v.w;
-            if constexpr (XYZ) {
-                const float* p3 = xyz + ((size_t)b * N + i) * 3;
-                const float w[3] = {p3[0], p3[1], p3[2]};
-#pragma unroll
-                for (int q = 0; q < 3; ++q) {
-                    s[q + 1].x = fma_plain(v.x, w[q], s[q + 1].x); s[q + 1].y = fma_plain(v.y, w[q], s[q + 1].y);
-                    s[q + 1].z = fma_plain(v.z, w[q], s[q + 1].z); s[q + 1].w = fma_plain(v.w, w[q], s[q + 1].w);
-                }
-            }
-        }
-#pragma unroll
-        for (int q = 0; q < NS; ++q) {
-            red[tid] = s[q];
-            __syncthreads();
-            if (rl == 0 && chunk < nchunk) {
-                float4 a = s[q];
-                for (int l = 1; l < RL; ++l) { const float4 v = red[(cs * RL + l) * G + gl]; a.x += v.x; a.y += v.y; a.z += v.z; a.w += v.w; }
-                cp[((size_t)q * nchunk + chunk) * G + gl] = a;
-            }
-            __syncthreads();
-        }
-    }
-    const int TC = G << 2;
-    if (tid < NS * TC) {
-        const int q = tid / TC, c = tid - q * TC;
-        out[(size_t)b * NS * C + (size_t)q * C + blockIdx.x * TC + c] =
-            chunk_fold8(reinterpret_cast<const float*>(cp) + (size_t)q * nchunk * TC + c, nchunk, TC);
-    }
+    colsum_cloud_body<XYZ, 1024, 1>(cc_smem, (int)blockIdx.x, (int)blockIdx.y, x, xyz, N, C, nchunk, rows, out);
 }
 
 __global__ __launch_bounds__(256) void colsum_partial_scalar_kernel(const float* __restrict__ x, int N, int C,
@@ -916,44 +857,118 @@
     return check_launch();
 }
 
-template <typename FT>
-__global__ __launch_bounds__(256) void gather_rows_bwd_csr_kernel(const FT* __restrict__ gout, int gstride,
-                                                                  const int32_t* __restrict__ rev_off,
-                                                                  const int32_t* __restrict__ rev_edge, int B,
-                                                                  int Nsrc, int Nq, int C,
-                                                                  FT* __restrict__ gfeat) {
-    const int pairs = C >> 1;
-    const int tpr = pairs < 256 ? pairs : 256;
+template <typename FT, int VEC>
+__device__ __forceinline__ void grow_ld(const FT* __restrict__ p, float (&v)[VEC]) {
+    if constexpr (sizeof(FT) == 4 && VEC == 2) {
+        const float2 t = *reinterpret_cast<const float2*>(p);
+        v[0] = t.x; v[1] = t.y;
+    } else if constexpr (sizeof(FT) == 4) {
+        const float4 t = *reinterpret_cast<const float4*>(p);
+        v[0] = t.x; v[1] = t.y; v[2] = t.z; v[3] = t.w;
+    } else if constexpr (VEC == 2) {
+        const unsigned w = *reinterpret_cast<const unsigned*>(p);
+        v[0] = __uint_as_float(w << 16); v[1] = __uint_as_float(w & 0xffff0000u);
+    } else {
+        const uint2 w = *reinterpret_cast<const uint2*>(p);
+        v[0] = __uint_as_float(w.x << 16); v[1] = __uint_as_float(w.x & 0xffff0000u);
+        v[2] = __uint_as_float(w.y << 16); v[3] = __uint_as_float(w.y & 0xffff0000u);
+    }
+}
+template <typename FT, int VEC>
+__device__ __forceinline__ void grow_st(FT* __restrict__ p, const float (&v)[VEC]) {
+    if constexpr (sizeof(FT) == 4 && VEC == 2) {
+        *reinterpret_cast<float2*>(p) = make_float2(v[0], v[1]);
+    } else if constexpr (sizeof(FT) == 4) {
+        *reinterpret_cast<float4*>(p) = make_float4(v[0], v[1], v[2], v[3]);
+    } else if constexpr (VEC == 2) {
+        *reinterpret_cast<unsigned*>(p) = f32_to_bf16_bits(v[0]) | (f32_to_bf16_bits(v[1]) << 16);
+    } else {
+        *reinterpret_cast<uint2*>(p) = make_uint2(f32_to_bf16_bits(v[0]) | (f32_to_bf16_bits(v[1]) << 16),
+                                                  f32_to_bf16_bits(v[2]) | (f32_to_bf16_bits(v[3]) << 16));
+    }
+}
+
+template <typename FT, int VEC>
+__device__ __forceinline__ void gather_rows_bwd_csr_body(const int bid, const FT* __restrict__ gout, int gstride,
+                                                         const int32_t* __restrict__ rev_off,
+                                                         const int32_t* __restrict__ rev_edge, int B, int Nsrc, int Nq, int C,
+                                                         FT* __restrict__ gfeat) {
+    const int cols = C / VEC;
+    const int tpr = cols < 256 ? cols : 256;
     const int RB = 256 / tpr;
     const int rl = threadIdx.x / tpr, t = threadIdx.x - rl * tpr;
-    const long long row = (long long)blockIdx.x * RB + rl;
+    const long long row = (long long)bid * RB + rl;
     if (rl >= RB || row >= (long long)B * Nsrc) return;
     const int m = (int)(row % Nsrc), b = (int)(row / Nsrc);
     const int32_t* off = rev_off + (size_t)b * (Nsrc + 1);
     const int32_t* edge = rev_edge + (size_t)b * Nq;
     const int o0 = off[m], o1 = off[m + 1];
     const FT* gb = gout + (size_t)b * Nq * gstride;
-    for (int p = t; p < pairs; p += tpr) {
-        float2 acc = make_float2(0.f, 0.f);
-        for (int e = o0; e < o1; e += 4) {
-            float2 v[4];
-#pragma unroll
-            for (int u = 0; u < 4; ++u) {
-                const int q = edge[min(e + u, o1 - 1)];
-                if constexpr (sizeof(FT) == 4) {
-                    v[u] = *reinterpret_cast<const float2*>(gb + (size_t)q * gstride + 2 * p);
-                } else {
-                    const unsigned w = *reinterpret_cast<const unsigned*>(gb + (size_t)q * gstride + 2 * p);
-                    v[u] = make_float2(__uint_as_float(w << 16), __uint_as_float(w & 0xffff0000u));
+    for (int p = t; p < cols; p += tpr) {
+        float acc[VEC];
+#pragma unroll
+        for (int c = 0; c < VEC; ++c) acc[c] = 0.f;
+        int e = o0;
+        for (; e + 8 <= o1; e += 8) {
+            float v[8][VEC];
+#pragma unroll
+            for (int u = 0; u < 8; ++u) grow_ld<FT, VEC>(gb + (size_t)edge[e + u] * gstride + VEC * p, v[u]);
+#pragma unroll
+            for (int u = 0; u < 8; ++u)
+#pragma unroll
+                for (int c = 0; c < VEC; ++c) acc[c] += v[u][c];
+        }
+        for (; e < o1; e += 4) {
+            float v[4][VEC];
+#pragma unroll
+            for (int u = 0; u < 4; ++u) grow_ld<FT, VEC>(gb + (size_t)edge[min(e + u, o1 - 1)] * gstride + VEC * p, v[u]);
+#pragma unroll
+            for (int u = 0; u < 4; ++u)
+                if (e + u < o1) {
+#pragma unroll
+                    for (int c = 0; c < VEC; ++c) acc[c] += v[u][c];
                 }
-            }
-#pragma unroll
-            for (int u = 0; u < 4; ++u)
-                if (e + u < o1) { acc.x += v[u].x; acc.y += v[u].y; }
-        }
-        if constexpr (sizeof(FT) == 4) *reinterpret_cast<float2*>(gfeat + (size_t)row * C + 2 * p) = acc;
-        else *reinterpret_cast<unsigned*>(gfeat + (size_t)row * C + 2 * p) = f32_to_bf16_bits(acc.x) | (f32_to_bf16_bits(acc.y) << 16);
-    }
+        }
+        grow_st<FT, VEC>(gfeat + (size_t)row * C + VEC * p, acc);
+    }
+}
+
+template <typename FT>
+__global__ __launch_bounds__(256) void gather_rows_bwd_csr_kernel(const FT* __restrict__ gout, int gstride,
+                                                                  const int32_t* __restrict__ rev_off,
+                                                                  const int32_t* __restrict__ rev_edge, int B,
+                                                                  int Nsrc, int Nq, int C,
+                                                                  FT* __restrict__ gfeat) {
+    gather_rows_bwd_csr_body<FT, 2>((int)blockIdx.x, gout, gstride, rev_off, rev_edge, B, Nsrc, Nq, C, gfeat);
+}
+
+struct GatherBwdSeg {
+    const void* gout; const int32_t* rev_off; const int32_t* rev_edge; void* gfeat;
+    int gstride, nsrc, nq, width, vec;
+};
+struct GatherBwdDesc { GatherBwdSeg seg[4]; int first[5]; int nseg; };
+
+template <typename FT>
+__global__ __launch_bounds__(256) void gather_rows_bwd_csr_multi_kernel(const GatherBwdDesc d, int B) {
+    const int bid = (int)blockIdx.x;
+    int s = 0;
+    while (s + 1 < d.nseg && bid >= d.first[s + 1]) ++s;
+    const GatherBwdSeg sg = d.seg[s];
+    const FT* gout = reinterpret_cast<const FT*>(sg.gout);
+    FT* gfeat = reinterpret_cast<FT*>(sg.gfeat);
+    if (sg.vec == 4)
+        gather_rows_bwd_csr_body<FT, 4>(bid - d.first[s], gout, sg.gstride, sg.rev_off, sg.rev_edge, B, sg.nsrc, sg.nq, sg.width, gfeat);
+    else
+        gather_rows_bwd_csr_body<FT, 2>(bid - d.first[s], gout, sg.gstride, sg.rev_off, sg.rev_edge, B, sg.nsrc, sg.nq, sg.width, gfeat);
+}
+
+template <typename FT>
+static bool gather_bwd_csr_vec_ok(int VEC, const FT* grad_out, int grad_stride, int C, const FT* grad_feat) {
+    if ((C % VEC) || (grad_stride % VEC)) return false;
+    const size_t al = (size_t)VEC * sizeof(FT) - 1;
+    if ((reinterpret_cast<uintptr_t>(grad_out) & al) || (VEC > 2 && (reinterpret_cast<uintptr_t>(grad_feat) & al))) return false;
+    const int cols = C / VEC;
+    return 256 % (cols < 256 ? cols : 256) == 0;
 }
 
 template <typename FT>
@@ -962,8 +977,7 @@
                                     hspStream_t stream) {
     if (!grad_out || !rev_off || !rev_edge || !grad_feat || B <= 0 || Nsrc <= 0 || Nq <= 0 || C <= 0 || grad_stride < C)
         return HSP_ERR_BAD_ARG;
-    if ((C & 1) || (grad_stride & 1) || (reinterpret_cast<uintptr_t>(grad_out) & (2 * sizeof(FT) - 1)) ||
-        (256 % ((C >> 1) < 256 ? (C >> 1) : 256)))
+    if (!gather_bwd_csr_vec_ok<FT>(2, grad_out, grad_stride, C, grad_feat))
         return HSP_ERR_UNSUPPORTED;
     const int tpr = (C >> 1) < 256 ? (C >> 1) : 256;
     const int RB = 256 / tpr;
@@ -971,6 +985,49 @@
     hipLaunchKernelGGL(gather_rows_bwd_csr_kernel<FT>, dim3((unsigned)((rows + RB - 1) / RB)), dim3(256), 0, as_stream(stream),
                        grad_out, grad_stride, rev_off, rev_edge, B, Nsrc, Nq, C, grad_feat);
     return check_launch();
+}
+
+template <typename FT>
+static int gather_rows_bwd_csr_multi_impl(int nseg, const FT* const* grad_out, int grad_stride, const int32_t* const* rev_off,
+                                          const int32_t* const* rev_edge, int B, const int* Nsrc, int Nq, const int* C,
+                                          FT* const* grad_feat, hspStream_t stream) {
+    if (nseg <= 0 || nseg > 4 || !grad_out || !rev_off || !rev_edge || !Nsrc || !C || !grad_feat || B <= 0 || Nq <= 0)
+        return HSP_ERR_BAD_ARG;
+    for (int s = 0; s < nseg; ++s)
+        if (!grad_out[s] || !rev_off[s] || !rev_edge[s] || !grad_feat[s] || Nsrc[s] <= 0 || C[s] <= 0 || grad_stride < C[s])
+            return HSP_ERR_BAD_ARG;
+    int order[4] = {0, 1, 2, 3};
+    for (int i = 1; i < nseg; ++i)
+        for (int j = i; j > 0 && Nsrc[order[j]] < Nsrc[order[j - 1]]; --j) { const int t = order[j]; order[j] = order[j - 1]; order[j - 1] = t; }
+    GatherBwdDesc d;
+    d.nseg = nseg;
+    long long blocks = 0;
+    for (int i = 0; i < nseg; ++i) {
+        const int s = order[i];
+        if (!gather_bwd_csr_vec_ok<FT>(2, grad_out[s], grad_stride, C[s], grad_feat[s])) return HSP_ERR_UNSUPPORTED;
+        const int vec = gather_bwd_csr_vec_ok<FT>(4, grad_out[s], grad_stride, C[s], grad_feat[s]) ? 4 : 2;
+        const int cols = C[s] / vec;
+        const int RB = 256 / (cols < 256 ? cols : 256);
+        d.seg[i] = GatherBwdSeg{grad_out[s], rev_off[s], rev_edge[s], grad_feat[s], grad_stride, Nsrc[s], Nq, C[s], vec};
+        d.first[i] = (int)blocks;
+        blocks += ((long long)B * Nsrc[s] + RB - 1) / RB;
+        if (blocks > 0x7fffffffLL) return HSP_ERR_UNSUPPORTED;
+    }
+    d.first[nseg] = (int)blocks;
+    hipLaunchKernelGGL(gather_rows_bwd_csr_multi_kernel<FT>, dim3((unsigned)blocks), dim3(256), 0, as_stream(stream), d, B);
+    return check_launch();
+}
+extern "C" int hsp_gather_rows_bwd_csr_multi(int nseg, const float* const* grad_out, int grad_stride,
+                                             const int32_t* const* rev_off, const int32_t* const* rev_edge, int B,
+                                             const int* Nsrc, int Nq, const int* C, float* const* grad_feat, hspStream_t stream) {
+    return gather_rows_bwd_csr_multi_impl<float>(nseg, grad_out, grad_stride, rev_off, rev_edge, B, Nsrc, Nq, C, grad_feat, stream);
+}
+extern "C" int hsp_gather_rows_bwd_csr_multi_bf16(int nseg, const hsp_bf16_t* const* grad_out, int grad_stride,
+                                                  const int32_t* const* rev_off, const int32_t* const* rev_edge, int B,
+                                                  const int* Nsrc, int Nq, const int* C, hsp_bf16_t* const* grad_feat,
+                                                  hspStream_t stream) {
+    return gather_rows_bwd_csr_multi_impl<bf16_t>(nseg, reinterpret_cast<const bf16_t* const*>(grad_out), grad_stride, rev_off, rev_edge, B,
+                                                  Nsrc, Nq, C, reinterpret_cast<bf16_t* const*>(grad_feat), stream);
 }
 extern "C" int hsp_gather_rows_bwd_csr(const float* grad_out, int grad_stride, const int32_t* rev_off,
                                        const int32_t* rev_edge, int B, int Nsrc, int Nq, int C, float* grad_feat,
@@ -1118,6 +1175,14 @@
 static size_t colsum_cloud_lds(int B, int N, int C, int with_xyz) {
     const int rows = chunk_rows(B, N, C);
     return (1024 + (size_t)(with_xyz ? 4 : 1) * ((N + rows - 1) / rows) * (C >> 5)) * sizeof(float4);
+}
+namespace hsp {
+int colsum_cloud_plan(int B, int N, int C, int* rows, int* nchunk) {
+    if (!hsp_colsum_cloud_ok(B, N, C, 0)) return 0;
+    *rows = chunk_rows(B, N, C);
+    *nchunk = (N + *rows - 1) / *rows;
+    return 1;
+}
 }
 extern "C" int hsp_colsum_cloud_ok(int B, int N, int C, int with_xyz) {
     if (B <= 0 || B > 65535 || N <= 0 || C <= 0 || (C & 31) || !colsum_vec4(C)) return 0;
diff --git a/hs_pose_amd/csrc/gemm.hip b/hs_pose_amd/csrc/gemm.hip
--- a/hs_pose_amd/csrc/gemm.hip
+++ b/hs_pose_amd/csrc/gemm.hip
@@ -1,5 +1,6 @@
 #include "common.h"
 #include "folds.h"
+#include "colsum_cloud.h"
 
 namespace hsp {
 
@@ -139,7 +140,18 @@
 }
 
 struct WgradProb { const float* A; const float* B; float* part; int lda, ldb, M, N, K, SK, kslice; };
-__global__ __launch_bounds__(256) void wgrad_pair_kernel(const WgradProb p0, const WgradProb p1, int blocks0) {
+struct ColsumRider { const float* x; float* out; int N, C, nchunk, rows, tpb, per_cloud; };
+__global__ __launch_bounds__(256) void wgrad_pair_kernel(const WgradProb p0, const WgradProb p1, int blocks0, int blocks01,
+                                                         const ColsumRider r) {
+    if ((int)blockIdx.x >= blocks01) {
+        extern __shared__ __attribute__((aligned(16))) char smem[];
+        const int rb = (int)blockIdx.x - blocks01;
+        const int b = rb / r.per_cloud, t0 = (rb - b * r.per_cloud) * r.tpb;
+        for (int t = 0; t < r.tpb; ++t)
+            colsum_cloud_body<false, 256, 4>(reinterpret_cast<float4*>(smem), t0 + t, b, r.x, nullptr, r.N, r.C, r.nchunk, r.rows,
+                                             r.out);
+        return;
+    }
     const bool second = (int)blockIdx.x >= blocks0;
     const WgradProb& p = second ? p1 : p0;
     wgrad_body<false, 4, float>((int)blockIdx.x - (second ? blocks0 : 0), p.A, p.lda, p.B, p.ldb, p.M, p.N, p.K, p.SK, p.kslice,
@@ -715,15 +727,16 @@
     if (!pending) return HSP_ERR_BAD_ARG;
     return wgrad_impl<bf16_t>(A, lda, B, ldb, M, N, K, C, ldc, colsum_B, ws, ws_bytes, stream, pending);
 }
-extern "C" int hsp_wgrad_partial_pair_f32(const float* A0, int lda0, const float* B0, int ldb0, int M0, int N0, int K0, float* C0,
-                                          int ldc0, void* ws0, size_t ws_bytes0, const float* A1, int lda1, const float* B1,
-                                          int ldb1, int M1, int N1, int K1, float* C1, int ldc1, void* ws1, size_t ws_bytes1,
-                                          HspWgradPending* pending, hspStream_t stream) {
+static int wgrad_pair_impl(const float* A0, int lda0, const float* B0, int ldb0, int M0, int N0, int K0, float* C0, int ldc0, void* ws0,
+                           size_t ws_bytes0, const float* A1, int lda1, const float* B1, int ldb1, int M1, int N1, int K1, float* C1,
+                           int ldc1, void* ws1, size_t ws_bytes1, HspWgradPending* pending, const float* cs_x, int cs_B, int cs_N,
+                           int cs_C, float* cs_out, hspStream_t stream) {
     if (!pending) return HSP_ERR_BAD_ARG;
     int ks0, kb0, ks1, kb1;
     const bool shapes_ok = A0 && B0 && C0 && A1 && B1 && C1 && M0 > 0 && N0 > 0 && K0 > 0 && M1 > 0 && N1 > 0 && K1 > 0 &&
                            !((M0 | N0 | M1 | N1) & 63) && !((lda0 | ldb0 | lda1 | ldb1) & 1) && lda0 >= M0 && ldb0 >= N0 &&
                            lda1 >= M1 && ldb1 >= N1 && ldc0 >= N0 && ldc1 >= N1;
+    if (cs_x && !shapes_ok) return HSP_ERR_UNSUPPORTED;
     if (shapes_ok) {
         int sk0 = wgrad_pick_sk(M0, N0, K0, &ks0, &kb0), sk1 = wgrad_pick_sk(M1, N1, K1, &ks1, &kb1);
         if (kb0 == 4 && kb1 == 4) {
@@ -750,6 +763,20 @@
             const WgradProb p1{A1, B1, reinterpret_cast<float*>(ws1), lda1, ldb1, M1, N1, K1, sk1, ks1};
             const int blocks0 = (M0 >> 6) * (N0 >> 6) * (sk0 / 4), blocks1 = (M1 >> 6) * (N1 >> 6) * (sk1 / 4);
             const size_t lds = (size_t)4 * 4 * 16 * 64 * sizeof(float) + (size_t)4 * 64 * sizeof(float2);
+            ColsumRider rider{nullptr, nullptr, 0, 0, 0, 0, 1, 1};
+            int rider_blocks = 0;
+            if (cs_x) {
+                int rows, nchunk;
+                if (!cs_out || cs_B <= 0 || cs_N <= 0 || cs_C <= 0) return HSP_ERR_BAD_ARG;
+                if (!colsum_cloud_plan(cs_B, cs_N, cs_C, &rows, &nchunk)) return HSP_ERR_UNSUPPORTED;
+                if (((size_t)4 * 256 + (size_t)nchunk * (cs_C >> 5)) * sizeof(float4) > lds) return HSP_ERR_UNSUPPORTED;
+                const long long room = 2LL * HSP_NUM_CU - blocks0 - blocks1;
+                int tpb = 1;
+                while (tpb <= 8 && (long long)cs_B * (8 / tpb) > room) tpb <<= 1;
+                if (tpb > 8) return HSP_ERR_UNSUPPORTED;
+                rider = ColsumRider{cs_x, cs_out, cs_N, cs_C, nchunk, rows, tpb, 8 / tpb};
+                rider_blocks = cs_B * (8 / tpb);
+            }
             static bool attr_set = false;
             if (!attr_set) {
                 hipError_t e = hipFuncSetAttribute(reinterpret_cast<const void*>(wgrad_pair_kernel),
@@ -757,7 +784,8 @@
                 if (e != hipSuccess) { set_last_hip_error(e); return HSP_ERR_LAUNCH; }
                 attr_set = true;
             }
-            hipLaunchKernelGGL(wgrad_pair_kernel, dim3(blocks0 + blocks1), dim3(256), lds, as_stream(stream), p0, p1, blocks0);
+            hipLaunchKernelGGL(wgrad_pair_kernel, dim3(blocks0 + blocks1 + rider_blocks), dim3(256), lds, as_stream(stream), p0, p1,
+                               blocks0, blocks0 + blocks1, rider);
             int rc = check_launch();
             if (rc) return rc;
             pending[0] = HspWgradPending{p0.part, nullptr, C0, nullptr, sk0 / 4, M0, N0, ldc0};
@@ -765,9 +793,26 @@
             return HSP_OK;
         }
     }
+    if (cs_x) return HSP_ERR_UNSUPPORTED;
     int rc = wgrad_impl<float>(A0, lda0, B0, ldb0, M0, N0, K0, C0, ldc0, nullptr, ws0, ws_bytes0, stream, pending);
     if (rc) return rc;
     return wgrad_impl<float>(A1, lda1, B1, ldb1, M1, N1, K1, C1, ldc1, nullptr, ws1, ws_bytes1, stream, pending + 1);
+}
+extern "C" int hsp_wgrad_partial_pair_f32(const float* A0, int lda0, const float* B0, int ldb0, int M0, int N0, int K0, float* C0,
+                                          int ldc0, void* ws0, size_t ws_bytes0, const float* A1, int lda1, const float* B1,
+                                          int ldb1, int M1, int N1, int K1, float* C1, int ldc1, void* ws1, size_t ws_bytes1,
+                                          HspWgradPending* pending, hspStream_t stream) {
+    return wgrad_pair_impl(A0, lda0, B0, ldb0, M0, N0, K0, C0, ldc0, ws0, ws_bytes0, A1, lda1, B1, ldb1, M1, N1, K1, C1, ldc1, ws1,
+                           ws_bytes1, pending, nullptr, 0, 0, 0, nullptr, stream);
+}
+extern "C" int hsp_wgrad_partial_pair_colsum_f32(const float* A0, int lda0, const float* B0, int ldb0, int M0, int N0, int K0,
+                                                 float* C0, int ldc0, void* ws0, size_t ws_bytes0, const float* A1, int lda1,
+                                                 const float* B1, int ldb1, int M1, int N1, int K1, float* C1, int ldc1, void* ws1,
+                                                 size_t ws_bytes1, HspWgradPending* pending, const float* x, int B, int N, int C,
+                                                 float* out, hspStream_t stream) {
+    if (!x || !out) return HSP_ERR_BAD_ARG;
+    return wgrad_pair_impl(A0, lda0, B0, ldb0, M0, N0, K0, C0, ldc0, ws0, ws_bytes0, A1, lda1, B1, ldb1, M1, N1, K1, C1, ldc1, ws1,
+                           ws_bytes1, pending, x, B, N, C, out, stream);
 }
 
 extern "C" int hsp_wgrad_fold(const HspWgradPending* pending, int n, hspStream_t stream) {
diff --git a/hs_pose_amd/ops.py b/hs_pose_amd/ops.py
--- a/hs_pose_amd/ops.py
+++ b/hs_pose_amd/ops.py
@@ -78,7 +78,10 @@
     return prev
 
 
-def _run(name, args, key="", abytes=0, aflops=0):
+_ERR_UNSUPPORTED = -2
+
+
+def _run(name, args, key="", abytes=0, aflops=0, may_decline=False):
     fn = getattr(lib(), name)
     t = _timer
     if t is not None and (t.only is None or name in t.only):
@@ -87,10 +90,14 @@
         e0.record()
         rc = fn(*args)
         e1.record()
-        t.records.append((name, key, abytes, aflops, e0, e1))
+        if not (may_decline and rc == _ERR_UNSUPPORTED):
+            t.records.append((name, key, abytes, aflops, e0, e1))
     else:
         rc = fn(*args)
+    if may_decline and rc == _ERR_UNSUPPORTED:
+        return False
     check(rc, name)
+    return True
 
 
 
@@ -243,6 +250,33 @@
     return off, edge
 
 
+def rev_index_multi(items):
+    missing = []
+    for idx, k, n_src in items:
+        cache = getattr(idx, "_hsp_rev", None)
+        if (cache is None or (k, n_src) not in cache) and not any(m[0] is idx and m[1:] == (k, n_src) for m in missing):
+            missing.append((idx, k, n_src))
+    if 2 <= len(missing) <= 4 and len({m[0].shape[0] for m in missing}) == 1:
+        n = len(missing)
+        B = missing[0][0].shape[0]
+        dims = [((idx.shape[1], 1) if idx.dim() == 2 else (idx.shape[1], idx.shape[2])) for idx, _, _ in missing]
+        offs = [torch.empty(B, n_src + 1, dtype=torch.int32, device=idx.device) for idx, _, n_src in missing]
+        edges = [torch.empty(B, nq * k, dtype=torch.int32, device=idx.device) for (idx, k, _), (nq, _) in zip(missing, dims)]
+        ptrs = lambda ts: ctypes.cast((ctypes.c_void_p * n)(*[t.data_ptr() for t in ts]), _vp)
+        ints = lambda vs: ctypes.cast((ctypes.c_int * n)(*vs), _vp)
+        _run("hsp_rev_build_multi", (n, ptrs([m[0] for m in missing]), B, ints([d[0] for d in dims]), ints([m[2] for m in missing]),
+                                     ints([m[1] for m in missing]), ints([d[1] for d in dims]), ptrs(offs), ptrs(edges), _stream()),
+             key=f"B{B}" + "+".join(f"Nq{d[0]}k{m[1]}" for m, d in zip(missing, dims)),
+             abytes=B * sum(8 * d[0] * m[1] + 4 * m[2] for m, d in zip(missing, dims)))
+        for (idx, k, n_src), off, edge in zip(missing, offs, edges):
+            cache = getattr(idx, "_hsp_rev", None)
+            if cache is None:
+                cache = {}
+                idx._hsp_rev = cache
+            cache[(k, n_src)] = (off, edge)
+    return [rev_index(idx, k, n_src) for idx, k, n_src in items]
+
+
 
 class _RFSurface(torch.autograd.Function):
     @staticmethod
@@ -606,12 +640,12 @@
             and A2.stride(0) % 2 == 0 and B2.stride(0) % 2 == 0 and A2.dtype in _FEAT_DTYPES and A2.is_cuda)
 
 
-def wgrad_pair(A0, B0, out0, A1, B1, out1):
+def wgrad_pair(A0, B0, out0, A1, B1, out1, colsum_of=None):
     batch = WgradBatch.current
     if batch is None or A0.dtype != torch.float32 or not _wgrad_ok(A0, B0, out0) or not _wgrad_ok(A1, B1, out1):
         wgrad(A0, B0, out=out0)
         wgrad(A1, B1, out=out1)
-        return
+        return False
     from ._lib import HspWgradPending
     L = lib()
     (K0, M0), N0 = A0.shape, B0.shape[1]
@@ -619,13 +653,21 @@
     wsb0, wsb1 = L.hsp_wgrad_workspace_bytes(M0, N0, K0), L.hsp_wgrad_workspace_bytes(M1, N1, K1)
     ws0, ws1 = _ws(wsb0, A0.device), _ws(wsb1, A0.device)
     pend = (HspWgradPending * 2)()
-    _run("hsp_wgrad_partial_pair_f32", (_p(A0), A0.stride(0), _p(B0), B0.stride(0), M0, N0, K0, _p(out0), out0.stride(0), _p(ws0), wsb0,
-                                        _p(A1), A1.stride(0), _p(B1), B1.stride(0), M1, N1, K1, _p(out1), out1.stride(0), _p(ws1), wsb1,
-                                        pend, _stream()),
-         key=f"M{M0}N{N0}K{K0}+M{M1}N{N1}K{K1}", abytes=4 * (K0 * (M0 + N0) + M0 * N0 + K1 * (M1 + N1) + M1 * N1),
-         aflops=2 * (M0 * N0 * K0 + M1 * N1 * K1))
+    pair = (_p(A0), A0.stride(0), _p(B0), B0.stride(0), M0, N0, K0, _p(out0), out0.stride(0), _p(ws0), wsb0,
+            _p(A1), A1.stride(0), _p(B1), B1.stride(0), M1, N1, K1, _p(out1), out1.stride(0), _p(ws1), wsb1, pend)
+    key, ab = f"M{M0}N{N0}K{K0}+M{M1}N{N1}K{K1}", 4 * (K0 * (M0 + N0) + M0 * N0 + K1 * (M1 + N1) + M1 * N1)
+    rode = False
+    if colsum_of is not None:
+        gx, mom = colsum_of
+        Bc, Nc, Cc = gx.shape
+        rode = _run("hsp_wgrad_partial_pair_colsum_f32", (*pair, _p(gx), Bc, Nc, Cc, _p(mom), _stream()),
+                    key=key + f"+cs B{Bc}N{Nc}C{Cc}", abytes=ab + 4 * Bc * Nc * Cc, aflops=2 * (M0 * N0 * K0 + M1 * N1 * K1),
+                    may_decline=True)
+    if not rode:
+        _run("hsp_wgrad_partial_pair_f32", (*pair, _stream()), key=key, abytes=ab, aflops=2 * (M0 * N0 * K0 + M1 * N1 * K1))
     batch.items.append((HspWgradPending.from_buffer_copy(pend[0]), ws0, _hold(out0)))
     batch.items.append((HspWgradPending.from_buffer_copy(pend[1]), ws1, _hold(out1)))
+    return rode
 
 
 def _ld(t):
@@ -1072,12 +1114,16 @@
             and lib().hsp_colsum_cloud_ok(B, N, C, 1 if with_xyz else 0) == 1)
 
 
-def _orl_bwd_small(g, xyz, fg, Wb, gWb, gste=None):
+COLSUM_RIDER = False
+
+
+def _orl_bwd_small(g, xyz, fg, Wb, gWb, gste=None, mom=None):
     B, N, C = g.shape
     ns = 4 if xyz is not None else 1
-    mom = torch.empty(B, ns * C, dtype=torch.float32, device=g.device)
-    _run("hsp_colsum_cloud_f32", (_p(g), _p(xyz), B, N, C, _p(mom), _stream()), key=f"B{B}N{N}C{C}{'x' if xyz is not None else ''}",
-         abytes=B * N * (4 * C + (12 if xyz is not None else 0)))
+    if mom is None:
+        mom = torch.empty(B, ns * C, dtype=torch.float32, device=g.device)
+        _run("hsp_colsum_cloud_f32", (_p(g), _p(xyz), B, N, C, _p(mom), _stream()), key=f"B{B}N{N}C{C}{'x' if xyz is not None else ''}",
+             abytes=B * N * (4 * C + (12 if xyz is not None else 0)))
     if _between_launches_hook is not None:
         _between_launches_hook(mom)
     gfg = torch.empty(B, C, dtype=torch.float32, device=g.device)
@@ -1277,13 +1323,21 @@
         Wb = w_conv2[:, C:]
         small = f32 and _orl_bwd_small_ok(B, N, C, False)
         g_conv2 = torch.empty_like(w_conv2)
-        if small:
+        rider = small and COLSUM_RIDER
+        if rider:
+            pass
+        elif small:
             gfg_n = _orl_bwd_small(g, None, fg, Wb, g_conv2[:, C:])
         else:
             gt = colsum_rows(g)
         with WgradBatch(), x3_scope(ctx.x3):
             g_ste = torch.empty(C, Cin, dtype=torch.float32, device=g.device)
-            wgrad_pair(g2, F2, g_conv2[:, :C], g2, X2, g_ste)
+            if rider:
+                mom = torch.empty(B, C, dtype=torch.float32, device=g.device)
+                rode = wgrad_pair(g2, F2, g_conv2[:, :C], g2, X2, g_ste, colsum_of=(g, mom))
+                gfg_n = _orl_bwd_small(g, None, fg, Wb, g_conv2[:, C:], mom=mom if rode else None)
+            else:
+                wgrad_pair(g2, F2, g_conv2[:, :C], g2, X2, g_ste)
             if not small:
                 _tiny_tn(gt, fg, g_conv2[:, C:])
             gF3 = torch.empty(B, N, C, dtype=g.dtype, device=g.device)
@@ -1860,6 +1914,8 @@
 
 ONE_HOT_WIDTH = 6
 
+CONCAT_BWD_MERGE = True
+
 FEAT_PITCH_ALIGN = 8
 
 
@@ -1904,11 +1960,37 @@
         return out
 
     @staticmethod
+    def _csr_ok(gs, w, W, es):
+        return w % 2 == 0 and W % 2 == 0 and (w // 2 >= 256 or 256 % (w // 2) == 0) and gs.data_ptr() % (2 * es) == 0
+
+    @staticmethod
     def backward(ctx, g):
         if not g.is_contiguous():
             g = g.contiguous()
         B, N, W = g.shape
         saved = list(ctx.saved_tensors)
+        es = _es(g)
+        merged = {}
+        if CONCAT_BWD_MERGE:
+            col, it, todo = 0, iter(saved), []
+            for s_, (kd, w) in enumerate(zip(ctx.kinds, ctx.widths)):
+                idx = next(it) if ctx.has_idx[s_] else None
+                gs = g[:, :, col:col + w]
+                if kd == 1 and ctx.needs_input_grad[2 + s_] and _AssembleFeat._csr_ok(gs, w, W, es):
+                    todo.append((s_, idx, ctx.nsrc[s_], w, gs))
+                col += w
+            if 2 <= len(todo) <= 4:
+                n = len(todo)
+                revs = rev_index_multi([(idx, 1, Ns) for _, idx, Ns, _, _ in todo])
+                outs = [torch.empty(B, Ns, w, dtype=g.dtype, device=g.device) for _, _, Ns, w, _ in todo]
+                ptrs = lambda ts: ctypes.cast((ctypes.c_void_p * n)(*[t.data_ptr() for t in ts]), _vp)
+                ints = lambda vs: ctypes.cast((ctypes.c_int * n)(*vs), _vp)
+                if _run("hsp_gather_rows_bwd_csr_multi" + _sfx(g),
+                        (n, ptrs([t[4] for t in todo]), W, ptrs([r[0] for r in revs]), ptrs([r[1] for r in revs]), B,
+                         ints([t[2] for t in todo]), N, ints([t[3] for t in todo]), ptrs(outs), _stream()),
+                        key=f"B{B}Nq{N}" + "+".join(f"Ns{t[2]}C{t[3]}" for t in todo),
+                        abytes=B * sum(es * t[2] * t[3] + N * (4 + es * t[3]) for t in todo), may_decline=True):
+                    merged = {t[0]: o for t, o in zip(todo, outs)}
         grads, col = [], 0
         for s_, (kd, w) in enumerate(zip(ctx.kinds, ctx.widths)):
             gs = g[:, :, col:col + w]
@@ -1918,12 +2000,14 @@
                     saved.pop(0)
             elif kd == 0:
                 grads.append(gs)
+            elif kd == 1 and s_ in merged:
+                saved.pop(0)
+                grads.append(merged[s_])
             elif kd == 1:
                 idx = saved.pop(0)
                 Ns = ctx.nsrc[s_]
                 gfeat = torch.empty(B, Ns, w, dtype=g.dtype, device=g.device)
-                es = _es(g)
-                if w % 2 == 0 and W % 2 == 0 and (w // 2 >= 256 or 256 % (w // 2) == 0) and gs.data_ptr() % (2 * es) == 0:
+                if _AssembleFeat._csr_ok(gs, w, W, es):
                     off, edge = rev_index(idx, 1, Ns)
                     _run("hsp_gather_rows_bwd_csr" + _sfx(g), (_p(gs), W, _p(off), _p(edge), B, Ns, N, w, _p(gfeat), _stream()),
                          key=f"B{B}Ns{Ns}Nq{N}C{w}", abytes=B * (es * Ns * w + N * (4 + es * w)))
diff --git a/include/hsp.h b/include/hsp.h
--- a/include/hsp.h
+++ b/include/hsp.h
@@ -71,6 +71,8 @@
 
 int hsp_rev_build(const int32_t *idx, int B, int Nq, int Nsrc, int k, int kstride, int32_t *rev_off,
                   int32_t *rev_edge, hspStream_t stream);
+int hsp_rev_build_multi(int nmaps, const int32_t *const *idx, int B, const int *Nq, const int *Nsrc, const int *k,
+                        const int *kstride, int32_t *const *rev_off, int32_t *const *rev_edge, hspStream_t stream);
 
 int hsp_gather_max_fwd(const float *feat, const int32_t *idx, const int32_t *qsel, int B, int Nsrc,
                        int Nidx, int Nq, int k, int kstride, int C, float *out, uint8_t *argmax,
@@ -119,6 +121,9 @@
                         int Nsrc, int Nq, int C, float *grad_feat, hspStream_t stream);
 int hsp_gather_rows_bwd_csr(const float *grad_out, int grad_stride, const int32_t *rev_off, const int32_t *rev_edge,
                             int B, int Nsrc, int Nq, int C, float *grad_feat, hspStream_t stream);
+int hsp_gather_rows_bwd_csr_multi(int nseg, const float *const *grad_out, int grad_stride, const int32_t *const *rev_off,
+                                  const int32_t *const *rev_edge, int B, const int *Nsrc, int Nq, const int *C,
+                                  float *const *grad_feat, hspStream_t stream);
 
 int hsp_gemm_rows_f32(const float *A1, int lda1, const float *B1, int ldb1, int b1_layout, int K1,
                       const float *A2, int lda2, const float *B2, int ldb2, int b2_layout, int K2, int M, int N,
@@ -210,6 +215,11 @@
                                void *ws0, size_t ws_bytes0, const float *A1, int lda1, const float *B1, int ldb1, int M1, int N1,
                                int K1, float *C1, int ldc1, void *ws1, size_t ws_bytes1, HspWgradPending *pending,
                                hspStream_t stream);
+int hsp_wgrad_partial_pair_colsum_f32(const float *A0, int lda0, const float *B0, int ldb0, int M0, int N0, int K0, float *C0,
+                                      int ldc0, void *ws0, size_t ws_bytes0, const float *A1, int lda1, const float *B1, int ldb1,
+                                      int M1, int N1, int K1, float *C1, int ldc1, void *ws1, size_t ws_bytes1,
+                                      HspWgradPending *pending, const float *x, int B, int N, int C, float *out,
+                                      hspStream_t stream);
 int hsp_wgrad_f32(const float *A, int lda, const float *B, int ldb, int M, int N, int K, float *C, int ldc,
                   float *colsum_B, void *ws, size_t ws_bytes, hspStream_t stream);
 int hsp_wgrad_partial_f32(const float *A, int lda, const float *B, int ldb, int M, int N, int K, float *C, int ldc,
@@ -293,6 +303,9 @@
 int hsp_gather_rows_bwd_csr_bf16(const hsp_bf16_t *grad_out, int grad_stride, const int32_t *rev_off,
                                  const int32_t *rev_edge, int B, int Nsrc, int Nq, int C, hsp_bf16_t *grad_feat,
                                  hspStream_t stream);
+int hsp_gather_rows_bwd_csr_multi_bf16(int nseg, const hsp_bf16_t *const *grad_out, int grad_stride,
+                                       const int32_t *const *rev_off, const int32_t *const *rev_edge, int B, const int *Nsrc,
+                                       int Nq, const int *C, hsp_bf16_t *const *grad_feat, hspStream_t stream);
 int hsp_wgrad_bf16(const hsp_bf16_t *A, int lda, const hsp_bf16_t *B, int ldb, int M, int N, int K, float *C, int ldc,
                    float *colsum_B, void *ws, size_t ws_bytes, hspStream_t stream);
 int hsp_wgrad_partial_bf16(const hsp_bf16_t *A, int lda, const hsp_bf16_t *B, int ldb, int M, int N, int K, float *C, int ldc,
```

Measured after the change: 9481 point-clouds/sec, median of 6. 1.01x the previous value.
